# AI4Science-WestlakeU/wdno

Hardware: AMD Instinct MI355X
Metric: diffusion train steps/sec, 2D smoke U-Net (8 samples per GPU per step) (higher is better)
Workload: dtype f32

## Files before the change

### include/wdno_hip.h

```cpp
#ifndef WDNO_HIP_H
#define WDNO_HIP_H
#include <stdint.h>
#include <stddef.h>

#ifdef __cplusplus
extern "C" {
#endif

typedef void* wdno_stream_t;

enum { WDNO_OK = 0, WDNO_EINVAL = -1, WDNO_ELAUNCH = -2, WDNO_EUNSUPPORTED = -3, WDNO_EWORKSPACE = -4 };

#define WDNO_AMAX_SLOTS 64
#define WDNO_AMAX_STRIDE 16
#define WDNO_AMAX_FLOATS (WDNO_AMAX_SLOTS * WDNO_AMAX_STRIDE)
const char* wdno_strerror(int code);
int wdno_version(void);
const char* wdno_last_hip_error(void);
int wdno_set_debug(int mode);

typedef struct {
  int nd;
  int mode;
  int L;
  int n_img;
  int in_dims[3];
  int out_dims[3];
  int64_t cs_img, cs_band, cs0, cs1;
} wdno_dwt_desc;
size_t wdno_dwt_ws_bytes(const wdno_dwt_desc* d);
int wdno_dwt_fwd(const float* x, float* coef, const wdno_dwt_desc* d, const float* filters_host, void* ws, size_t ws_bytes, wdno_stream_t s);
int wdno_dwt_inv(const float* coef, float* x, const wdno_dwt_desc* d, const float* filters_host, void* ws, size_t ws_bytes, wdno_stream_t s);
int wdno_dwt_fwd_adjoint(const float* dcoef, float* dx, const wdno_dwt_desc* d, const float* filters_host, void* ws, size_t ws_bytes, wdno_stream_t s);
int wdno_dwt_inv_adjoint(const float* dx, float* dcoef, const wdno_dwt_desc* d, const float* filters_host, void* ws, size_t ws_bytes, wdno_stream_t s);
int wdno_dwt_fwd_packed(const float* x, float* state, const wdno_dwt_desc* d, const float* filters_host, int img_inner, int64_t cs_outer, int row_w,
                        const float* rescaler, wdno_stream_t s);
int wdno_upsample_coef(const float* in, float* out, int64_t outer, int a, int mid, int b, int c, int fa, int fb, int fc, wdno_stream_t s);
int wdno_pack_smoke_state(const float* coef, int64_t coef_sim_stride, const float* init_coef, int64_t init_sim_stride, const float* smokeout,
                          int64_t so_sim_stride, const int64_t* idx, const float* rescaler, float* state, int64_t B, int F, int nt, int nx,
                          int pad_t, int pad_x, wdno_stream_t s);
int wdno_pack_smoke_fields(const float* coef, int64_t coef_sim_stride, const float* rho0, int64_t rho0_sim_stride, const float* curve,
                           int64_t curve_sim_stride, const float* dec_lo_host, const float* dec_hi_host, int L, const float* rescaler,
                           float* state, int64_t B, int F, int nt, int nx, int pad_t, int pad_x, int H0, int W0, int T0, wdno_stream_t s);

int wdno_nc_to_cl(const float* src, float* dst, int64_t N, int C, int64_t S, int Cp, wdno_stream_t s);
int wdno_cl_to_nc(const float* src, float* dst, int64_t N, int C, int64_t S, int Cp, wdno_stream_t s);
int wdno_concat2_cl_planes(const float* a, int Ca, const float* b, int Cb, const float* rec_a, const float* rec_b, void* hi, void* lo,
                           float* scale_out, int64_t P, wdno_stream_t s);
int wdno_concat2_cl(const float* a, int Ca, const float* b, int Cb, float* out, int64_t P, wdno_stream_t s);
int wdno_concat2_cl_amax(const float* a, int Ca, const float* b, int Cb, float* out, float* amax_rec, int64_t P, wdno_stream_t s);
int wdno_split2_cl(const float* in, float* a, int Ca, float* b, int Cb, int64_t P, wdno_stream_t s);
int wdno_upsample2x_cl_fwd(const float* in, float* out, int64_t N, int H, int W, int C, wdno_stream_t s);
int wdno_upsample2x_cl_bwd(const float* dout, float* din, int64_t N, int H, int W, int C, wdno_stream_t s);

typedef struct {
  int N, D, H, W, C;
  int OD, OH, OW, K;
  int kd, kh, kw;
  int sd, sh, sw;
  int pd, ph, pw;
  int YD, YH, YW;
  int osd, osh, osw, ood, ooh, oow;
} wdno_conv_geom;
int wdno_conv_fwd(const float* x, const float* wp, const float* bias, const float* residual, float* y,
                  const wdno_conv_geom* g, wdno_stream_t s);
int wdno_amax(const float* x, int64_t n, float* amax_zeroed, wdno_stream_t s);
int wdno_amax_record(const float* x, int64_t n, float* rec_zeroed, wdno_stream_t s);
int wdno_split_f16(const float* x, const float* amax_rec, void* hi, void* lo, float* scale_out, int64_t rows, int C, int C8, wdno_stream_t s);
size_t wdno_split_colsum_ws_bytes(int64_t rows, int C8);
int wdno_split_f16_colsum(const float* x, const float* amax_rec, void* hi, void* lo, float* scale_out, float* colsum_out,
                          void* ws, size_t ws_bytes, int64_t rows, int C, int C8, wdno_stream_t s);
int wdno_pack_split_weight(const float* w, const float* amax, void* hi, void* lo, float* scale_out, int K, int C, int kd, int kh, int kw,
                           int A, int B, int mode, wdno_stream_t s);
typedef struct { const void* x; int64_t n; void* out; } wdno_amax_item;
typedef struct {
  const void* w; const void* amax; void* hi; void* lo; void* scale_out;
  int K, C, kd, kh, kw, A, B, mode;
} wdno_wsplit_item;
int wdno_amax_multi(const void* table, int n_items, int blocks_per_item, wdno_stream_t s);
int wdno_pack_split_weight_multi(const void* table, int n_items, int blocks_per_item, wdno_stream_t s);
int wdno_conv_fwd_f16x3(const void* xh, const void* xl, const float* sx, const void* wph, const void* wpl, const float* sw,
                        const float* bias, const float* residual, float* y, const wdno_conv_geom* g, wdno_stream_t s);
int wdno_conv_fwd_f16x3_amax(const void* xh, const void* xl, const float* sx, const void* wph, const void* wpl, const float* sw,
                             const float* bias, const float* residual, float* y, float* amax_rec, const wdno_conv_geom* g,
                             wdno_stream_t s);
typedef struct { int channels, d0, h0, w0; } wdno_zero_box;
int wdno_conv_fwd_f16x3_zbox(const void* xh, const void* xl, const float* sx, const void* wph, const void* wpl, const float* sw,
                             const float* bias, const float* residual, float* y, float* amax_rec, const wdno_conv_geom* g,
                             const wdno_zero_box* zb, wdno_stream_t s);
int wdno_conv_fwd_bf16_ex(const void* x16, const void* wp16, const float* bias, const float* residual, void* y, int y_bf16, float* amax_rec,
                          const wdno_conv_geom* g, const wdno_zero_box* zb, wdno_stream_t s);
int wdno_conv_fwd_f16x3_ws(const void* xh, const void* xl, const float* sx, const void* wph, const void* wpl, const float* sw,
                           const float* bias, const float* residual, float* y, float* amax_rec, const wdno_conv_geom* g,
                           void* ws, size_t ws_bytes, wdno_stream_t s);
size_t wdno_conv_fwd_split_ws_bytes(const wdno_conv_geom* g);
size_t wdno_conv_wgrad_f16x3_ws_bytes(const wdno_conv_geom* g);
int wdno_conv_pixel_table(void* table, const wdno_conv_geom* g, wdno_stream_t s);
int wdno_conv_wgrad_f16x3(const void* xh, const void* xl, const float* sx, const void* dyh, const void* dyl, const float* sdy,
                          const void* pixel_table, float* dwp, void* ws, size_t ws_bytes, const wdno_conv_geom* g, wdno_stream_t s);
int wdno_conv_wgrad_f16x3_param(const void* xh, const void* xl, const float* sx, const void* dyh, const void* dyl, const float* sdy,
                                const void* pixel_table, float* dw, int Kn, int Cn, void* ws, size_t ws_bytes,
                                const wdno_conv_geom* g, wdno_stream_t s);
#define WDNO_WGRAD_REDUCE_MAX 40
typedef struct wdno_wgrad_reduce_item {
  const float* ws; float* dw;
  int n, splits;
  int K8, C8, kw, ntap, Kn, Cn;
  int tiled;
  int reserved;
} wdno_wgrad_reduce_item;
int wdno_conv_wgrad_partials(const void* xh, const void* xl, const float* sx, const void* dyh, const void* dyl, const float* sdy,
                             const void* pixel_table, float* dw, int Kn, int Cn, void* ws, size_t ws_bytes,
                             const wdno_conv_geom* g, wdno_wgrad_reduce_item* item, wdno_stream_t s);
int wdno_wgrad_reduce_multi(const wdno_wgrad_reduce_item* items, int n_items, wdno_stream_t s);
size_t wdno_conv_wgrad_ws_bytes(const wdno_conv_geom* g);
int wdno_conv_wgrad(const float* x, const float* dy, float* dwp, void* ws, size_t ws_bytes,
                    const wdno_conv_geom* g, wdno_stream_t s);
#define WDNO_ROWS_SUM_MAX 64
typedef struct wdno_rows_sum_item {
  const void* part; float* out;
  int rows, stride, col0, ncols;
  int is_double, reserved;
} wdno_rows_sum_item;
int wdno_rows_sum_multi(const wdno_rows_sum_item* items, int n_items, wdno_stream_t s);
size_t wdno_colsum_ws_bytes(int64_t P, int C);
int wdno_colsum(const float* in, float* out, int64_t P, int C, void* ws, size_t ws_bytes, wdno_stream_t s);

int wdno_cast_bf16(const float* x, void* out16, int64_t rows, int C, int C8, wdno_stream_t s);
int wdno_cast_bf16_colsum(const float* x, void* out16, float* colsum_out, void* ws, size_t ws_bytes, int64_t rows, int C, int C8, wdno_stream_t s);
int wdno_conv_fwd_bf16(const void* x16, const void* wp16, const float* bias, const float* residual, float* y, float* amax_rec,
                       const wdno_conv_geom* g, wdno_stream_t s);
int wdno_conv_wgrad_bf16_param(const void* x16, const void* dy16, const void* pixel_table, float* dw, int Kn, int Cn, void* ws,
                               size_t ws_bytes, const wdno_conv_geom* g, wdno_stream_t s);

size_t wdno_groupnorm_ws_bytes(int64_t N, int64_t S, int C, int G);
size_t wdno_groupnorm_stats_floats(int64_t N, int C, int G);
int wdno_groupnorm_act_fwd(const float* x, const float* gamma, const float* beta, const float* ss, float* y,
                           float* stats, int64_t N, int64_t S, int C, int G, float eps, int silu,
                           void* ws, size_t ws_bytes, wdno_stream_t s);
int wdno_groupnorm_act_fwd_amax(const float* x, const float* gamma, const float* beta, const float* ss, float* y,
                                float* stats, float* amax_rec, int64_t N, int64_t S, int C, int G, float eps, int silu,
                                void* ws, size_t ws_bytes, wdno_stream_t s);
int wdno_groupnorm_act_bwd(const float* x, const float* dy, const float* gamma, const float* beta, const float* ss,
                           const float* stats, float* dx, float* dgb_partial, float* dss,
                           int64_t N, int64_t S, int C, int G, int silu, void* ws, size_t ws_bytes, wdno_stream_t s);
int wdno_groupnorm_act_bwd_amax(const float* x, const float* dy, const float* gamma, const float* beta, const float* ss,
                                const float* stats, float* dx, float* dgb_partial, float* dss, float* amax_rec,
                                int64_t N, int64_t S, int C, int G, int silu, void* ws, size_t ws_bytes, wdno_stream_t s);
size_t wdno_groupnorm_bwd_planes_ws_bytes(int64_t N, int64_t S, int C, int G);
size_t wdno_groupnorm_fwd_planes_ws_bytes(int64_t N, int64_t S, int C, int G);
int wdno_groupnorm_act_fwd_planes(const float* x, const float* gamma, const float* beta, const float* ss, void* y_hi, void* y_lo,
                                  float* y_scale, float* stats, float* bound_rec, int64_t N, int64_t S, int C, int G, float eps, int silu,
                                  void* ws, size_t ws_bytes, wdno_stream_t s);
int wdno_groupnorm_act_add_fwd_planes(const float* x, const float* gamma, const float* beta, const float* ss, const float* residual,
                                      const float* res_rec, float* y, void* y_hi, void* y_lo, float* y_scale, float* stats,
                                      float* bound_rec, float* y_amax_rec, int64_t N, int64_t S, int C, int G, float eps, int silu,
                                      void* ws, size_t ws_bytes, wdno_stream_t s);
int wdno_groupnorm_act_bwd_planes(const float* x, const float* dy, const float* gamma, const float* beta, const float* ss,
                                  const float* stats, void* dx_hi, void* dx_lo, float* dx_scale, float* dx_colsum,
                                  float* dgb_partial, float* dgb_sum, float* dss, float* bound_rec, int64_t N, int64_t S, int C, int G, int silu,
                                  void* ws, size_t ws_bytes, wdno_stream_t s);
int wdno_groupnorm_bwd_planes_tail(int64_t N, int64_t S, int C, int G, size_t* csp_offset, int* rows);
int wdno_groupnorm_act_fwd_amax_t(const void* x, int x_bf16, const float* gamma, const float* beta, const float* ss, float* y,
                                  float* stats, float* amax_rec, int64_t N, int64_t S, int C, int G, float eps, int silu,
                                  void* ws, size_t ws_bytes, wdno_stream_t s);
int wdno_groupnorm_act_fwd_planes_t(const void* x, int x_bf16, const float* gamma, const float* beta, const float* ss, void* y_hi, void* y_lo,
                                    float* y_scale, float* stats, float* bound_rec, int64_t N, int64_t S, int C, int G, float eps,
                                    int silu, void* ws, size_t ws_bytes, wdno_stream_t s);
int wdno_groupnorm_act_add_fwd_planes_t(const void* x, int x_bf16, const float* gamma, const float* beta, const float* ss, const float* residual,
                                        const float* res_rec, float* y, void* y_hi, void* y_lo, float* y_scale, float* stats,
                                        float* bound_rec, float* y_amax_rec, int64_t N, int64_t S, int C, int G, float eps, int silu,
                                        void* ws, size_t ws_bytes, wdno_stream_t s);
int wdno_groupnorm_act_bwd_planes_t(const void* x, int x_bf16, const void* dy, int dy_bf16, const float* gamma, const float* beta, const float* ss,
                                    const float* stats, void* dx_hi, void* dx_lo, float* dx_scale, float* dx_colsum,
                                    float* dgb_partial, float* dgb_sum, float* dss, float* bound_rec, int64_t N, int64_t S, int C, int G, int silu,
                                    void* ws, size_t ws_bytes, wdno_stream_t s);
int wdno_layernorm_fwd(const float* x, const float* g, float* y, int64_t P, int C, float eps, wdno_stream_t s);
int wdno_layernorm_fwd_amax(const float* x, const float* g, float* y, float* amax_rec, int64_t P, int C, float eps, wdno_stream_t s);
int wdno_layernorm_fwd_planes(const float* x, const float* g, void* y_hi, void* y_lo, float* y_scale, int64_t P, int C, float eps,
                              wdno_stream_t s);
size_t wdno_layernorm_bwd_ws_bytes(int64_t P, int C);
int wdno_layernorm_bwd(const float* x, const float* g, const float* dy, float* dx, float* dg, int64_t P, int C,
                       float eps, void* ws, size_t ws_bytes, wdno_stream_t s);
int wdno_layernorm_bwd_add(const float* x, const float* g, const float* dy, const float* add_to, float* dx, float* dg, int64_t P, int C,
                           float eps, void* ws, size_t ws_bytes, wdno_stream_t s);
int wdno_layernorm_bwd_add_amax(const float* x, const float* g, const float* dy, const float* add_to, float* dx, float* dg, float* amax_rec,
                                int64_t P, int C, float eps, void* ws, size_t ws_bytes, wdno_stream_t s);

typedef struct {
  int n_uo, n_ui, n_tok, heads;
  int64_t so, si, st;
} wdno_attn_desc;
int wdno_attn_fwd(const float* qkv, const float* rot_cos, const float* rot_sin, const float* bias, float* out,
                  const wdno_attn_desc* d, float scale, wdno_stream_t s);
size_t wdno_attn_bwd_ws_bytes(const wdno_attn_desc* d);
int wdno_attn_bwd(const float* qkv, const float* rot_cos, const float* rot_sin, const float* bias, const float* out,
                  const float* dout, float* dqkv, float* dbias, const wdno_attn_desc* d, float scale, void* ws, size_t ws_bytes,
                  wdno_stream_t s);
int wdno_attn_fwd_amax(const float* qkv, const float* rot_cos, const float* rot_sin, const float* bias, float* out, float* amax_rec,
                       const wdno_attn_desc* d, float scale, wdno_stream_t s);
int wdno_attn_bwd_amax(const float* qkv, const float* rot_cos, const float* rot_sin, const float* bias, const float* out,
                       const float* dout, float* dqkv, float* dbias, float* amax_rec, const wdno_attn_desc* d, float scale,
                       void* ws, size_t ws_bytes, wdno_stream_t s);
int wdno_attn_bwd_planes(const float* qkv, const float* rot_cos, const float* rot_sin, const float* bias, const float* out,
                         const float* dout, void* dqkv_hi, void* dqkv_lo, float* dqkv_scale, float* dbias,
                         const float* rec_qkv, const float* rec_dout, const wdno_attn_desc* d, float scale, void* ws, size_t ws_bytes,
                         wdno_stream_t s);
int wdno_attn_fwd_planes(const float* qkv, const float* rot_cos, const float* rot_sin, const float* bias, float* out, void* out_hi,
                         void* out_lo, float* out_scale, float* amax_rec, const float* rec_qkv, const wdno_attn_desc* d, float scale,
                         wdno_stream_t s);
size_t wdno_linattn_ws_bytes(int64_t units, int heads);
int wdno_linattn_fwd(const float* qkv, float* out, float* kstats , float* ctx ,
                     int64_t units, int n_tok, int heads, float scale, wdno_stream_t s);
int wdno_linattn_bwd(const float* qkv, const float* dout, const float* kstats, const float* ctx, float* dqkv,
                     void* ws, size_t ws_bytes, int64_t units, int n_tok, int heads, float scale, wdno_stream_t s);
int wdno_linattn_fwd_amax(const float* qkv, float* out, float* kstats, float* ctx, float* amax_rec, int64_t units, int n_tok, int heads,
                          float scale, wdno_stream_t s);
int wdno_linattn_bwd_amax(const float* qkv, const float* dout, const float* kstats, const float* ctx, float* dqkv, float* amax_rec,
                          void* ws, size_t ws_bytes, int64_t units, int n_tok, int heads, float scale, wdno_stream_t s);
int wdno_linattn_bwd_planes(const float* qkv, const float* dout, const float* kstats, const float* ctx, void* dqkv_hi, void* dqkv_lo,
                            float* dqkv_scale, const float* rec_qkv, const float* rec_dout, float* rec_dctx, void* ws, size_t ws_bytes,
                            int64_t units, int n_tok, int heads, float scale, wdno_stream_t s);
int wdno_linattn_fwd_planes(const float* qkv, void* out_hi, void* out_lo, float* out_scale, float* kstats, float* ctx,
                            const float* rec_qkv, int64_t units, int n_tok, int heads, float scale, wdno_stream_t s);

int wdno_tattn_fused_takes(int C, int n_tok, int heads);
int wdno_tattn_fused_fwd(const float* x, const float* gamma, float eps, const void* wq_hi, const void* wq_lo, const float* wq_scale,
                         const void* wo_hi, const void* wo_lo, const float* wo_scale, const float* rot_cos, const float* rot_sin,
                         const float* bias, float* y, float* amax_rec, float* qkv_out, float* rec_v,
                         int64_t n_batch, int n_tok, int64_t hw, int C, int heads, float scale, wdno_stream_t s);
size_t wdno_tattn_fused_bwd_ws_bytes(void);
int wdno_tattn_fused_bwd_grads(void);
int wdno_tattn_fused_bwd(const float* x, const float* dy, const float* gamma, float eps, const void* wq_hi, const void* wq_lo,
                         const float* wq_scale, const void* wo_hi, const void* wo_lo, const float* wo_scale, const float* rot_cos,
                         const float* rot_sin, const float* bias, const float* rec_dy, const float* rec_v, float* dx, float* amax_rec,
                         float* grads, void* ws, size_t ws_bytes,
                         int64_t n_batch, int n_tok, int64_t hw, int C, int heads, float scale, wdno_stream_t s);

int wdno_lattn_fused_takes(int C, int heads, int n_tok);
size_t wdno_lattn_fused_ws_bytes(int64_t units, int n_tok);
int wdno_lattn_fused_fwd(const float* x, const float* gamma, float eps, const void* wq_hi, const void* wq_lo, const float* wq_scale,
                         const void* wo_hi, const void* wo_lo, const float* wo_scale, const float* bias_out, float* y, float* amax_rec,
                         float* ctx_out, float* kstat_out, void* ws, size_t ws_bytes, int64_t units, int n_tok, int C, int heads, float scale,
                         wdno_stream_t s);

int wdno_lattn_fused_bwd_grads(void);
size_t wdno_lattn_fused_bwd_ws_bytes(int64_t units, int n_tok);
int wdno_lattn_fused_bwd(const float* x, const float* dy, const float* gamma, float eps, const void* wq_hi, const void* wq_lo,
                         const float* wq_scale, const void* wot_hi, const void* wot_lo, const float* wot_scale, const float* ctx,
                         const float* kstat, const float* rec_dy, float* dx, float* amax_rec, float* grads, void* ws, size_t ws_bytes,
                         int64_t units, int n_tok, int C, int heads, float scale, wdno_stream_t s);

int wdno_relpos_bias_fwd(const float* w, const int64_t* bucket, float* out, int n, int heads, wdno_stream_t s);
int wdno_relpos_bias_bwd(const float* dbias, const int64_t* bucket, float* dw, int n, int heads, int num_buckets, wdno_stream_t s);

int wdno_linear_rows_fwd(const float* x, int x_stride, const float* w, int w_stride, const float* bias, float* y, int P, int C, int K,
                         int Kp, wdno_stream_t s);
int wdno_linear_rows_wgrad(const float* x, int x_stride, const float* dy, int dy_stride, float* dw, float* db, int P, int C, int K,
                           wdno_stream_t s);
// ... 112 lines not shown
```

### wdno_amd/_lib.py

```python
import contextlib
import ctypes as C
import os

import torch

HERE = os.path.dirname(os.path.abspath(__file__))
LIB_PATH = os.path.join(HERE, 'libwdno_hip.so')

P = C.c_void_p
I = C.c_int
L = C.c_int64
F = C.c_float
Z = C.c_size_t


class DwtDesc(C.Structure):
    _fields_ = [('nd', I), ('mode', I), ('L', I), ('n_img', I), ('in_dims', I * 3), ('out_dims', I * 3),
                ('cs_img', L), ('cs_band', L), ('cs0', L), ('cs1', L)]


class ConvGeom(C.Structure):
    _fields_ = [(k, I) for k in ('N', 'D', 'H', 'W', 'C', 'OD', 'OH', 'OW', 'K', 'kd', 'kh', 'kw', 'sd', 'sh', 'sw',
                                 'pd', 'ph', 'pw', 'YD', 'YH', 'YW', 'osd', 'osh', 'osw', 'ood', 'ooh', 'oow')]


class AttnDesc(C.Structure):
    _fields_ = [('n_uo', I), ('n_ui', I), ('n_tok', I), ('heads', I), ('so', L), ('si', L), ('st', L)]


class CondDesc(C.Structure):
    _fields_ = [(k, I) for k in ('tree', 'B', 'F', 'C', 'H', 'W', 'cT', 'cH', 'cW', 'cond_pad', 'cond_a', 'cond_b',
                                 'cond_c', 'cond_low', 'u_rows', 'uT_rows')]


class WgradReduceItem(C.Structure):
    _fields_ = [('ws', C.c_void_p), ('dw', C.c_void_p), ('n', I), ('splits', I), ('K8', I), ('C8', I), ('kw', I), ('ntap', I), ('Kn', I), ('Cn', I),
                ('tiled', I), ('reserved', I)]


class RowsSumItem(C.Structure):
    _fields_ = [('part', C.c_void_p), ('out', C.c_void_p), ('rows', I), ('stride', I), ('col0', I), ('ncols', I), ('is_double', I), ('reserved', I)]


class BurgersDesc(C.Structure):
    _fields_ = [(k, I) for k in ('N', 's', 'nx0', 'nt_f', 'nxf', 'steps', 'record_time', 'f_time', 'num_t', 'sub_s', 'out_cols', 'waves',
                                 'points')] + [(k, F) for k in ('c', 'd', 'dm', 'dt')]


class BurgersGenerateDesc(C.Structure):
    _fields_ = [(k, I) for k in ('N', 's', 't', 'steps', 'record_time', 'f_time', 'num_t', 'st', 'sx', 'f_rows', 'cols', 'waves', 'points',
                                 'clamp')] + [(k, F) for k in ('c', 'd', 'dm', 'dt', 'alpha')]


class BurgersGuidanceDesc(C.Structure):
    _fields_ = [(k, I) for k in ('B', 'C', 'H', 'W', 'sample_stride', 'chan_stride', 'row_stride', 'h', 'w', 'n_t', 'n_x', 'L', 'mode', 'ntile',
                                 'tw', 'lds_bytes', 'num_timesteps', 'condition_f', 'clip_x0')] + [(k, F) for k in ('wu', 'wf')]


class SmokeSolveDesc(C.Structure):
    _fields_ = [(k, I) for k in ('B', 'nt', 'nx', 'time_interval', 'space_interval', 'num_t', 'max_iter', 'n_out', 'threads')] + [('accuracy', F)]


class SmokeGenerateDesc(C.Structure):
    _fields_ = [(k, I) for k in ('B', 'scenelength', 'record_scale', 'stride', 'max_iter', 'threads', 'noise_mode')] + [('accuracy', F), ('seed', C.c_uint64)]


PD, PG, PA, PC = C.POINTER(DwtDesc), C.POINTER(ConvGeom), C.POINTER(AttnDesc), C.POINTER(CondDesc)
PF = C.POINTER(C.c_float)

PROTOTYPES = {
    'wdno_strerror': (C.c_char_p, [I]),
    'wdno_version': (I, []),
    'wdno_last_hip_error': (C.c_char_p, []),
    'wdno_set_debug': (I, [I]),
    'wdno_dwt_ws_bytes': (Z, [PD]),
    'wdno_dwt_fwd': (I, [P, P, PD, PF, P, Z, P]),
    'wdno_dwt_fwd_packed': (I, [P, P, PD, PF, I, L, I, P, P]),
    'wdno_dwt_inv': (I, [P, P, PD, PF, P, Z, P]),
    'wdno_dwt_fwd_adjoint': (I, [P, P, PD, PF, P, Z, P]),
    'wdno_dwt_inv_adjoint': (I, [P, P, PD, PF, P, Z, P]),
    'wdno_upsample_coef': (I, [P, P, L, I, I, I, I, I, I, I, P]),
    'wdno_pack_smoke_state': (I, [P, L, P, L, P, L, P, P, P, L, I, I, I, I, I, P]),
    'wdno_pack_smoke_fields': (I, [P, L, P, L, P, L, PF, PF, I, P, P, L, I, I, I, I, I, I, I, I, P]),
    'wdno_nc_to_cl': (I, [P, P, L, I, L, I, P]),
    'wdno_cl_to_nc': (I, [P, P, L, I, L, I, P]),
    'wdno_concat2_cl': (I, [P, I, P, I, P, L, P]),
    'wdno_concat2_cl_planes': (I, [P, I, P, I, P, P, P, P, P, L, P]),
    'wdno_concat2_cl_amax': (I, [P, I, P, I, P, P, L, P]),
    'wdno_split2_cl': (I, [P, P, I, P, I, L, P]),
    'wdno_upsample2x_cl_fwd': (I, [P, P, L, I, I, I, P]),
    'wdno_upsample2x_cl_bwd': (I, [P, P, L, I, I, I, P]),
    'wdno_conv_fwd': (I, [P, P, P, P, P, PG, P]),
    'wdno_amax': (I, [P, L, P, P]),
    'wdno_amax_record': (I, [P, L, P, P]),
    'wdno_split_f16': (I, [P, P, P, P, P, L, I, I, P]),
    'wdno_split_colsum_ws_bytes': (Z, [L, I]),
    'wdno_split_f16_colsum': (I, [P, P, P, P, P, P, P, Z, L, I, I, P]),
    'wdno_pack_split_weight': (I, [P, P, P, P, P, I, I, I, I, I, I, I, I, P]),
    'wdno_amax_multi': (I, [P, I, I, P]),
    'wdno_pack_split_weight_multi': (I, [P, I, I, P]),
    'wdno_conv_fwd_f16x3': (I, [P, P, P, P, P, P, P, P, P, PG, P]),
    'wdno_conv_fwd_f16x3_amax': (I, [P, P, P, P, P, P, P, P, P, P, PG, P]),
    'wdno_conv_fwd_f16x3_ws': (I, [P, P, P, P, P, P, P, P, P, P, PG, P, Z, P]),
    'wdno_conv_fwd_split_ws_bytes': (Z, [PG]),
    'wdno_conv_wgrad_f16x3_ws_bytes': (Z, [PG]),
    'wdno_conv_pixel_table': (I, [P, PG, P]),
    'wdno_conv_wgrad_f16x3': (I, [P, P, P, P, P, P, P, P, P, Z, PG, P]),
    'wdno_conv_wgrad_f16x3_param': (I, [P, P, P, P, P, P, P, P, I, I, P, Z, PG, P]),
    'wdno_conv_wgrad_partials': (I, [P, P, P, P, P, P, P, P, I, I, P, Z, PG, P, P]),
    'wdno_wgrad_reduce_multi': (I, [P, I, P]),
    'wdno_rows_sum_multi': (I, [P, I, P]),
    'wdno_cast_bf16': (I, [P, P, L, I, I, P]),
    'wdno_cast_bf16_colsum': (I, [P, P, P, P, Z, L, I, I, P]),
    'wdno_conv_fwd_bf16': (I, [P, P, P, P, P, P, PG, P]),
    'wdno_conv_fwd_f16x3_zbox': (I, [P, P, P, P, P, P, P, P, P, P, PG, P, P]),
    'wdno_conv_fwd_bf16_ex': (I, [P, P, P, P, P, I, P, PG, P, P]),
    'wdno_conv_wgrad_bf16_param': (I, [P, P, P, P, I, I, P, Z, PG, P]),
    'wdno_conv_wgrad_ws_bytes': (Z, [PG]),
    'wdno_conv_wgrad': (I, [P, P, P, P, Z, PG, P]),
    'wdno_colsum_ws_bytes': (Z, [L, I]),
    'wdno_colsum': (I, [P, P, L, I, P, Z, P]),
    'wdno_groupnorm_ws_bytes': (Z, [L, L, I, I]),
    'wdno_groupnorm_stats_floats': (Z, [L, I, I]),
    'wdno_groupnorm_act_fwd': (I, [P, P, P, P, P, P, L, L, I, I, F, I, P, Z, P]),
    'wdno_groupnorm_act_fwd_amax': (I, [P, P, P, P, P, P, P, L, L, I, I, F, I, P, Z, P]),
    'wdno_groupnorm_act_bwd': (I, [P, P, P, P, P, P, P, P, P, L, L, I, I, I, P, Z, P]),
    'wdno_groupnorm_act_bwd_amax': (I, [P, P, P, P, P, P, P, P, P, P, L, L, I, I, I, P, Z, P]),
    'wdno_groupnorm_bwd_planes_ws_bytes': (Z, [L, L, I, I]),
    'wdno_groupnorm_bwd_planes_tail': (I, [L, L, I, I, C.POINTER(Z), C.POINTER(I)]),
    'wdno_groupnorm_fwd_planes_ws_bytes': (Z, [L, L, I, I]),
    'wdno_groupnorm_act_fwd_planes': (I, [P, P, P, P, P, P, P, P, P, L, L, I, I, F, I, P, Z, P]),
    'wdno_groupnorm_act_add_fwd_planes': (I, [P, P, P, P, P, P, P, P, P, P, P, P, P, L, L, I, I, F, I, P, Z, P]),
    'wdno_layernorm_fwd_planes': (I, [P, P, P, P, P, L, I, F, P]),
    'wdno_groupnorm_act_bwd_planes': (I, [P, P, P, P, P, P, P, P, P, P, P, P, P, P, L, L, I, I, I, P, Z, P]),
    'wdno_groupnorm_act_fwd_amax_t': (I, [P, I, P, P, P, P, P, P, L, L, I, I, F, I, P, Z, P]),
    'wdno_groupnorm_act_fwd_planes_t': (I, [P, I, P, P, P, P, P, P, P, P, L, L, I, I, F, I, P, Z, P]),
    'wdno_groupnorm_act_add_fwd_planes_t': (I, [P, I, P, P, P, P, P, P, P, P, P, P, P, P, L, L, I, I, F, I, P, Z, P]),
    'wdno_groupnorm_act_bwd_planes_t': (I, [P, I, P, I, P, P, P, P, P, P, P, P, P, P, P, P, L, L, I, I, I, P, Z, P]),
    'wdno_layernorm_fwd': (I, [P, P, P, L, I, F, P]),
    'wdno_layernorm_fwd_amax': (I, [P, P, P, P, L, I, F, P]),
    'wdno_layernorm_bwd_ws_bytes': (Z, [L, I]),
    'wdno_layernorm_bwd': (I, [P, P, P, P, P, L, I, F, P, Z, P]),
    'wdno_layernorm_bwd_add': (I, [P, P, P, P, P, P, L, I, F, P, Z, P]),
    'wdno_layernorm_bwd_add_amax': (I, [P, P, P, P, P, P, P, L, I, F, P, Z, P]),
    'wdno_attn_fwd': (I, [P, P, P, P, P, PA, F, P]),
    'wdno_attn_bwd_ws_bytes': (Z, [PA]),
    'wdno_attn_bwd': (I, [P, P, P, P, P, P, P, P, PA, F, P, Z, P]),
    'wdno_attn_fwd_amax': (I, [P, P, P, P, P, P, PA, F, P]),
    'wdno_attn_bwd_amax': (I, [P, P, P, P, P, P, P, P, P, PA, F, P, Z, P]),
    'wdno_attn_fwd_planes': (I, [P, P, P, P, P, P, P, P, P, P, PA, F, P]),
    'wdno_linattn_fwd_planes': (I, [P, P, P, P, P, P, P, L, I, I, F, P]),
    'wdno_attn_bwd_planes': (I, [P, P, P, P, P, P, P, P, P, P, P, P, PA, F, P, Z, P]),
    'wdno_tattn_fused_takes': (I, [I, I, I]),
    'wdno_tattn_fused_fwd': (I, [P, P, F, P, P, P, P, P, P, P, P, P, P, P, P, P, L, I, L, I, I, F, P]),
    'wdno_lattn_fused_takes': (I, [I, I, I]),
    'wdno_lattn_fused_ws_bytes': (Z, [L, I]),
    'wdno_lattn_fused_fwd': (I, [P, P, F, P, P, P, P, P, P, P, P, P, P, P, P, Z, L, I, I, I, F, P]),
    'wdno_lattn_fused_bwd_grads': (I, []),
    'wdno_lattn_fused_bwd_ws_bytes': (Z, [L, I]),
    'wdno_lattn_fused_bwd': (I, [P, P, P, F, P, P, P, P, P, P, P, P, P, P, P, P, P, Z, L, I, I, I, F, P]),
    'wdno_tattn_fused_bwd_ws_bytes': (Z, []),
    'wdno_tattn_fused_bwd_grads': (I, []),
    'wdno_tattn_fused_bwd': (I, [P, P, P, F, P, P, P, P, P, P, P, P, P, P, P, P, P, P, P, Z, L, I, L, I, I, F, P]),
    'wdno_linattn_ws_bytes': (Z, [L, I]),
    'wdno_linattn_fwd': (I, [P, P, P, P, L, I, I, F, P]),
    'wdno_linattn_bwd': (I, [P, P, P, P, P, P, Z, L, I, I, F, P]),
    'wdno_linattn_fwd_amax': (I, [P, P, P, P, P, L, I, I, F, P]),
    'wdno_linattn_bwd_amax': (I, [P, P, P, P, P, P, P, Z, L, I, I, F, P]),
    'wdno_linattn_bwd_planes': (I, [P, P, P, P, P, P, P, P, P, P, P, Z, L, I, I, F, P]),
    'wdno_act_fwd': (I, [P, P, L, I, P]),
    'wdno_act_bwd': (I, [P, P, P, L, I, P]),
    'wdno_linear_rows_fwd': (I, [P, I, P, I, P, P, I, I, I, I, P]),
    'wdno_linear_rows_wgrad': (I, [P, I, P, I, P, P, I, I, I, P]),
    'wdno_linear_multi_fwd': (I, [P, I, I, P, P, I, I, P]),
    'wdno_linear_multi_wgrad': (I, [P, I, I, P, P, P, P, I, I, P]),
    'wdno_linear_multi_dgrad_ws_bytes': (Z, [I, I, I]),
    'wdno_linear_multi_dgrad': (I, [P, I, I, P, P, I, I, P, Z, P]),
    'wdno_add': (I, [P, P, P, L, P]),
    'wdno_add_amax': (I, [P, P, P, P, L, P]),
    'wdno_sinusoidal_emb': (I, [P, P, P, I, I, P]),
    'wdno_q_sample_cond': (I, [P, P, P, P, P, P, P, PC, P]),
    'wdno_apply_cond': (I, [P, P, PC, P]),
    'wdno_weighted_mse_ws_bytes': (Z, [L]),
    'wdno_weighted_mse': (I, [P, P, P, P, F, P, P, L, L, I, L, P, Z, P]),
    'wdno_weighted_mse_bwd': (I, [P, P, P, P, F, P, P, L, L, I, L, P]),
    'wdno_p_sample_update': (I, [P, P, P, P, P, P, P, P, P, P, P, L, L, I, P]),
    'wdno_ddim_update': (I, [P, P, P, P, P, P, F, F, F, P, P, L, L, P]),
    'wdno_ddim_update_dev': (I, [P, P, P, P, P, P, P, P, P, L, L, P]),
    'wdno_sumsq_ws_bytes': (Z, [L]),
    'wdno_sumsq': (I, [P, L, P, P, Z, P]),
    'wdno_adam_clip_step': (I, [P, P, P, P, L, P, F, F, F, F, F, F, I, P]),
    'wdno_ema_update': (I, [P, P, L, F, P]),
    'wdno_gather_items': (I, [P, I, I, P]),
    'wdno_relpos_bias_fwd': (I, [P, P, P, I, I, P]),
    'wdno_relpos_bias_bwd': (I, [P, P, P, I, I, I, P]),
    'wdno_burgers_solve': (I, [P, P, P, C.POINTER(BurgersDesc), P]),
    'wdno_burgers_generate': (I, [P, P, P, P, P, C.POINTER(BurgersGenerateDesc), P]),
    'wdno_burgers_guidance': (I, [P, P, P, P, P, P, P, P, P, C.POINTER(BurgersGuidanceDesc), PF, P]),
    'wdno_smoke_solve': (I, [P, P, P, P, P, P, P, P, P, P, P, P, P, P, C.POINTER(SmokeSolveDesc), P]),
    'wdno_smoke_generate': (I, [P, P, P, P, P, P, P, P, P, P, P, P, P, P, C.POINTER(SmokeGenerateDesc), P]),
    'wdno_smoke_noise': (I, [P, P, P, P, I, C.c_uint64, P, P]),
}

_lib = None


def load():
    global _lib
    if _lib is not None:
        return _lib
    if not os.path.exists(LIB_PATH):
        raise RuntimeError(f'{LIB_PATH} is missing: run `python -c "import __graft_entry__ as g; g.build()"` '
                           '(there is no CPU / eager fallback for the wdno_amd hot path)')
    lib = C.CDLL(LIB_PATH)
    for name, (res, args) in PROTOTYPES.items():
        fn = getattr(lib, name)
        fn.restype = res
        fn.argtypes = args
    _lib = lib
    if os.environ.get('WDNO_DEBUG'):
# ... 25 lines not shown
```

### wdno_amd/csrc/conv_common.h

```cpp
#pragma once
#include "common.h"

typedef float f32x16 __attribute__((ext_vector_type(16)));

#define BK 32
#define LDS_STRIDE 36

struct ConvP {
  wdno_conv_geom g;
  int R;
  int nchunk;
  int nsteps;
  int64_t P;
  int identity_out;
  int debug;
  int tiles_n;
  int ntiles;
  int ksplit;
  float* amax_rec;
  int tsplit;
  float* split_ws;
  size_t split_ws_bytes;
  int zb_blocks, zb_d, zb_h;
  int out_bf16;
};

__device__ __forceinline__ int xcd_swizzle(int bid, int nwg) {
  int q = nwg >> 3, r = nwg & 7;
  int xcd = bid & 7, idx = bid >> 3;
  int start = xcd < r ? xcd * (q + 1) : r * (q + 1) + (xcd - r) * q;
  return start + idx;
}

__device__ __forceinline__ int64_t out_row(const wdno_conv_geom& g, int64_t p) {
  int ow = (int)(p % g.OW); int64_t t = p / g.OW;
  int oh = (int)(t % g.OH); t /= g.OH;
  int od = (int)(t % g.OD);
  int64_t n = t / g.OD;
  return ((n * g.YD + (od * g.osd + g.ood)) * g.YH + (oh * g.osh + g.ooh)) * g.YW + (ow * g.osw + g.oow);
}

static inline int check_geom(const wdno_conv_geom* g) {
  if (!g) return WDNO_EINVAL;
  if (g->N <= 0 || g->D <= 0 || g->H <= 0 || g->W <= 0 || g->C <= 0 || g->K <= 0) return WDNO_EINVAL;
  if (g->OD <= 0 || g->OH <= 0 || g->OW <= 0 || g->kd <= 0 || g->kh <= 0 || g->kw <= 0) return WDNO_EINVAL;
  if (g->sd <= 0 || g->sh <= 0 || g->sw <= 0 || g->osd <= 0 || g->osh <= 0 || g->osw <= 0) return WDNO_EINVAL;
  if ((g->C & 3) || (g->K & 3)) return WDNO_EUNSUPPORTED;
  if ((g->OD - 1) * g->osd + g->ood >= g->YD || (g->OH - 1) * g->osh + g->ooh >= g->YH || (g->OW - 1) * g->osw + g->oow >= g->YW)
    return WDNO_EINVAL;
  return WDNO_OK;
}
#include "debug_modes.h"
void wdno_wgrad_h3d_plan(const wdno_conv_geom* g, int* bm, int* bn, int* splits, int* pix_per_split, int* splitpair = nullptr);
int wdno_conv_wgrad_h3_dma(const void* xh, const void* xl, const void* dyh, const void* dyl, const float* sx, const float* sdy,
                           const void* table, float* wsf, const wdno_conv_geom* g, hipStream_t st);
int wdno_conv_fwd_h3_dma(const void* xh, const void* xl, const void* wh, const void* wl, const float* sx, const float* sw,
                         const float* bias, const float* residual, float* y, ConvP& p, hipStream_t st, int stages);
bool wdno_conv_h3t_takes(const wdno_conv_geom& g);
int wdno_conv_h3t_split(const wdno_conv_geom& g, int64_t P, int cus);
int wdno_conv_fwd_h3_tap(int shape, const void* xh, const void* xl, const void* wh, const void* wl, const float* sx, const float* sw,
                         const float* bias, const float* residual, float* y, ConvP& p, hipStream_t st);
#ifdef __HIPCC__
__device__ __forceinline__ uint4 bf16x8_from_runs(float4 va, float4 vb) {
  const uint2 A = bf16x4_pack(va), B = bf16x4_pack(vb);
  const auto sx = __builtin_amdgcn_permlane32_swap(A.x, B.x, false, false);
  const auto sy = __builtin_amdgcn_permlane32_swap(A.y, B.y, false, false);
  return make_uint4(sx[0], sy[0], sx[1], sy[1]);
}
__device__ __forceinline__ void lgkm0_barrier() {
  __builtin_amdgcn_s_waitcnt(0xc07f);
  asm volatile("s_barrier" : : : "memory");
}
#endif
static inline void fill_params(ConvP& p, const wdno_conv_geom* g) {
  p.g = *g;
  p.amax_rec = nullptr;
  p.ksplit = 1;
  p.tsplit = 1;
  p.split_ws = nullptr;
  p.split_ws_bytes = 0;
  p.zb_blocks = 0; p.zb_d = 0; p.zb_h = 0;
  p.out_bf16 = 0;
  p.debug = wdno_debug_mode;
  p.R = g->kw * g->C;
  p.nchunk = cdiv(p.R, BK);
  p.nsteps = g->kd * g->kh * p.nchunk;
  p.P = (int64_t)g->N * g->OD * g->OH * g->OW;
  p.identity_out = (g->YD == g->OD && g->YH == g->OH && g->YW == g->OW && g->osd == 1 && g->osh == 1 && g->osw == 1 &&
                    g->ood == 0 && g->ooh == 0 && g->oow == 0) ? 1 : 0;
}
```

### wdno_amd/csrc/conv_h3.hip

```cpp
#include "conv_common.h"
#include <type_traits>
#include <algorithm>

typedef _Float16 half8 __attribute__((ext_vector_type(8)));
typedef __bf16 bf16x8 __attribute__((ext_vector_type(8)));
template <bool LP>
__device__ __forceinline__ f32x16 mfma_16(half8 a, half8 b, f32x16 c) {
  if constexpr (LP) return __builtin_amdgcn_mfma_f32_32x32x16_bf16(__builtin_bit_cast(bf16x8, a), __builtin_bit_cast(bf16x8, b), c, 0, 0, 0);
  else return __builtin_amdgcn_mfma_f32_32x32x16_f16(a, b, c, 0, 0, 0);
}

#define HBK 32
#define HST 40

template <bool RECORD>
__global__ __launch_bounds__(256) void amax_kernel(const float* __restrict__ x, int64_t n, unsigned* __restrict__ out) {
  __shared__ float red[4];
  const int64_t n4 = n >> 2;
  const float4* x4 = reinterpret_cast<const float4*>(x);
  float m = 0.f;
  const int64_t stride = (int64_t)gridDim.x * 1024;
  for (int64_t k0 = (int64_t)blockIdx.x * 1024 + threadIdx.x; k0 < n4; k0 += stride) {
    float4 v[4];
#pragma unroll
// ... 392 lines not shown
  __syncthreads();
  if (nst > 1) load_tile(S1{});
  if (nst > 2) load_tile(S0{});
  for (int step = 0; step < nst; step += 2) {
    iter(S0{}, step);
    if (step + 1 < nst) iter(S1{}, step + 1);
  }

  const float inv = LP ? 1.0f : 1.0f / (sx[0] * sw[0]);
  float am = 0.f;
#pragma unroll
  for (int a = 0; a < TM; ++a) {
#pragma unroll
    for (int e = 0; e < 16; ++e) {
      int row = (e & 3) + 8 * (e >> 2) + 4 * hh;
      int64_t pm = m0 + m_base + a * 32 + row;
      if (pm >= p.P) continue;
      int64_t yr = p.identity_out ? pm : out_row(g, pm);
#pragma unroll
      for (int b = 0; b < TN; ++b) {
        int kc = n0 + n_base + b * 32 + li;
        if (kc < g.K) {
          float v = acc[a][b][e] * inv;
          if (p.ksplit > 1) {
            if (blockIdx.y == 0) {
              if (bias) v += bias[kc];
              if (res) v += res[yr * g.K + kc];
            }
            unsafeAtomicAdd(&y[yr * g.K + kc], v);
            continue;
          }
          if (bias) v += bias[kc];
          if (res) v += res[yr * g.K + kc];
          if (LP && p.out_bf16) reinterpret_cast<unsigned short*>(y)[yr * g.K + kc] = bf16_rne(v);
          else y[yr * g.K + kc] = v;
          am = fmaxf(am, fabsf(v));
        }
      }
    }
  }
  if (p.amax_rec) wave_amax_emit(am, p.amax_rec, (int)blockIdx.x * 4 + wave);
}

template <int BM, int BN, int WM, int WN, bool LP>
static int launch_h3(const void* xh, const void* xl, const void* wh, const void* wl, const float* sx, const float* sw,
                     const float* bias, const float* residual, float* y, ConvP& p, hipStream_t st) {
  const wdno_conv_geom& g = p.g;
  int64_t tiles_m = cdiv64(p.P, BM);
  p.tiles_n = cdiv(g.K, BN);
  int64_t nt = tiles_m * p.tiles_n;
  if (nt > 0x7fffffff) return WDNO_EUNSUPPORTED;
  p.ntiles = (int)nt;
  size_t lds = (size_t)2 * (LP ? 1 : 2) * (BM + BN) * HST * sizeof(_Float16);
  static bool attr_done = false;
  if (!attr_done) {
    (void)hipFuncSetAttribute((const void*)conv_fwd_h3_kernel<BM, BN, WM, WN, LP>, hipFuncAttributeMaxDynamicSharedMemorySize, (int)lds);
    attr_done = true;
  }
  const int64_t x_elems = (int64_t)g.N * g.D * g.H * g.W * g.C;
  const int64_t w_elems = (int64_t)g.kd * g.kh * g.K * p.R;
  if (x_elems * 2 >= OOB_OFFSET || w_elems * 2 >= OOB_OFFSET || p.P >= 0x7fffffff) return WDNO_EUNSUPPORTED;
  float* rec = p.amax_rec;
  if (p.ksplit > 1) {
    if (hipMemsetAsync(y, 0, (size_t)p.P * g.K * sizeof(float), st) != hipSuccess) return WDNO_ELAUNCH;
    p.amax_rec = nullptr;
  }
  conv_fwd_h3_kernel<BM, BN, WM, WN, LP><<<dim3((unsigned)p.ntiles, (unsigned)p.ksplit), 256, lds, st>>>(
      (const _Float16*)xh, (const _Float16*)xl, (const _Float16*)wh, (const _Float16*)wl, sx, sw, bias, residual, y, p,
      (unsigned)(x_elems * 2), (unsigned)(w_elems * 2));
  if (p.ksplit > 1 && rec) {
    amax_kernel<true><<<stream_grid(p.P * g.K / 16 + 1, 256), 256, 0, st>>>(y, p.P * g.K, reinterpret_cast<unsigned*>(rec));
    p.amax_rec = rec;
  }
  return WDNO_OK;
}

extern "C" int wdno_conv_fwd_f16x3(const void* xh, const void* xl, const float* sx, const void* wph, const void* wpl, const float* sw,
                                   const float* bias, const float* residual, float* y, const wdno_conv_geom* g, wdno_stream_t s) {
  return wdno_conv_fwd_f16x3_amax(xh, xl, sx, wph, wpl, sw, bias, residual, y, nullptr, g, s);
}
template <bool LP>
static int conv_fwd_16(const void* xh, const void* xl, const float* sx, const void* wph, const void* wpl, const float* sw,
                       const float* bias, const float* residual, float* y, float* amax_rec, const wdno_conv_geom* g, wdno_stream_t s,
                       float* split_ws = nullptr, size_t split_ws_bytes = 0, const wdno_zero_box* zb = nullptr, int y_bf16 = 0) {
  int rc = check_geom(g);
  if (rc) return rc;
  if (g->C & 7) return WDNO_EUNSUPPORTED;
  if (y_bf16 && (!LP || residual)) return WDNO_EUNSUPPORTED;
  ConvP p;
  fill_params(p, g);
  p.out_bf16 = y_bf16 ? 1 : 0;
  if (zb) {
    if (zb->channels < 0 || zb->d0 < 0 || zb->h0 < 0 || zb->w0 < 0) return WDNO_EINVAL;
    p.zb_blocks = zb->channels / 16; p.zb_d = zb->d0; p.zb_h = zb->h0;
  }
  p.amax_rec = amax_rec;
  p.split_ws = split_ws;
  p.split_ws_bytes = split_ws_bytes;
  p.nchunk = cdiv(p.R, HBK);
  p.nsteps = g->kd * g->kh * p.nchunk;
  hipStream_t st = as_stream(s);
  const int64_t P = p.P;
  const int K = g->K;
  auto blocks = [&](int bm, int bn) { return cdiv64(P, bm) * cdiv(K, bn); };
  const int dbg = wdno_debug_mode;
  const bool small_tap = p.identity_out && wdno_conv_h3t_takes(*g) && g->kw == 3 && blocks(64, 64) >= 64;
  if (dbg != WDNO_DBG_ROW_ATTN_AND_REG_STAGED_CONV && (dbg == WDNO_DBG_FORCE_DMA_CONV || dbg == WDNO_DBG_CHUNKED_DMA_CONV || dbg == WDNO_DBG_FORCE_TILES_160 || dbg == WDNO_DBG_FORCE_TILES_320 || small_tap || (K > 64 ? blocks(128, 128) : blocks(256, 64)) >= 100)) {
    rc = wdno_conv_fwd_h3_dma(xh, LP ? nullptr : xl, wph, LP ? nullptr : wpl, sx, sw, bias, residual, y, p, st, 3);
    if (rc == WDNO_OK) return wdno_check_launch();
    if (rc != WDNO_EUNSUPPORTED) return rc;
  }
  if (K > 64) {
    if (blocks(128, 128) >= 512 || blocks(64, 128) < 2 * blocks(128, 128)) rc = launch_h3<128, 128, 2, 2, LP>(xh, xl, wph, wpl, sx, sw, bias, residual, y, p, st);
    else if (blocks(64, 128) < 200) {
      if (blocks(64, 64) <= 384 && g->kd * g->kh >= 2 && p.nsteps >= 64 && p.identity_out && residual != y && !LP) p.ksplit = 2;
      rc = launch_h3<64, 64, 2, 2, LP>(xh, xl, wph, wpl, sx, sw, bias, residual, y, p, st);
    }
    else rc = launch_h3<64, 128, 1, 4, LP>(xh, xl, wph, wpl, sx, sw, bias, residual, y, p, st);
  } else {
    if (blocks(128, 64) >= 512 || P <= 128) rc = launch_h3<128, 64, 4, 1, LP>(xh, xl, wph, wpl, sx, sw, bias, residual, y, p, st);
    else rc = launch_h3<64, 64, 2, 2, LP>(xh, xl, wph, wpl, sx, sw, bias, residual, y, p, st);
  }
  if (rc) return rc;
  return wdno_check_launch();
}
extern "C" int wdno_conv_fwd_f16x3_amax(const void* xh, const void* xl, const float* sx, const void* wph, const void* wpl, const float* sw,
                                        const float* bias, const float* residual, float* y, float* amax_rec, const wdno_conv_geom* g,
                                        wdno_stream_t s) {
  return conv_fwd_16<false>(xh, xl, sx, wph, wpl, sw, bias, residual, y, amax_rec, g, s);
}
extern "C" int wdno_conv_fwd_f16x3_ws(const void* xh, const void* xl, const float* sx, const void* wph, const void* wpl, const float* sw,
                                      const float* bias, const float* residual, float* y, float* amax_rec, const wdno_conv_geom* g,
                                      void* ws, size_t ws_bytes, wdno_stream_t s) {
  return conv_fwd_16<false>(xh, xl, sx, wph, wpl, sw, bias, residual, y, amax_rec, g, s, (float*)ws, ws ? ws_bytes : 0);
}
extern "C" int wdno_conv_fwd_f16x3_zbox(const void* xh, const void* xl, const float* sx, const void* wph, const void* wpl, const float* sw,
                                        const float* bias, const float* residual, float* y, float* amax_rec, const wdno_conv_geom* g,
                                        const wdno_zero_box* zb, wdno_stream_t s) {
  return conv_fwd_16<false>(xh, xl, sx, wph, wpl, sw, bias, residual, y, amax_rec, g, s, nullptr, 0, zb);
}
extern "C" int wdno_conv_fwd_bf16_ex(const void* x16, const void* wp16, const float* bias, const float* residual, void* y, int y_bf16, float* amax_rec,
                                     const wdno_conv_geom* g, const wdno_zero_box* zb, wdno_stream_t s) {
  return conv_fwd_16<true>(x16, x16, nullptr, wp16, wp16, nullptr, bias, residual, (float*)y, amax_rec, g, s, nullptr, 0, zb, y_bf16);
}
extern "C" size_t wdno_conv_fwd_split_ws_bytes(const wdno_conv_geom* g) {
  if (!g || check_geom(g) || (g->C & 7)) return 0;
  ConvP p;
  fill_params(p, g);
  if (!p.identity_out || !wdno_conv_h3t_takes(*g)) return 0;
  const int runs = wdno_conv_h3t_split(*g, p.P, wdno_num_cus() & ~7);
  return runs > 1 ? (size_t)runs * p.P * g->K * sizeof(float) : 0;
}
extern "C" int wdno_conv_fwd_bf16(const void* x16, const void* wp16, const float* bias, const float* residual, float* y, float* amax_rec,
                                  const wdno_conv_geom* g, wdno_stream_t s) {
  return conv_fwd_16<true>(x16, x16, nullptr, wp16, wp16, nullptr, bias, residual, y, amax_rec, g, s);
}

typedef _Float16 half4 __attribute__((ext_vector_type(4)));
#define WH_BKP 32
#define WH_PAD 32

__global__ __launch_bounds__(256) void pixel_table_kernel(int4v* __restrict__ tbl, wdno_conv_geom g, int P) {
  int p = blockIdx.x * 256 + threadIdx.x;
  if (p >= P) return;
  int q = p;
  int ow = q % g.OW; q /= g.OW;
  int oh = q % g.OH; q /= g.OH;
  int od = q % g.OD;
  int n = q / g.OD;
  int d0 = od * g.sd - g.pd, h0 = oh * g.sh - g.ph, w0 = ow * g.sw - g.pw;
  int4v e;
  e.x = ((n * g.YD + (od * g.osd + g.ood)) * g.YH + (oh * g.osh + g.ooh)) * g.YW + (ow * g.osw + g.oow);
  e.y = (((n * g.D + d0) * g.H + h0) * g.W + w0) * g.C;
  e.z = (d0 << 16) | (h0 & 0xffff);
  e.w = w0;
  tbl[p] = e;
}
extern "C" int wdno_conv_pixel_table(void* table, const wdno_conv_geom* g, wdno_stream_t s) {
  int rc = check_geom(g);
  if (rc) return rc;
  int64_t P = (int64_t)g->N * g->OD * g->OH * g->OW;
  if (P >= 0x7fffffff || (int64_t)g->N * g->D * g->H * g->W * g->C >= 0x3fffffff) return WDNO_EUNSUPPORTED;
  pixel_table_kernel<<<(unsigned)cdiv64(P, 256), 256, 0, as_stream(s)>>>((int4v*)table, *g, (int)P);
  return wdno_check_launch();
}

struct WgradHP {
  ConvP c;
  int tiles_k, tiles_r, splits, bn;
  int64_t pix_per_split;
  int xcd_group;
};

__device__ __forceinline__ half8 tr_frag(const _Float16* tile, int stride, int pix0, int ch0, int lane) {
  const int g = lane >> 4, xl = lane & 15;
  const _Float16* p0 = tile + (pix0 + 8 * (g >> 1) + (xl >> 2)) * stride + ch0 + 16 * (g & 1) + 4 * (xl & 3);
  typedef short short4v __attribute__((ext_vector_type(4)));
  typedef short4v __attribute__((address_space(3))) * lds_s4;
  short4v a = __builtin_amdgcn_ds_read_tr16_b64_v4i16((lds_s4)(p0));
  short4v b = __builtin_amdgcn_ds_read_tr16_b64_v4i16((lds_s4)(p0 + 4 * stride));
  typedef short short8v __attribute__((ext_vector_type(8)));
  short8v c = __builtin_shufflevector(a, b, 0, 1, 2, 3, 4, 5, 6, 7);
  return __builtin_bit_cast(half8, c);
}

#define WH_RING 4
template <int BM, int BN, int WM, int WN, bool LP>
__global__ __launch_bounds__(256) void conv_wgrad_h3_kernel(const _Float16* __restrict__ xh, const _Float16* __restrict__ xl,
                                                             const _Float16* __restrict__ dyh, const _Float16* __restrict__ dyl,
                                                             const float* __restrict__ sx, const float* __restrict__ sdy,
                                                             const int4v* __restrict__ table, float* __restrict__ ws, WgradHP wpz,
                                                             unsigned x_bytes, unsigned dy_bytes) {
  constexpr int TM = BM / (WM * 32);
  constexpr int TN = BN / (WN * 32);
  constexpr int SA = BM + WH_PAD, SB = BN + WH_PAD;
  constexpr int A_C8 = BM / 8, B_C8 = BN / 8;
  constexpr int A_RPP = 256 / A_C8;
  constexpr int A_PASSES = WH_BKP / A_RPP, B_PASSES = WH_BKP * B_C8 / 256;
  static_assert(256 % A_C8 == 0 && (WH_BKP * B_C8) % 256 == 0, "loader mapping");
  constexpr int NPL = LP ? 1 : 2;
  constexpr int STAGE = NPL * WH_BKP * (SA + SB);
  extern __shared__ __attribute__((aligned(16))) _Float16 hsm[];
  int4v* pinfo = reinterpret_cast<int4v*>(hsm + 2 * STAGE);

  const ConvP& p = wpz.c;
  const wdno_conv_geom& g = p.g;
// ... 618 lines not shown
```

### wdno_amd/csrc/conv_h3t.hip

```cpp
#include "conv_common.h"
#include <type_traits>

typedef _Float16 half8 __attribute__((ext_vector_type(8)));
typedef __bf16 bf16x8 __attribute__((ext_vector_type(8)));
typedef int int4v __attribute__((ext_vector_type(4)));
#define T_OOB 0x7ffffff0

template <bool LP>
__device__ __forceinline__ f32x16 t_mfma(half8 a, half8 b, f32x16 c) {
  if constexpr (LP) return __builtin_amdgcn_mfma_f32_32x32x16_bf16(__builtin_bit_cast(bf16x8, a), __builtin_bit_cast(bf16x8, b), c, 0, 0, 0);
  else return __builtin_amdgcn_mfma_f32_32x32x16_f16(a, b, c, 0, 0, 0);
}
__device__ __forceinline__ int4v t_rsrc(const void* ptr, unsigned bytes) {
  uint64_t a = reinterpret_cast<uint64_t>(ptr);
  int4v r;
  r.x = __builtin_amdgcn_readfirstlane((int)(unsigned)a);
  r.y = __builtin_amdgcn_readfirstlane((int)(unsigned)((a >> 32) & 0xffffu));
  r.z = __builtin_amdgcn_readfirstlane((int)bytes);
  r.w = 0x00020000;
  return r;
}
__device__ __forceinline__ void t_piece(int4v rsrc, int off, unsigned lds_dst) {
  lds_dst = __builtin_amdgcn_readfirstlane(lds_dst);
  asm volatile("s_mov_b32 m0, %1\n\ts_nop 0\n\tbuffer_load_dwordx4 %0, %2, 0 offen lds" : : "v"(off), "s"(lds_dst), "s"(rsrc) : "memory");
}

struct TapLive { unsigned z[2], y[2]; };
__device__ __forceinline__ unsigned t_bits(int lo, int hi, int k) {
  lo = max(lo, 0); hi = min(hi, k - 1);
  return hi >= lo ? ((2u << hi) - 1u) & ~((1u << lo) - 1u) : 0u;
}
__device__ __forceinline__ TapLive t_tap_live(const wdno_conv_geom& g, int p0, int p1, int zb_d, int zb_h) {
  const int hw = g.OH * g.OW;
  const int f0 = p0 / hw, f1 = p1 / hw;
  const int od0 = f0 % g.OD, od1 = f1 % g.OD;
  const int oh0 = (p0 - f0 * hw) / g.OW, oh1 = (p1 - f1 * hw) / g.OW;
  TapLive t;
#pragma unroll
  for (int c = 0; c < 2; ++c) {
    const int dl = c ? g.D : min(g.D, zb_d), hl = c ? g.H : min(g.H, zb_h);
    t.z[c] = f1 - f0 > 1 ? t_bits(0, g.kd - 1, g.kd) : t_bits(g.pd - od0, dl - 1 + g.pd - od0, g.kd) | t_bits(g.pd - od1, dl - 1 + g.pd - od1, g.kd);
    t.y[c] = f0 == f1 ? t_bits(g.ph - oh1, hl - 1 + g.ph - oh0, g.kh)
           : f1 - f0 == 1 ? t_bits(g.ph - (g.OH - 1), hl - 1 + g.ph - oh0, g.kh) | t_bits(g.ph - oh1, hl - 1 + g.ph, g.kh)
           : t_bits(g.ph - (g.OH - 1), hl - 1 + g.ph, g.kh);
  }
  return t;
}
__device__ __forceinline__ int t_live_stages(const TapLive& t, int ncb, int nzb) {
  const int n = __builtin_popcount(t.z[0]) * __builtin_popcount(t.y[0]) * nzb + __builtin_popcount(t.z[1]) * __builtin_popcount(t.y[1]) * (ncb - nzb);
  return (n + 1) & ~1;
}

template <int BM, int BN, int KW, int CB>
struct TapShape {
  static constexpr int ROWB = CB * 2;
  static constexpr int RPP = 1024 / ROWB;
  static constexpr int ZR = CB == 32 ? 4 : 16;
  static constexpr int AROWS = BM + KW - 1;
  static constexpr int ZB = (AROWS + ZR - 1) / ZR * ZR;
  static constexpr int APIECES = (ZB + ZR + RPP - 1) / RPP;
  static constexpr int A_PLANE = APIECES * 1024;
  static constexpr int BPIECES = (KW * BN + RPP - 1) / RPP;
  static constexpr int B_PLANE = BPIECES * 1024;
};

template <int BM, int BN, int WM, int WN, int KW, int CB, bool LP, bool SP = false>
__global__ __launch_bounds__(512) void conv_fwd_h3t_kernel(const _Float16* __restrict__ xh, const _Float16* __restrict__ xl,
                                                            const _Float16* __restrict__ wh, const _Float16* __restrict__ wl,
                                                            const float* __restrict__ sx, const float* __restrict__ sw,
                                                            const float* __restrict__ bias, const float* __restrict__ res,
                                                            float* __restrict__ y, ConvP p, unsigned x_bytes, unsigned w_bytes) {
  using S = TapShape<BM, BN, KW, CB>;
  constexpr int TM = BM / (WM * 32), TN = BN / (WN * 32);
  constexpr int NPL = LP ? 1 : 2;
  constexpr int ROWB = S::ROWB, RPP = S::RPP, CPR = ROWB / 16;
  constexpr int A_PLANE = S::A_PLANE, B_PLANE = S::B_PLANE;
  constexpr int A_LO = A_PLANE, B_HI = NPL * A_PLANE, B_LO = B_HI + B_PLANE;
  constexpr int STAGE = NPL * (A_PLANE + B_PLANE);
  constexpr int PA = (S::APIECES + 3) / 4, PB = (S::BPIECES + 3) / 4;
  constexpr int KSN = CB / 16;
  constexpr int NSUB = KSN * KW;
  extern __shared__ __attribute__((aligned(1024))) char smem[];
  const wdno_conv_geom& g = p.g;
  const int tid = threadIdx.x;
  const int wave = __builtin_amdgcn_readfirstlane(tid >> 6), lane = tid & 63;
  const int nruns = SP ? p.tsplit : 1;
  const int nvt = p.ntiles * nruns;
  const int my_tiles = (nvt - (int)blockIdx.x + (int)gridDim.x - 1) / (int)gridDim.x;
  const int ncb = (g.C + CB - 1) / CB;
  const bool padded = (NSUB & 1) && ((g.kd * g.kh * ncb) & 1);
  const int nstages = g.kd * g.kh * ncb / nruns + (padded ? 1 : 0);
  constexpr bool SKIP = KW == 7 && !SP;
  const int nzb = SKIP ? p.zb_blocks : 0;
  const bool skipping = SKIP && p.zb_blocks >= 0 && p.debug != WDNO_DBG_STEM_EVERY_STAGE;
  auto tile_live = [&](int t) {
    const int vt = xcd_swizzle((int)blockIdx.x + t * (int)gridDim.x, nvt);
    const int m0 = (vt / p.tiles_n) * BM;
    return t_tap_live(g, m0, min(m0 + BM, (int)p.P) - 1, nzb > 0 ? p.zb_d : g.D, nzb > 0 ? p.zb_h : g.H);
  };

  if (wave >= WM * WN) {
    const int pq = wave - WM * WN;
    int4v rxh = t_rsrc(xh, x_bytes), rxl = t_rsrc(xl, x_bytes), rwh = t_rsrc(wh, w_bytes), rwl = t_rsrc(wl, w_bytes);
    asm volatile("s_nop 4" : "+s"(rxh), "+s"(rxl), "+s"(rwh), "+s"(rwl));
    const unsigned lds0 = __builtin_amdgcn_readfirstlane((unsigned)(size_t)(__attribute__((address_space(3))) char*)smem);
    const int prow = lane / CPR;
    const int c8 = (CB == 32 ? ((lane & 3) ^ ((lane >> 4) & 3)) : ((lane & 1) ^ ((lane >> 4) & 1))) * 8;
    int a_off[PA], b_off[PB];
    unsigned a_mask[PA];
    bool b_ok[PB];
    auto tap_bits = [](int c0, int k, int n) -> unsigned {
      int lo = c0 < 0 ? -c0 : 0, hi = n - c0 < k ? n - c0 : k;
      return hi > lo ? ((1u << hi) - 1u) & ~((1u << lo) - 1u) : 0u;
    };
    int c_tile = 0, s_dz = 0, s_dy = 0, s_cb = 0, s_rem = 0;
    int x_uni = 0, w_uni = 0;
    TapLive lv = {{0u, 0u}, {0u, 0u}};
    int s_cnt = 0;
    auto next_live = [&]() {
      for (;;) {
        if (++s_cb == ncb) { s_cb = 0; if (++s_dy == g.kh) { s_dy = 0; ++s_dz; } }
        if (s_dz >= g.kd) return;
        const int c = s_cb < nzb ? 0 : 1;
        if (((lv.z[c] >> s_dz) & 1u) && ((lv.y[c] >> s_dy) & 1u)) return;
      }
    };
    auto setup_tile = [&](int t) {
      const int vt = xcd_swizzle((int)blockIdx.x + t * (int)gridDim.x, nvt);
      const int run = SP ? vt / p.ntiles : 0, tile = vt - run * p.ntiles;
      if constexpr (SP) {
        const int g0 = run * nstages;
        s_cb = g0 % ncb;
        s_dy = (g0 / ncb) % g.kh;
        s_dz = g0 / (ncb * g.kh);
        s_rem = nstages;
        x_uni = ((s_dz * g.H + s_dy) * g.W * g.C + s_cb * CB) * 2;
        w_uni = ((s_dz * g.kh + s_dy) * g.K * p.R + s_cb * CB) * 2;
      }
      const int tile_m = tile / p.tiles_n, tile_n = tile - tile_m * p.tiles_n;
      const int64_t p0 = (int64_t)tile_m * BM;
#pragma unroll
      for (int i = 0; i < PA; ++i) {
        const int r = RPP * (pq + 4 * i) + prow;
        const int64_t pr = p0 + r - g.pw;
        const bool live = r < S::AROWS && pr >= 0 && pr < p.P;
        int q = live ? (int)pr : 0;
        q /= g.OW;
        const int oh = q % g.OH; q /= g.OH;
        const int od = q % g.OD;
        a_mask[i] = live ? (tap_bits(od - g.pd, g.kd, g.D) | (tap_bits(oh - g.ph, g.kh, g.H) << 8)) : 0u;
        a_off[i] = (((int)pr - (g.pd * g.H + g.ph) * g.W) * g.C + c8) * 2;
      }
#pragma unroll
      for (int i = 0; i < PB; ++i) {
        const int row = RPP * (pq + 4 * i) + prow;
        const int dx = row / BN, k = tile_n * BN + (row - dx * BN);
        b_ok[i] = k < g.K && dx < KW;
        b_off[i] = (k * p.R + dx * g.C + c8) * 2;
      }
    };
    bool fresh = true;
    if (my_tiles > 0) setup_tile(0);
    const bool no_dma = p.debug == WDNO_DBG_NO_DMA || p.debug >= WDNO_DBG_NO_DMA_OFFSET;
    auto issue_stage = [&](int buf) {
      if (skipping) {
        if (fresh) {
          lv = tile_live(c_tile);
          s_dz = 0; s_dy = 0; s_cb = -1; s_cnt = 0; fresh = false;
          next_live();
        }
        x_uni = ((s_dz * g.H + s_dy) * g.W * g.C + s_cb * CB) * 2;
        w_uni = ((s_dz * g.kh + s_dy) * g.K * p.R + s_cb * CB) * 2;
      }
      const bool pad = s_dz == g.kd;
      const unsigned need = pad ? 0x10000u : (1u << s_dz) | (1u << (8 + s_dy));
// ... 145 lines not shown
      for (int i = 0; i < NMF; ++i) {
        __builtin_amdgcn_sched_group_barrier(0x008, 1, 0);
        if (i * RPM < NRD) __builtin_amdgcn_sched_group_barrier(0x100, RPM, 0);
      }
    };
    auto stage_body = [&](auto PARC, auto LASTC) {
      constexpr int PAR = decltype(PARC)::value;
      constexpr bool LAST = decltype(LASTC)::value;
#pragma unroll
      for (int sub = 0; sub < NSUB; ++sub) {
        if (sub + 1 < NSUB) {
          read_frags((PAR + sub + 1) & 1, boff, (sub + 1) / KSN, (sub + 1) % KSN);
        } else if (!LAST) {
          boff = STAGE - boff;
          lgkm0_barrier();
          read_frags((PAR + NSUB) & 1, boff, 0, 0);
        }
        mfma_set((PAR + sub) & 1);
        if (sub + 1 < NSUB || !LAST) interleave();
        __builtin_amdgcn_sched_barrier(0);
      }
    };
    using P0 = std::integral_constant<int, 0>;
    using P1 = std::integral_constant<int, 1>;
    if constexpr (NSUB % 2 == 0) {
      for (int s = 0; s + 1 < nstages; ++s) stage_body(P0{}, std::false_type{});
      stage_body(P0{}, std::true_type{});
    } else if constexpr (KW != 7) {
      for (int s = 0; s + 2 < nstages; s += 2) { stage_body(P0{}, std::false_type{}); stage_body(P1{}, std::false_type{}); }
      stage_body(P0{}, std::false_type{});
      stage_body(P1{}, std::true_type{});
    } else {
      const unsigned allz = (1u << g.kd) - 1u, ally = (1u << g.kh) - 1u;
      const TapLive lvc = skipping ? tile_live(t) : TapLive{{allz, allz}, {ally, ally}};
      const int nst = t_live_stages(lvc, ncb, nzb);
      f32x16 acc2[TM][TN];
#pragma unroll
      for (int a = 0; a < TM; ++a)
#pragma unroll
        for (int b = 0; b < TN; ++b)
#pragma unroll
          for (int e = 0; e < 16; ++e) asm volatile("v_mov_b32 %0, 0" : "=v"(acc2[a][b][e]));
      int g_dz = 0, g_dy = -1, flush_at = 0;
      auto next_row = [&]() {
        for (;;) {
          if (++g_dy == g.kh) { g_dy = 0; ++g_dz; }
          if (g_dz >= g.kd) { flush_at = 0x7fffffff; return; }
          const int n = (int)((lvc.z[0] >> g_dz) & (lvc.y[0] >> g_dy) & 1u) * nzb + (int)((lvc.z[1] >> g_dz) & (lvc.y[1] >> g_dy) & 1u) * (ncb - nzb);
          if (n) { flush_at += n; return; }
        }
      };
      next_row();
      auto row_done = [&](int done) {
        if (done != flush_at) return;
#pragma unroll
        for (int a = 0; a < TM; ++a)
#pragma unroll
          for (int b = 0; b < TN; ++b)
#pragma unroll
            for (int e = 0; e < 16; ++e) {
              acc2[a][b][e] += acc[a][b][e];
              asm volatile("v_mov_b32 %0, 0" : "=v"(acc[a][b][e]));
            }
        next_row();
      };
      for (int s = 0; s + 2 < nst; s += 2) {
        stage_body(P0{}, std::false_type{}); row_done(s + 1);
        stage_body(P1{}, std::false_type{}); row_done(s + 2);
      }
      stage_body(P0{}, std::false_type{}); row_done(nst - 1);
      stage_body(P1{}, std::true_type{});
#pragma unroll
      for (int a = 0; a < TM; ++a)
#pragma unroll
        for (int b = 0; b < TN; ++b)
#pragma unroll
          for (int e = 0; e < 16; ++e) acc[a][b][e] += acc2[a][b][e];
    }
    boff = STAGE - boff;
    const uint64_t e_begin = stamps ? __builtin_amdgcn_s_memtime() : 0;
#pragma unroll
    for (int a = 0; a < TM; ++a) {
      const int64_t pm = m0 + m_base + a * 32 + li;
      if (pm >= p.P) continue;
      const int64_t yr = pm;
      if constexpr (SP) {
        float* wrow = p.split_ws + ((int64_t)run * p.P + pm) * g.K;
#pragma unroll
        for (int b = 0; b < TN; ++b) {
#pragma unroll
          for (int e4 = 0; e4 < 4; ++e4) {
            const int kc = n0 + n_base + b * 32 + 8 * e4 + 4 * hh;
            if (kc < g.K) *reinterpret_cast<float4*>(wrow + kc) = make_float4(acc[a][b][4 * e4], acc[a][b][4 * e4 + 1], acc[a][b][4 * e4 + 2], acc[a][b][4 * e4 + 3]);
          }
        }
        continue;
      }
      float* yrow = y + yr * g.K;
      const float* rrow = res ? res + yr * g.K : nullptr;
      if (LP && p.out_bf16) {
        unsigned short* y16 = reinterpret_cast<unsigned short*>(y) + yr * g.K;
#pragma unroll
        for (int b = 0; b < TN; ++b) {
#pragma unroll
          for (int e4 = 0; e4 < 4; e4 += 2) {
            const int k0 = n0 + n_base + b * 32 + 8 * e4;
            if (k0 >= g.K) continue;
            const int ka = k0 + 4 * hh, kb = ka + 8;
            float4 va = make_float4(acc[a][b][4 * e4] * inv, acc[a][b][4 * e4 + 1] * inv, acc[a][b][4 * e4 + 2] * inv, acc[a][b][4 * e4 + 3] * inv);
            float4 vb = make_float4(acc[a][b][4 * e4 + 4] * inv, acc[a][b][4 * e4 + 5] * inv, acc[a][b][4 * e4 + 6] * inv, acc[a][b][4 * e4 + 7] * inv);
            if (bias) {
              const float4 ta = *reinterpret_cast<const float4*>(bias + ka);
              va.x += ta.x; va.y += ta.y; va.z += ta.z; va.w += ta.w;
              if (k0 + 8 < g.K) { const float4 tb = *reinterpret_cast<const float4*>(bias + kb); vb.x += tb.x; vb.y += tb.y; vb.z += tb.z; vb.w += tb.w; }
            }
            const uint4 o = bf16x8_from_runs(va, vb);
            if (k0 + 8 * hh < g.K) *reinterpret_cast<uint4*>(y16 + k0 + 8 * hh) = o;
            am = amax4(amax4(am, va), vb);
          }
        }
        continue;
      }
#pragma unroll
      for (int b = 0; b < TN; ++b) {
#pragma unroll
        for (int e4 = 0; e4 < 4; ++e4) {
          const int kc = n0 + n_base + b * 32 + 8 * e4 + 4 * hh;
          if (kc < g.K) {
            float4 v = make_float4(acc[a][b][4 * e4] * inv, acc[a][b][4 * e4 + 1] * inv, acc[a][b][4 * e4 + 2] * inv, acc[a][b][4 * e4 + 3] * inv);
            if (bias) { const float4 tb = *reinterpret_cast<const float4*>(bias + kc); v.x += tb.x; v.y += tb.y; v.z += tb.z; v.w += tb.w; }
            if (rrow) { const float4 tr = *reinterpret_cast<const float4*>(rrow + kc); v.x += tr.x; v.y += tr.y; v.z += tr.z; v.w += tr.w; }
            *reinterpret_cast<float4*>(yrow + kc) = v;
            am = amax4(am, v);
          }
        }
      }
    }
    if (stamps) c_epi += __builtin_amdgcn_s_memtime() - e_begin;
  }
  if (stamps) am = sdbg == WDNO_DBG_STAMP_CYCLES ? (float)(__builtin_amdgcn_s_memtime() - c_begin) : sdbg == WDNO_DBG_STAMP_EPILOGUE ? (float)c_epi : (float)(__builtin_amdgcn_s_memrealtime() - r_begin);
  if (p.amax_rec) wave_amax_emit(am, p.amax_rec, (int)blockIdx.x * (WM * WN) + wave);
}

__global__ __launch_bounds__(256) void conv_split_reduce_kernel(const float4* __restrict__ ws, int nruns, int64_t n4, int K4, const float* __restrict__ sx,
                                                                 const float* __restrict__ sw, const float4* __restrict__ bias, const float4* res,
                                                                 float4* y, float* __restrict__ amax_rec) {
  const float inv = sx ? 1.0f / (sx[0] * sw[0]) : 1.0f;
  float am = 0.f;
  for (int64_t i = (int64_t)blockIdx.x * 256 + threadIdx.x; i < n4; i += (int64_t)gridDim.x * 256) {
    float4 v = ws[i];
    for (int r = 1; r < nruns; ++r) { const float4 u = ws[(int64_t)r * n4 + i]; v.x += u.x; v.y += u.y; v.z += u.z; v.w += u.w; }
    v.x *= inv; v.y *= inv; v.z *= inv; v.w *= inv;
    if (bias) { const float4 tb = bias[(int)(i % K4)]; v.x += tb.x; v.y += tb.y; v.z += tb.z; v.w += tb.w; }
    if (res) { const float4 tr = res[i]; v.x += tr.x; v.y += tr.y; v.z += tr.z; v.w += tr.w; }
    y[i] = v;
    am = amax4(am, v);
  }
  if (amax_rec) wave_amax_emit(am, amax_rec, (int)blockIdx.x * 4 + (int)(threadIdx.x >> 6));
}

template <int BM, int BN, int WM, int WN, int KW, int CB, bool LP, bool SP = false>
static int launch_h3t(const void* xh, const void* xl, const void* wh, const void* wl, const float* sx, const float* sw,
                      const float* bias, const float* residual, float* y, ConvP& p, hipStream_t st) {
  using S = TapShape<BM, BN, KW, CB>;
  const wdno_conv_geom& g = p.g;
  int64_t tiles_m = cdiv64(p.P, BM);
  p.tiles_n = cdiv(g.K, BN);
  int64_t nt = tiles_m * p.tiles_n;
  if (nt > 0x7fffffff) return WDNO_EUNSUPPORTED;
  p.ntiles = (int)nt;
  constexpr size_t lds = (size_t)2 * (LP ? 1 : 2) * (S::A_PLANE + S::B_PLANE);
  static_assert(lds <= 160 * 1024, "two stages must fit the LDS");
  const int64_t x_elems = (int64_t)g.N * g.D * g.H * g.W * g.C;
  const int64_t w_elems = (int64_t)g.kd * g.kh * g.K * p.R;
  if (x_elems * 2 >= T_OOB || w_elems * 2 >= T_OOB || p.P >= 0x7fffffff - BM) return WDNO_EUNSUPPORTED;
  if (SP) {
    const int nst = g.kd * g.kh * ((g.C + CB - 1) / CB);
    if (p.tsplit < 2 || ((CB / 16) * KW & 1) || nst % p.tsplit || !p.split_ws || (size_t)p.tsplit * p.P * g.K * sizeof(float) > p.split_ws_bytes || (g.K & 3))
      return WDNO_EINVAL;
  } else p.tsplit = 1;
  int grid = wdno_num_cus() & ~7;
  if (grid < 8) grid = 8;
  if ((int64_t)p.ntiles * p.tsplit < grid) grid = p.ntiles * p.tsplit;
  static bool done = false;
  if (!done) { (void)hipFuncSetAttribute((const void*)conv_fwd_h3t_kernel<BM, BN, WM, WN, KW, CB, LP, SP>, hipFuncAttributeMaxDynamicSharedMemorySize, (int)lds); done = true; }
  conv_fwd_h3t_kernel<BM, BN, WM, WN, KW, CB, LP, SP><<<grid, 512, lds, st>>>((const _Float16*)xh, (const _Float16*)xl, (const _Float16*)wh, (const _Float16*)wl,
                                                                    sx, sw, bias, residual, y, p, (unsigned)(x_elems * 2), (unsigned)(w_elems * 2));
  if (p.tsplit > 1) {
    const int64_t n4 = p.P * g.K / 4;
    conv_split_reduce_kernel<<<(unsigned)std::min<int64_t>((n4 + 255) / 256, 2048), 256, 0, st>>>(
        (const float4*)p.split_ws, p.tsplit, n4, g.K / 4, LP ? nullptr : sx, sw, (const float4*)bias, (const float4*)residual, (float4*)y, p.amax_rec);
  }
  return WDNO_OK;
}

static bool t_stem(const wdno_conv_geom& g) { return g.kw == 7 && (g.C % 16) == 0 && g.K <= 64; }
bool wdno_conv_h3t_takes(const wdno_conv_geom& g) {
  return g.sd == 1 && g.sh == 1 && g.sw == 1 && g.OD == g.D && g.OH == g.H && g.OW == g.W && ((g.kw == 3 && (g.C % 32) == 0) || t_stem(g)) &&
         g.kd <= 8 && g.kh <= 8 && wdno_debug_mode != WDNO_DBG_CHUNKED_DMA_CONV;
}
int wdno_conv_h3t_split(const wdno_conv_geom& g, int64_t P, int cus) {
  if (wdno_debug_mode == WDNO_DBG_CONV_NO_RUN_SPLIT || g.kw != 3 || (g.C % 32) || g.K < 128 || (g.K & 3)) return 1;
  const int64_t t128 = cdiv64(P, 128) * cdiv(g.K, 128);
  const int nst = g.kd * g.kh * (g.C / 32);
  return t128 * 4 <= cus && nst % 4 == 0 && nst / 4 >= 8 ? 4 : 1;
}
template <bool LP>
static int fwd_h3t(int shape, const void* xh, const void* xl, const void* wh, const void* wl, const float* sx, const float* sw,
                   const float* bias, const float* residual, float* y, ConvP& p, hipStream_t st) {
  if (shape == 0 && p.tsplit > 1 && !LP) return launch_h3t<128, 128, 2, 2, 3, 32, false, true>(xh, xl, wh, wl, sx, sw, bias, residual, y, p, st);
  if (shape == 0) return launch_h3t<128, 128, 2, 2, 3, 32, LP>(xh, xl, wh, wl, sx, sw, bias, residual, y, p, st);
  if (shape == 1) return launch_h3t<192, 128, 2, 2, 3, 32, LP>(xh, xl, wh, wl, sx, sw, bias, residual, y, p, st);
  if (shape == 3) return launch_h3t<192, 64, 2, 2, 3, 32, LP>(xh, xl, wh, wl, sx, sw, bias, residual, y, p, st);
  if (shape == 4) return launch_h3t<160, 128, 1, 4, 3, 32, LP>(xh, xl, wh, wl, sx, sw, bias, residual, y, p, st);
  if (shape == 5) return launch_h3t<320, 64, 2, 2, 3, 32, LP>(xh, xl, wh, wl, sx, sw, bias, residual, y, p, st);
  if (shape == 6) return launch_h3t<64, 64, 2, 2, 3, 32, LP>(xh, xl, wh, wl, sx, sw, bias, residual, y, p, st);
  if (shape == 7) return launch_h3t<128, 64, 2, 2, 3, 32, LP>(xh, xl, wh, wl, sx, sw, bias, residual, y, p, st);
  return launch_h3t<256, 64, 4, 1, 3, 32, LP>(xh, xl, wh, wl, sx, sw, bias, residual, y, p, st);
}
int wdno_conv_fwd_h3_tap(int shape, const void* xh, const void* xl, const void* wh, const void* wl, const float* sx, const float* sw,
                         const float* bias, const float* residual, float* y, ConvP& p, hipStream_t st) {
  if (p.g.kw == 7) {
    const int ncb = (p.g.C + 15) / 16;
    if (p.zb_blocks >= ncb) p.zb_blocks = ncb - 1;
    const int cus = wdno_num_cus();
    if (xl != nullptr && cdiv64(p.P, 256) < cus && cdiv64(p.P, 192) <= cus && cdiv64(p.P, 192) > cdiv64(p.P, 256) && wdno_debug_mode != WDNO_DBG_STEM_TILES_256)
      return launch_h3t<192, 64, 2, 2, 7, 16, false>(xh, xl, wh, wl, sx, sw, bias, residual, y, p, st);
    if (xl == nullptr) return launch_h3t<256, 64, 4, 1, 7, 16, true>(xh, xh, wh, wh, sx, sw, bias, residual, y, p, st);
    return launch_h3t<256, 64, 4, 1, 7, 16, false>(xh, xl, wh, wl, sx, sw, bias, residual, y, p, st);
  }
  if (xl == nullptr && p.g.K > 64 && cdiv64(p.P, 256) * cdiv(p.g.K, 128) >= 2 * wdno_num_cus())
    return launch_h3t<256, 128, 4, 1, 3, 32, true>(xh, xh, wh, wh, sx, sw, bias, residual, y, p, st);
  if (xl == nullptr) return fwd_h3t<true>(shape, xh, xh, wh, wh, sx, sw, bias, residual, y, p, st);
  return fwd_h3t<false>(shape, xh, xl, wh, wl, sx, sw, bias, residual, y, p, st);
}
```

### wdno_amd/csrc/debug_modes.h

```cpp
#pragma once

#define WDNO_DEBUG_MODES(X)                                                                                                                       \
  X(WDNO_DBG_OFF, 0)                                                                                                               \
                                \
  X(WDNO_DBG_ROW_ATTN_AND_REG_STAGED_CONV, 5)                                                                                                      \
  X(WDNO_DBG_WGRAD_NO_XCD_GROUPING, 6)   \
  X(WDNO_DBG_FORCE_DMA_CONV, 7)                     \
       \
  X(WDNO_DBG_CHUNKED_DMA_CONV, 8)                                                                                                                  \
                                                                                                               \
  X(WDNO_DBG_PER_AXIS_DWT_AND_WGRAD_WINDOW_K64, 11)                                                                                                \
  X(WDNO_DBG_DWT_SKIP_W_PASS, 12)                                        \
  X(WDNO_DBG_DWT_SKIP_H_PASS, 13)                                                    \
  X(WDNO_DBG_DWT_SKIP_T_PASS, 14)                                     \
     \
  X(WDNO_DBG_NO_DMA, 21)                                                                                                                           \
  X(WDNO_DBG_WGRAD_NO_DMA_NO_PIECE, 22)                  \
            \
  X(WDNO_DBG_STAMP_CYCLES, 23)                                                         \
  X(WDNO_DBG_STAMP_EPILOGUE, 24)                                                                          \
  X(WDNO_DBG_STAMP_REALTIME, 26)                                          \
  X(WDNO_DBG_FORCE_TILES_160, 30)           \
  X(WDNO_DBG_FORCE_TILES_320, 31)                                   \
  X(WDNO_DBG_ATTN_GENERIC_NTOK, 44)      \
  X(WDNO_DBG_DWT3_SYNTH_LDS, 45)              \
  X(WDNO_DBG_CONV_NO_RUN_SPLIT, 56)      \
  X(WDNO_DBG_STEM_EVERY_STAGE, 57)                  \
  X(WDNO_DBG_ATTN_FWD_ROWS, 67)          \
  X(WDNO_DBG_ATTN_BWD_ROWS, 68)                                              \
  X(WDNO_DBG_WGRAD_NO_SPLIT_PAIR, 70)    \
  X(WDNO_DBG_STEM_TILES_256, 72)                             \
                               \
  X(WDNO_DBG_NO_DMA_STAMP_CYCLES, 123)                                                                                                             \
  X(WDNO_DBG_NO_DMA_STAMP_EPILOGUE, 124)                                                                                                           \
  X(WDNO_DBG_NO_DMA_STAMP_REALTIME, 126)

enum wdno_debug : int {
#define WDNO_DBG_ENUM(name, value) name = value,
  WDNO_DEBUG_MODES(WDNO_DBG_ENUM)
#undef WDNO_DBG_ENUM
  WDNO_DBG_NO_DMA_OFFSET = 100
};

extern int wdno_debug_mode;
```

### wdno_amd/csrc/norm.hip

```cpp
#include "common.h"
#include <type_traits>

#define GN_MAXC 1024

struct gn_bf16 {};
template <typename T> struct gn_ld;
template <> struct gn_ld<float> {
  static __device__ __forceinline__ float4 ld4(const void* p, int64_t e) { return *reinterpret_cast<const float4*>(static_cast<const float*>(p) + e); }
};
template <> struct gn_ld<gn_bf16> {
  static __device__ __forceinline__ float4 ld4(const void* p, int64_t e) {
    const uint2 u = *reinterpret_cast<const uint2*>(static_cast<const unsigned short*>(p) + e);
    return make_float4(__uint_as_float(u.x << 16), __uint_as_float(u.x & 0xffff0000u), __uint_as_float(u.y << 16), __uint_as_float(u.y & 0xffff0000u));
  }
};
template <typename T> __device__ __forceinline__ void gn_ld8(const void* p, int64_t e, float (&v)[8]) {
  const float4 a = gn_ld<T>::ld4(p, e), b = gn_ld<T>::ld4(p, e + 4);
  v[0] = a.x; v[1] = a.y; v[2] = a.z; v[3] = a.w; v[4] = b.x; v[5] = b.y; v[6] = b.z; v[7] = b.w;
}

static inline int pow2ceil(int v) { int p = 1; while (p < v) p <<= 1; return p; }
static inline int gn_chunks(int64_t S, int64_t N, int C) {
  int64_t c = cdiv64(S, 64);
  if (c > 64) c = 64;
// ... 58 lines not shown
          float dv[4] = {d.x, d.y, d.z, d.w};
#pragma unroll
          for (int j = 0; j < 4; ++j) {
            float dz = dv[j];
            if (silu) dz *= silu_grad_f(ca[j] * xv[j] + cbb[j]);
            float xh = (xv[j] - mean[j]) * rstd[j];
            s0[j] += (double)dz;
            s1[j] += (double)dz * (double)xh;
            m0[j] = fmaxf(m0[j], fabsf(dz)); m1[j] = fmaxf(m1[j], fabsf(xh));
          }
        }
      }
    }
  }
#pragma unroll
  for (int j = 0; j < 4; ++j) { red[(ty * txp + tx) * 8 + j] = s0[j]; red[(ty * txp + tx) * 8 + 4 + j] = s1[j]; }
  __syncthreads();
  if (ty == 0 && tx < C4) {
    for (int t = 1; t < nty; ++t)
#pragma unroll
      for (int j = 0; j < 4; ++j) { s0[j] += red[(t * txp + tx) * 8 + j]; s1[j] += red[(t * txp + tx) * 8 + 4 + j]; }
    double* o = part + (((int64_t)n * nchunk + chunk) * C + tx * 4) * 2;
#pragma unroll
    for (int j = 0; j < 4; ++j) { o[j * 2] = s0[j]; o[j * 2 + 1] = s1[j]; }
  }
  if (mx) {
    float a = fmaxf(fmaxf(m0[0], m0[1]), fmaxf(m0[2], m0[3])), b = fmaxf(fmaxf(m1[0], m1[1]), fmaxf(m1[2], m1[3]));
    a = wave_max(a); b = wave_max(b);
    if ((threadIdx.x & 63) == 0) { redm[(threadIdx.x >> 6) * 2] = a; redm[(threadIdx.x >> 6) * 2 + 1] = b; }
    __syncthreads();
    if (threadIdx.x == 0) {
      float* o = mx + ((int64_t)n * nchunk + chunk) * 2;
      o[0] = fmaxf(fmaxf(redm[0], redm[2]), fmaxf(redm[4], redm[6]));
      o[1] = fmaxf(fmaxf(redm[1], redm[3]), fmaxf(redm[5], redm[7]));
    }
  }
}

__device__ __forceinline__ void gn_chunk_totals(const double* __restrict__ part, int n, int nchunk, int Call, double* sa, double* sb, int cb0 = 0, int cn = -1) {
  const int C = cn < 0 ? Call : cn;
  part += cb0 * 2;
  const int nsub = C <= 128 ? 256 / C : 1;
  for (int idx = threadIdx.x; idx < C * nsub; idx += 256) {
    const int q = idx / C, c = idx - q * C;
    const int k1 = (q + 1) * nchunk / nsub;
    int k = q * nchunk / nsub;
    double a0 = 0, b0 = 0, a1 = 0, b1 = 0;
    for (; k + 7 < k1; k += 8) {
      const double* q0 = part + (((int64_t)n * nchunk + k) * Call + c) * 2;
      double va[8], vb[8];
#pragma unroll
      for (int u = 0; u < 8; ++u) { va[u] = q0[(int64_t)u * Call * 2]; vb[u] = q0[(int64_t)u * Call * 2 + 1]; }
#pragma unroll
      for (int u = 0; u < 8; u += 2) { a0 += va[u]; b0 += vb[u]; a1 += va[u + 1]; b1 += vb[u + 1]; }
    }
    for (; k + 1 < k1; k += 2) {
      const double* q0 = part + (((int64_t)n * nchunk + k) * Call + c) * 2;
      const double* q1 = q0 + (int64_t)Call * 2;
      a0 += q0[0]; b0 += q0[1]; a1 += q1[0]; b1 += q1[1];
    }
    if (k < k1) {
      const double* q0 = part + (((int64_t)n * nchunk + k) * Call + c) * 2;
      a0 += q0[0]; b0 += q0[1];
    }
    sa[idx] = a0 + a1; sb[idx] = b0 + b1;
  }
  __syncthreads();
  if (nsub > 1) {
    const int c = threadIdx.x;
    double a = 0, b = 0;
    if (c < C)
      for (int q = 0; q < nsub; ++q) { a += sa[q * C + c]; b += sb[q * C + c]; }
    __syncthreads();
    if (c < C) { sa[c] = a; sb[c] = b; }
    __syncthreads();
  }
}

__global__ __launch_bounds__(256) void gn_finalize_kernel(const double* __restrict__ part, const float* __restrict__ stats_in,
                                                           const float* __restrict__ gamma, const float* __restrict__ beta,
                                                           const float* __restrict__ ss, float* __restrict__ stats_out,
                                                           float* __restrict__ cb, float* __restrict__ gb, int64_t S, int C, int G,
                                                           int nchunk, float eps, const float* __restrict__ mx = nullptr,
                                                           float* __restrict__ bound_rec = nullptr) {
  __shared__ double chs[GN_MAXC], chq[GN_MAXC];
  __shared__ float gmean[GN_MAXC], grstd[GN_MAXC];
  const int n = blockIdx.x, cg = C / G;
  const int gps = (G + (int)gridDim.y - 1) / (int)gridDim.y, gs0 = (int)blockIdx.y * gps, gs1 = min(G, gs0 + gps);
  if (gs0 >= gs1) return;
  const int cs0 = gs0 * cg, csn = (gs1 - gs0) * cg;
  gamma += cs0; beta += cs0;
  if (ss) ss += cs0;
  cb += (int64_t)cs0 * 4; gb += (int64_t)gs0 * 4;
  if (stats_out) stats_out += (int64_t)gs0 * 2;
  if (stats_in) stats_in += (int64_t)gs0 * 2;
  const int Call = C, Gall = G;
  C = csn; G = gs1 - gs0;
  if (part) {
    gn_chunk_totals(part, n, nchunk, Call, chs, chq, cs0, csn);
    if (cg > 64) {
      __shared__ double ra[256], rb[256];
      for (int g = 0; g < G; ++g) {
        double a = 0, b = 0;
        for (int c = g * cg + threadIdx.x; c < (g + 1) * cg; c += 256) { a += chs[c]; b += chq[c]; }
        ra[threadIdx.x] = a; rb[threadIdx.x] = b;
        __syncthreads();
        for (int o = 128; o > 0; o >>= 1) {
          if (threadIdx.x < o) { ra[threadIdx.x] += ra[threadIdx.x + o]; rb[threadIdx.x] += rb[threadIdx.x + o]; }
          __syncthreads();
        }
        if (threadIdx.x == 0) { chs[g * cg] = ra[0]; chq[g * cg] = rb[0]; }
        __syncthreads();
      }
    }
    for (int g = threadIdx.x; g < G; g += 256) {
      double a = 0, b = 0;
      if (cg > 64) { a = chs[g * cg]; b = chq[g * cg]; }
      else for (int c = g * cg; c < (g + 1) * cg; ++c) { a += chs[c]; b += chq[c]; }
      double m = (double)cg * (double)S;
      double mean = a / m;
      double var = b / m - mean * mean;
      if (var < 0) var = 0;
      float rstd = (float)(1.0 / sqrt(var + (double)eps));
      gmean[g] = (float)mean; grstd[g] = rstd;
      stats_out[((int64_t)n * Gall + g) * 2 + 0] = (float)mean;
      stats_out[((int64_t)n * Gall + g) * 2 + 1] = rstd;
    }
  } else {
    for (int g = threadIdx.x; g < G; g += 256) {
      gmean[g] = stats_in[((int64_t)n * Gall + g) * 2 + 0];
      grstd[g] = stats_in[((int64_t)n * Gall + g) * 2 + 1];
    }
  }
  __syncthreads();
  for (int g = threadIdx.x; g < G; g += 256) {
    float* o = gb + ((int64_t)n * Gall + g) * 4;
    o[0] = gmean[g]; o[1] = grstd[g]; o[2] = 0.f; o[3] = 0.f;
  }
  float ma = 0.f, mb = 0.f;
  for (int c = threadIdx.x; c < C; c += 256) {
    int g = c / cg;
    float sc1 = ss ? ss[(int64_t)n * 2 * Call + c] + 1.0f : 1.0f;
    float sh = ss ? ss[(int64_t)n * 2 * Call + Call + c] : 0.0f;
    float k1 = grstd[g] * gamma[c];
    float a = k1 * sc1;
    float b = (beta[c] - gmean[g] * k1) * sc1 + sh;
    float* o = cb + ((int64_t)n * Call + c) * 4;
    o[0] = a; o[1] = b; o[2] = a; o[3] = 0.f;
    ma = fmaxf(ma, fabsf(a)); mb = fmaxf(mb, fabsf(b));
  }
  if (bound_rec) {
    float mxx = 0.f;
    for (int k = threadIdx.x; k < nchunk; k += 256) mxx = fmaxf(mxx, mx[((int64_t)n * nchunk + k) * 2]);
    __shared__ float bm[3][4];
    float v[3] = {wave_max(ma), wave_max(mb), wave_max(mxx)};
    if ((threadIdx.x & 63) == 0)
      for (int q = 0; q < 3; ++q) bm[q][threadIdx.x >> 6] = v[q];
    __syncthreads();
    if (threadIdx.x == 0) {
      float t[3];
      for (int q = 0; q < 3; ++q) t[q] = fmaxf(fmaxf(bm[q][0], bm[q][1]), fmaxf(bm[q][2], bm[q][3]));
      atomicMax(reinterpret_cast<unsigned*>(bound_rec) + (n & (WDNO_AMAX_SLOTS - 1)) * WDNO_AMAX_STRIDE, __float_as_uint(t[0] * t[2] + t[1]));
    }
  }
}

template <typename XT = float>
__global__ __launch_bounds__(256) void gn_apply_kernel(const void* __restrict__ x, const float* __restrict__ cb, float* __restrict__ y,
                                                        int64_t S, int C, int silu, float* __restrict__ amax_rec) {
  const int n = blockIdx.y;
  const int C4 = C >> 2;
  const int64_t total4 = S * C4;
  const int64_t xe = (int64_t)n * S * C;
  float4* yp = reinterpret_cast<float4*>(y + (int64_t)n * S * C);
  const float4* cbp = reinterpret_cast<const float4*>(cb + (int64_t)n * C * 4);
  const int64_t stride = (int64_t)gridDim.x * 256;
  float am = 0.f;
  for (int64_t i = (int64_t)blockIdx.x * 256 + threadIdx.x; i < total4; i += stride) {
    int c4 = (int)(i % C4);
    float4 v = gn_ld<XT>::ld4(x, xe + i * 4);
    float4 k0 = cbp[c4 * 4 + 0], k1 = cbp[c4 * 4 + 1], k2 = cbp[c4 * 4 + 2], k3 = cbp[c4 * 4 + 3];
    float4 o;
    o.x = k0.x * v.x + k0.y; o.y = k1.x * v.y + k1.y; o.z = k2.x * v.z + k2.y; o.w = k3.x * v.w + k3.y;
    if (silu) { o.x = silu_f(o.x); o.y = silu_f(o.y); o.z = silu_f(o.z); o.w = silu_f(o.w); }
    yp[i] = o;
    am = amax4(am, o);
  }
  if (amax_rec) amax_record_emit(am, amax_rec, blockIdx.y * gridDim.x + blockIdx.x);
}

__global__ __launch_bounds__(256) void gn_bwd_finalize_kernel(const double* __restrict__ part, const float* __restrict__ gamma,
                                                               const float* __restrict__ beta, const float* __restrict__ ss,
                                                               float* __restrict__ gb, float* __restrict__ dgb, float* __restrict__ dss,
                                                               int64_t S, int C, int G, int nchunk, const float* __restrict__ cb = nullptr,
                                                               const float* __restrict__ mx = nullptr, float* __restrict__ bound_rec = nullptr) {
  __shared__ double chA[GN_MAXC], chB[GN_MAXC];
  const int n = blockIdx.x, cg = C / G;
  const int gps = (G + (int)gridDim.y - 1) / (int)gridDim.y, gs0 = (int)blockIdx.y * gps, gs1 = min(G, gs0 + gps);
  if (gs0 >= gs1) return;
  const int cs0 = gs0 * cg, csn = (gs1 - gs0) * cg;
  gamma += cs0; beta += cs0;
  if (ss) ss += cs0;
  if (dss) dss += cs0;
  dgb += cs0; gb += (int64_t)gs0 * 4;
  if (cb) cb += (int64_t)cs0 * 4;
  const int Call = C, Gall = G;
  C = csn; G = gs1 - gs0;
  gn_chunk_totals(part, n, nchunk, Call, chA, chB, cs0, csn);
  for (int c = threadIdx.x; c < C; c += 256) {
    const double a = chA[c], b = chB[c];
    float sc1 = ss ? ss[(int64_t)n * 2 * Call + c] + 1.0f : 1.0f;
    if (dss) {
      dss[(int64_t)n * 2 * Call + c] = (float)((double)gamma[c] * b + (double)beta[c] * a);
      dss[(int64_t)n * 2 * Call + Call + c] = (float)a;
    }
    dgb[((int64_t)n * 2 + 0) * Call + c] = (float)((double)sc1 * b);
    dgb[((int64_t)n * 2 + 1) * Call + c] = (float)((double)sc1 * a);
    double w = (double)gamma[c] * (double)sc1;
    chA[c] = w * a; chB[c] = w * b;
  }
  __syncthreads();
  if (cg > 64) {
    __shared__ double ra[256], rb[256];
    for (int g = 0; g < G; ++g) {
      double a = 0, b = 0;
      for (int c = g * cg + threadIdx.x; c < (g + 1) * cg; c += 256) { a += chA[c]; b += chB[c]; }
      ra[threadIdx.x] = a; rb[threadIdx.x] = b;
      __syncthreads();
      for (int o = 128; o > 0; o >>= 1) {
        if (threadIdx.x < o) { ra[threadIdx.x] += ra[threadIdx.x + o]; rb[threadIdx.x] += rb[threadIdx.x + o]; }
        __syncthreads();
      }
      if (threadIdx.x == 0) { chA[g * cg] = ra[0]; chB[g * cg] = rb[0]; }
      __syncthreads();
    }
  }
// ... 144 lines not shown
      ov[j] = o;
      am = fmaxf(am, fabsf(o));
      _Float16 th, tl;
      plane_pack(o, s, single, th, tl);
      h[j] = th; l[j] = tl;
    }
    *reinterpret_cast<float4*>(yp + i * 8) = make_float4(ov[0], ov[1], ov[2], ov[3]);
    *reinterpret_cast<float4*>(yp + i * 8 + 4) = make_float4(ov[4], ov[5], ov[6], ov[7]);
    if (planes) *reinterpret_cast<gn_half8*>(hp + i * 8) = h;
    if (planes && !single) *reinterpret_cast<gn_half8*>(lp + i * 8) = l;
  }
  if (amax_out) amax_record_emit(am, amax_out, blockIdx.y * gridDim.x + blockIdx.x);
}

template <typename XT = float, typename DT = float>
__global__ __launch_bounds__(256) void gn_bwd_apply_planes_kernel(const void* __restrict__ x, const void* __restrict__ dy,
                                                                   const float* __restrict__ cb, const float* __restrict__ gb,
                                                                   _Float16* __restrict__ hi, _Float16* __restrict__ lo,
                                                                   float* __restrict__ scale_out, const float* __restrict__ rec,
                                                                   double* __restrict__ csp, int64_t S, int C, int cg, int G, int silu) {
  __shared__ double red[256][9];
  const int n = blockIdx.y;
  const int C8 = C >> 3;
  const int64_t total8 = S * C8;
  const bool single = lo == nullptr;
  const float s = single ? 1.0f : scale_from_amax(amax_record_read(rec));
  if (!single && blockIdx.x == 0 && blockIdx.y == 0 && threadIdx.x == 0) scale_out[0] = s;
  const int64_t xe = (int64_t)n * S * C;
  _Float16* hp = hi + (int64_t)n * S * C;
  _Float16* lp = single ? nullptr : lo + (int64_t)n * S * C;
  const float4* cbp = reinterpret_cast<const float4*>(cb + (int64_t)n * C * 4);
  const float4* gbp = reinterpret_cast<const float4*>(gb + (int64_t)n * G * 4);
  const int64_t stride = (int64_t)gridDim.x * 256;
  const int c0 = (int)(((int64_t)blockIdx.x * 256 + threadIdx.x) % C8) * 8;
  float4 kk[8], gq[8];
#pragma unroll
  for (int j = 0; j < 8; ++j) { kk[j] = cbp[c0 + j]; gq[j] = gbp[(c0 + j) / cg]; }
  double acc[8] = {0, 0, 0, 0, 0, 0, 0, 0};
  for (int64_t i = (int64_t)blockIdx.x * 256 + threadIdx.x; i < total8; i += stride) {
    float xv[8], dv[8];
    gn_ld8<XT>(x, xe + i * 8, xv);
    gn_ld8<DT>(dy, xe + i * 8, dv);
    gn_half8 h, l;
#pragma unroll
    for (int j = 0; j < 8; ++j) {
      float dz = dv[j];
      if (silu) dz *= silu_grad_f(kk[j].x * xv[j] + kk[j].y);
      const float xh = (xv[j] - gq[j].x) * gq[j].y;
      const float o = kk[j].z * dz - gq[j].z - xh * gq[j].w;
      acc[j] += (double)o;
      _Float16 th, tl;
      plane_pack(o, s, single, th, tl);
      h[j] = th; l[j] = tl;
    }
    *reinterpret_cast<gn_half8*>(hp + i * 8) = h;
    if (!single) *reinterpret_cast<gn_half8*>(lp + i * 8) = l;
  }
#pragma unroll
  for (int j = 0; j < 8; ++j) red[threadIdx.x][j] = acc[j];
  __syncthreads();
  if (threadIdx.x < C8) {
    for (int t = threadIdx.x + C8; t < 256; t += C8)
#pragma unroll
      for (int j = 0; j < 8; ++j) acc[j] += red[t][j];
    double* o = csp + ((int64_t)n * gridDim.x + blockIdx.x) * C + c0;
#pragma unroll
    for (int j = 0; j < 8; ++j) o[j] = acc[j];
  }
}

extern "C" size_t wdno_groupnorm_ws_bytes(int64_t N, int64_t S, int C, int G) {
  size_t part = (size_t)N * gn_chunks(S, N, C) * C * 2 * sizeof(double);
  return part + (size_t)N * C * 4 * sizeof(float) + (size_t)N * G * 4 * sizeof(float) + 64;
}
extern "C" size_t wdno_groupnorm_stats_floats(int64_t N, int C, int G) { return (size_t)N * G * 2 + (size_t)N * C * 4 + (size_t)N * G * 4; }
static inline float* gn_cb(float* stats, int64_t N, int G) { return stats + (size_t)N * G * 2; }
static inline float* gn_gb(float* stats, int64_t N, int C, int G) { return stats + (size_t)N * G * 2 + (size_t)N * C * 4; }
static inline unsigned gn_slices(int C, int G) { return C / G > 64 ? 1u : (unsigned)(G < 32 ? G : 32); }
static int gn_check(int64_t N, int64_t S, int C, int G) {
  if (N <= 0 || S <= 0 || C <= 0 || G <= 0 || N > 65535) return WDNO_EINVAL;
  if ((C & 3) || C > GN_MAXC || (C % G) != 0) return WDNO_EUNSUPPORTED;
  return WDNO_OK;
}
#define GN_PARTIAL0(XB, ...) do { if (XB) gn_partial_kernel<0, gn_bf16><<<__VA_ARGS__; else gn_partial_kernel<0, float><<<__VA_ARGS__; } while (0)
extern "C" int wdno_groupnorm_act_fwd_amax_t(const void* x, int x_bf16, const float* gamma, const float* beta, const float* ss, float* y,
                                      float* stats, float* amax_rec, int64_t N, int64_t S, int C, int G, float eps, int silu,
                                      void* ws, size_t ws_bytes, wdno_stream_t s) {
  int rc = gn_check(N, S, C, G);
  if (rc) return rc;
  if (ws_bytes < wdno_groupnorm_ws_bytes(N, S, C, G)) return WDNO_EWORKSPACE;
  const int nchunk = gn_chunks(S, N, C);
  double* part = (double*)ws;
  float* cb = gn_cb(stats, N, G);
  float* gb = gn_gb(stats, N, C, G);
  const int txp = pow2ceil(C / 4);
  const int64_t rpc = cdiv64(S, nchunk);
  hipStream_t st = as_stream(s);
  GN_PARTIAL0(x_bf16, dim3(nchunk, (unsigned)N), 256, 0, st>>>(x, nullptr, nullptr, nullptr, part, S, C, C / G, G, txp, rpc, 0));
  gn_finalize_kernel<<<dim3((unsigned)N, gn_slices(C, G)), 256, 0, st>>>(part, nullptr, gamma, beta, ss, stats, cb, gb, S, C, G, nchunk, eps);
  int gx = stream_grid(S * (C / 4), 256);
  if (gx > 512) gx = 512;
  if (x_bf16) gn_apply_kernel<gn_bf16><<<dim3(gx, (unsigned)N), 256, 0, st>>>(x, cb, y, S, C, silu, amax_rec);
  else gn_apply_kernel<float><<<dim3(gx, (unsigned)N), 256, 0, st>>>(x, cb, y, S, C, silu, amax_rec);
  return wdno_check_launch();
}
extern "C" int wdno_groupnorm_act_fwd_amax(const float* x, const float* gamma, const float* beta, const float* ss, float* y,
                                      float* stats, float* amax_rec, int64_t N, int64_t S, int C, int G, float eps, int silu,
                                      void* ws, size_t ws_bytes, wdno_stream_t s) {
  return wdno_groupnorm_act_fwd_amax_t(x, 0, gamma, beta, ss, y, stats, amax_rec, N, S, C, G, eps, silu, ws, ws_bytes, s);
}
extern "C" int wdno_groupnorm_act_fwd(const float* x, const float* gamma, const float* beta, const float* ss, float* y,
                                      float* stats, int64_t N, int64_t S, int C, int G, float eps, int silu,
                                      void* ws, size_t ws_bytes, wdno_stream_t s) {
  return wdno_groupnorm_act_fwd_amax(x, gamma, beta, ss, y, stats, nullptr, N, S, C, G, eps, silu, ws, ws_bytes, s);
}
extern "C" int wdno_groupnorm_act_bwd_amax(const float* x, const float* dy, const float* gamma, const float* beta, const float* ss,
                                      const float* stats, float* dx, float* dgb_partial, float* dss, float* amax_rec,
                                      int64_t N, int64_t S, int C, int G, int silu, void* ws, size_t ws_bytes, wdno_stream_t s) {
  int rc = gn_check(N, S, C, G);
  if (rc) return rc;
  if (ws_bytes < wdno_groupnorm_ws_bytes(N, S, C, G)) return WDNO_EWORKSPACE;
  const int nchunk = gn_chunks(S, N, C);
  double* part = (double*)ws;
  const float* cb = gn_cb(const_cast<float*>(stats), N, G);
  float* gb = gn_gb(const_cast<float*>(stats), N, C, G);
  const int txp = pow2ceil(C / 4);
  const int64_t rpc = cdiv64(S, nchunk);
  hipStream_t st = as_stream(s);
  gn_partial_kernel<1><<<dim3(nchunk, (unsigned)N), 256, 0, st>>>(x, dy, cb, gb, part, S, C, C / G, G, txp, rpc, silu);
  gn_bwd_finalize_kernel<<<dim3((unsigned)N, gn_slices(C, G)), 256, 0, st>>>(part, gamma, beta, ss, gb, dgb_partial, dss, S, C, G, nchunk);
  int gx = stream_grid(S * (C / 4), 256);
  if (gx > 512) gx = 512;
  gn_bwd_apply_kernel<<<dim3(gx, (unsigned)N), 256, 0, st>>>(x, dy, cb, gb, dx, S, C, C / G, G, silu, amax_rec);
  return wdno_check_launch();
}
extern "C" int wdno_groupnorm_act_bwd(const float* x, const float* dy, const float* gamma, const float* beta, const float* ss,
                                      const float* stats, float* dx, float* dgb_partial, float* dss,
                                      int64_t N, int64_t S, int C, int G, int silu, void* ws, size_t ws_bytes, wdno_stream_t s) {
  return wdno_groupnorm_act_bwd_amax(x, dy, gamma, beta, ss, stats, dx, dgb_partial, dss, nullptr, N, S, C, G, silu, ws, ws_bytes, s);
}


extern "C" size_t wdno_groupnorm_fwd_planes_ws_bytes(int64_t N, int64_t S, int C, int G) {
  return wdno_groupnorm_ws_bytes(N, S, C, G) + (size_t)N * gn_chunks(S, N, C) * 2 * sizeof(float) + 128;
}
extern "C" int wdno_groupnorm_act_fwd_planes_t(const void* x, int x_bf16, const float* gamma, const float* beta, const float* ss, void* y_hi, void* y_lo,
                                             float* y_scale, float* stats, float* bound_rec, int64_t N, int64_t S, int C, int G, float eps,
                                             int silu, void* ws, size_t ws_bytes, wdno_stream_t s) {
  int rc = gn_check(N, S, C, G);
  if (rc) return rc;
  const int C8 = C / 8;
  if ((C & 7) || C8 > 256 || (C8 & (C8 - 1))) return WDNO_EUNSUPPORTED;
  if (ws_bytes < wdno_groupnorm_fwd_planes_ws_bytes(N, S, C, G)) return WDNO_EWORKSPACE;
  const int nchunk = gn_chunks(S, N, C);
  double* part = (double*)ws;
  float* cb = gn_cb(stats, N, G);
  float* gb = gn_gb(stats, N, C, G);
  float* mx = (float*)((char*)ws + ((wdno_groupnorm_ws_bytes(N, S, C, G) + 63) & ~(size_t)63));
  const int txp = pow2ceil(C / 4);
  const int64_t rpc = cdiv64(S, nchunk);
  hipStream_t st = as_stream(s);
  GN_PARTIAL0(x_bf16, dim3(nchunk, (unsigned)N), 256, 0, st>>>(x, nullptr, nullptr, nullptr, part, S, C, C / G, G, txp, rpc, 0, y_lo ? mx : nullptr));
  gn_finalize_kernel<<<dim3((unsigned)N, gn_slices(C, G)), 256, 0, st>>>(part, nullptr, gamma, beta, ss, stats, cb, gb, S, C, G, nchunk, eps, mx, y_lo ? bound_rec : nullptr);
  int gx = stream_grid(S * (C / 8), 256);
  if (gx > 512) gx = 512;
  if (x_bf16) gn_apply_planes_kernel<gn_bf16><<<dim3(gx, (unsigned)N), 256, 0, st>>>(x, cb, (_Float16*)y_hi, (_Float16*)y_lo, y_scale, bound_rec, S, C, silu);
  else gn_apply_planes_kernel<float><<<dim3(gx, (unsigned)N), 256, 0, st>>>(x, cb, (_Float16*)y_hi, (_Float16*)y_lo, y_scale, bound_rec, S, C, silu);
  return wdno_check_launch();
}
extern "C" int wdno_groupnorm_act_fwd_planes(const float* x, const float* gamma, const float* beta, const float* ss, void* y_hi, void* y_lo,
                                             float* y_scale, float* stats, float* bound_rec, int64_t N, int64_t S, int C, int G, float eps,
                                             int silu, void* ws, size_t ws_bytes, wdno_stream_t s) {
  return wdno_groupnorm_act_fwd_planes_t(x, 0, gamma, beta, ss, y_hi, y_lo, y_scale, stats, bound_rec, N, S, C, G, eps, silu, ws, ws_bytes, s);
}

extern "C" int wdno_groupnorm_act_add_fwd_planes_t(const void* x, int x_bf16, const float* gamma, const float* beta, const float* ss, const float* residual,
                                                 const float* res_rec, float* y, void* y_hi, void* y_lo, float* y_scale, float* stats,
                                                 float* bound_rec, float* y_amax_rec, int64_t N, int64_t S, int C, int G, float eps, int silu,
                                                 void* ws, size_t ws_bytes, wdno_stream_t s) {
  int rc = gn_check(N, S, C, G);
  if (rc) return rc;
  const int C8 = C / 8;
  if ((C & 7) || C8 > 256 || (C8 & (C8 - 1))) return WDNO_EUNSUPPORTED;
  if (!residual || !y || (y_lo && (!y_hi || !res_rec || !bound_rec || !y_scale))) return WDNO_EINVAL;
  if (ws_bytes < wdno_groupnorm_fwd_planes_ws_bytes(N, S, C, G)) return WDNO_EWORKSPACE;
  const int nchunk = gn_chunks(S, N, C);
  double* part = (double*)ws;
  float* cb = gn_cb(stats, N, G);
  float* gb = gn_gb(stats, N, C, G);
  float* mx = (float*)((char*)ws + ((wdno_groupnorm_ws_bytes(N, S, C, G) + 63) & ~(size_t)63));
  const int txp = pow2ceil(C / 4);
  const int64_t rpc = cdiv64(S, nchunk);
  hipStream_t st = as_stream(s);
  GN_PARTIAL0(x_bf16, dim3(nchunk, (unsigned)N), 256, 0, st>>>(x, nullptr, nullptr, nullptr, part, S, C, C / G, G, txp, rpc, 0, y_lo ? mx : nullptr));
  gn_finalize_kernel<<<dim3((unsigned)N, gn_slices(C, G)), 256, 0, st>>>(part, nullptr, gamma, beta, ss, stats, cb, gb, S, C, G, nchunk, eps, mx, y_lo ? bound_rec : nullptr);
  int gx = stream_grid(S * (C / 8), 256);
  if (gx > 512) gx = 512;
  if (x_bf16) gn_apply_add_planes_kernel<gn_bf16><<<dim3(gx, (unsigned)N), 256, 0, st>>>(x, cb, residual, y, (_Float16*)y_hi, (_Float16*)y_lo, y_scale, bound_rec,
                                                                                       res_rec, y_amax_rec, S, C, silu);
  else gn_apply_add_planes_kernel<float><<<dim3(gx, (unsigned)N), 256, 0, st>>>(x, cb, residual, y, (_Float16*)y_hi, (_Float16*)y_lo, y_scale, bound_rec, res_rec,
                                                                           y_amax_rec, S, C, silu);
  return wdno_check_launch();
}
extern "C" int wdno_groupnorm_act_add_fwd_planes(const float* x, const float* gamma, const float* beta, const float* ss, const float* residual,
                                                 const float* res_rec, float* y, void* y_hi, void* y_lo, float* y_scale, float* stats,
                                                 float* bound_rec, float* y_amax_rec, int64_t N, int64_t S, int C, int G, float eps, int silu,
                                                 void* ws, size_t ws_bytes, wdno_stream_t s) {
  return wdno_groupnorm_act_add_fwd_planes_t(x, 0, gamma, beta, ss, residual, res_rec, y, y_hi, y_lo, y_scale, stats, bound_rec, y_amax_rec, N, S, C, G, eps, silu,
                                             ws, ws_bytes, s);
}

__global__ __launch_bounds__(PRS_THREADS) void gn_bwd_tail_kernel(const double* __restrict__ csp, float* __restrict__ dx_colsum, int nb, int C, int nbx,
                                                                     const float* __restrict__ dgb, float* __restrict__ dgb_sum, int N) {
  if ((int)blockIdx.x < nbx) {
    partial_rows_sum_body<double>(csp, dx_colsum, nb, C, (int)blockIdx.x);
    return;
  }
  partial_rows_sum_body<float>(dgb, dgb_sum, N, 2 * C, (int)blockIdx.x - nbx);
}

static inline int gn_planes_grid(int64_t N, int64_t S, int C) {
  int gx = stream_grid(S * (C / 8), 256);
  int cap = (int)(2048 / N);
  if (cap < 2) cap = 2;
  if (cap > 128) cap = 128;
  if (gx > cap) gx = cap;
  return gx;
}
extern "C" size_t wdno_groupnorm_bwd_planes_ws_bytes(int64_t N, int64_t S, int C, int G) {
  return wdno_groupnorm_ws_bytes(N, S, C, G) + (size_t)N * gn_chunks(S, N, C) * 2 * sizeof(float) + (size_t)N * 128 * C * sizeof(double) + 64;
}
extern "C" int wdno_groupnorm_bwd_planes_tail(int64_t N, int64_t S, int C, int G, size_t* csp_offset, int* rows) {
  int rc = gn_check(N, S, C, G);
  if (rc) return rc;
  WDNO_REQUIRE(csp_offset && rows);
  *csp_offset = (wdno_groupnorm_ws_bytes(N, S, C, G) + 63) & ~(size_t)63;
  *rows = (int)N * gn_planes_grid(N, S, C);
  return WDNO_OK;
}
extern "C" int wdno_groupnorm_act_bwd_planes_t(const void* x, int x_bf16, const void* dy, int dy_bf16, const float* gamma, const float* beta, const float* ss,
                                             const float* stats, void* dx_hi, void* dx_lo, float* dx_scale, float* dx_colsum,
                                             float* dgb_partial, float* dgb_sum, float* dss, float* bound_rec, int64_t N, int64_t S, int C, int G, int silu,
                                             void* ws, size_t ws_bytes, wdno_stream_t s) {
  int rc = gn_check(N, S, C, G);
  if (rc) return rc;
  const int C8 = C / 8;
  if ((C & 7) || C8 > 256 || (C8 & (C8 - 1))) return WDNO_EUNSUPPORTED;
  if (ws_bytes < wdno_groupnorm_bwd_planes_ws_bytes(N, S, C, G)) return WDNO_EWORKSPACE;
  const int nchunk = gn_chunks(S, N, C);
  double* part = (double*)ws;
  const float* cb = gn_cb(const_cast<float*>(stats), N, G);
  float* gb = gn_gb(const_cast<float*>(stats), N, C, G);
  char* tail = (char*)ws + ((wdno_groupnorm_ws_bytes(N, S, C, G) + 63) & ~(size_t)63);
  double* csp = (double*)tail;
  float* mx = (float*)(csp + (size_t)N * 128 * C);
  const int txp = pow2ceil(C / 4);
  const int64_t rpc = cdiv64(S, nchunk);
  hipStream_t st = as_stream(s);
#define GN_BWD_TYPES(KERNEL, ...) do { \
    if (x_bf16 && dy_bf16) KERNEL(gn_bf16, gn_bf16, __VA_ARGS__); else if (x_bf16) KERNEL(gn_bf16, float, __VA_ARGS__); \
    else if (dy_bf16) KERNEL(float, gn_bf16, __VA_ARGS__); else KERNEL(float, float, __VA_ARGS__); } while (0)
#define GN_K_PARTIAL1(XT, DT, ...) gn_partial_kernel<1, XT, DT><<<dim3(nchunk, (unsigned)N), 256, 0, st>>>(__VA_ARGS__)
#define GN_K_BWD_APPLY(XT, DT, ...) gn_bwd_apply_planes_kernel<XT, DT><<<dim3(gx, (unsigned)N), 256, 0, st>>>(__VA_ARGS__)
  GN_BWD_TYPES(GN_K_PARTIAL1, x, dy, cb, gb, part, S, C, C / G, G, txp, rpc, silu, dx_lo ? mx : nullptr);
  gn_bwd_finalize_kernel<<<dim3((unsigned)N, gn_slices(C, G)), 256, 0, st>>>(part, gamma, beta, ss, gb, dgb_partial, dss, S, C, G, nchunk, cb, mx, dx_lo ? bound_rec : nullptr);
  const int gx = gn_planes_grid(N, S, C);
  GN_BWD_TYPES(GN_K_BWD_APPLY, x, dy, cb, gb, (_Float16*)dx_hi, (_Float16*)dx_lo, dx_scale, bound_rec, csp, S, C, C / G, G, silu);
  const int nbx = dx_colsum ? cdiv(C, 32) : 0, nby = dgb_sum ? cdiv(2 * C, 32) : 0;
  if (nbx + nby) gn_bwd_tail_kernel<<<nbx + nby, PRS_THREADS, 0, st>>>(csp, dx_colsum, (int)N * gx, C, nbx, dgb_partial, dgb_sum, (int)N);
  return wdno_check_launch();
}

extern "C" int wdno_groupnorm_act_bwd_planes(const float* x, const float* dy, const float* gamma, const float* beta, const float* ss,
                                             const float* stats, void* dx_hi, void* dx_lo, float* dx_scale, float* dx_colsum,
                                             float* dgb_partial, float* dgb_sum, float* dss, float* bound_rec, int64_t N, int64_t S, int C, int G, int silu,
                                             void* ws, size_t ws_bytes, wdno_stream_t s) {
  return wdno_groupnorm_act_bwd_planes_t(x, 0, dy, 0, gamma, beta, ss, stats, dx_hi, dx_lo, dx_scale, dx_colsum, dgb_partial, dgb_sum, dss, bound_rec, N, S, C, G,
                                         silu, ws, ws_bytes, s);
}

template <int TPR, int VPL, bool BWD>
__global__ __launch_bounds__(256) void layernorm_kernel(const float* __restrict__ x, const float* __restrict__ g,
                                                         const float* __restrict__ dy, float* __restrict__ out,
                                                         float* __restrict__ dg_part, int64_t P, int C, float eps,
                                                         const float* __restrict__ add_to, float* __restrict__ dx_amax,
// ... 198 lines not shown
```

### wdno_amd/ops.py

```python
import contextlib
import ctypes as C
import math
import os

import torch

from . import _lib
from ._lib import AttnDesc, CondDesc, ConvGeom, DwtDesc

WEIGHT_EPOCH = 0
_pack_cache = {}


PROFILE = None


class _timed:

    def __init__(self, key, flops):
        self.key, self.flops = key, flops

    def __enter__(self):
        if PROFILE is not None:
            self.e0 = torch.cuda.Event(enable_timing=True)
# ... 315 lines not shown
        out = w.new_zeros((2, 2, 1, 2, cout_p, 2, cin_p))
        for py in range(2):
            for px in range(2):
                for dy in range(2):
                    for dx in range(2):
                        out[py, px, 0, dy, :cout, dx, :cin] = w[:, :, 0, 3 - py - 2 * dy, 3 - px - 2 * dx].t()
        return out
    return _cached(w_io, 't', cin_p, cout_p, build)


CONV_MATH = os.environ.get('WDNO_CONV_MATH', 'f16x3')
LOWP_AVAILABLE = True


def _lp():
    return CONV_MATH == 'bf16'


@contextlib.contextmanager
def _math(mode):
    global CONV_MATH
    prev, CONV_MATH = CONV_MATH, mode
    try:
        yield
    finally:
        CONV_MATH = prev
H3_MIN_PIXELS = 1024
PATCH_DGRAD_H3 = True
H3_MIN_REDUCTION = 64


def pad8(c):
    return (c + 7) // 8 * 8


_amax_pool = {}
AMAX_FLOATS = 64 * 16
AMAX_HINTS = True


PLANES_FWD = True
GRAD_PLANES = True
_CAPTURE = None


@contextlib.contextmanager
def graph_capture(graph, stream=None):
    global _CAPTURE
    assert _CAPTURE is None, 'nested graph captures are not supported'
    with torch.cuda.graph(graph, stream=stream, capture_error_mode='thread_local'):
        _CAPTURE = [None, 0]
        try:
            yield graph
        finally:
            _CAPTURE = None


def _amax_slot(device):
    if _CAPTURE is not None:
        st = _CAPTURE
        if st[0] is None or st[1] >= st[0].shape[0]:
            st[0], st[1] = torch.zeros((1024, AMAX_FLOATS), device=device, dtype=torch.float32), 0
        rec = st[0][st[1]]
        st[1] += 1
        return rec
    key = str(device)
    st = _amax_pool.get(key)
    if st is None or st[1] >= st[0].shape[0]:
        st = [torch.zeros((1024, AMAX_FLOATS), device=device, dtype=torch.float32), 0]
        _amax_pool[key] = st
    rec = st[0][st[1]]
    st[1] += 1
    return rec


def _new_amax_record(device):
    return _amax_slot(device) if AMAX_HINTS and not _lp() else None


def _leave_amax(t, rec):
    if rec is not None:
        t._wdno_amax = (rec, t._version)
    return t


def _known_amax(t):
    h = getattr(t, '_wdno_amax', None)
    return h[0] if h is not None and h[1] == t._version and AMAX_HINTS else None


def tensor_amax(x):
    amax = _amax_slot(x.device)
    _lib.check(_lib_().wdno_amax_record(_p(x), x.numel(), _p(amax), _stream()), 'amax')
    return amax


def split_f16_of(t, x2d, amax=None, c8=None):
    h = getattr(t, '_wdno_planes', None)
    if (h is not None and h[1] == t._version and h[0][0].shape[0] == x2d.shape[0] and h[2] == CONV_MATH
            and (c8 is None or h[0][0].shape[1] == c8)):
        return h[0]
    planes = split_f16(x2d, amax, c8)
    try:
        t._wdno_planes = (planes, t._version, CONV_MATH)
    except Exception:
        pass
    return planes


def split_f16(x2d, amax=None, c8=None):
    rows, c = x2d.shape
    if c8 is None or _lp():
        c8 = pad8(c)
    lib = _lib_()
    if _lp():
        hi = torch.empty((rows, c8), device=x2d.device, dtype=torch.float16)
        _lib.check(lib.wdno_cast_bf16(_p(x2d), _p(hi), rows, c, c8, _stream()), 'cast_bf16')
        return hi, None, None
    if amax is None:
        amax = tensor_amax(x2d)
    hi = torch.empty((rows, c8), device=x2d.device, dtype=torch.float16)
    lo = torch.empty((rows, c8), device=x2d.device, dtype=torch.float16)
    scale = amax[1:2]
    _lib.check(lib.wdno_split_f16(_p(x2d), _p(amax), _p(hi), _p(lo), _p(scale), rows, c, c8, _stream()), 'split_f16')
    return hi, lo, scale


def split_f16_colsum(x2d, amax=None, bias=None, k=None):
    rows, c = x2d.shape
    c8 = pad8(c)
    g8 = c8 // 8
    if g8 > 256 or (g8 & (g8 - 1)):
        return split_f16(x2d, amax), colsum(x2d)
    lib = _lib_()
    nb = lib.wdno_split_colsum_ws_bytes(rows, c8)
    ws = _ws(nb, x2d.device)
    flat = None
    if bias is not None and DEFER_ROW_SUMS and _WGRAD_PENDING is not None:
        flat = _flat_grad_out(bias, (k,))
    cs = None if flat is not None else torch.empty(c8, device=x2d.device, dtype=torch.float32)
    if _lp():
        hi = torch.empty((rows, c8), device=x2d.device, dtype=torch.float16)
        _lib.check(lib.wdno_cast_bf16_colsum(_p(x2d), _p(hi), _p(cs), _p(ws), nb, rows, c, c8, _stream()), 'cast_bf16_colsum')
        planes = (hi, None, None)
    else:
        if amax is None:
            amax = tensor_amax(x2d)
        hi = torch.empty((rows, c8), device=x2d.device, dtype=torch.float16)
        lo = torch.empty((rows, c8), device=x2d.device, dtype=torch.float16)
        scale = amax[1:2]
        _lib.check(lib.wdno_split_f16_colsum(_p(x2d), _p(amax), _p(hi), _p(lo), _p(scale), _p(cs), _p(ws), nb, rows, c, c8, _stream()), 'split_f16_colsum')
        planes = (hi, lo, scale)
    if flat is not None:
        return planes, rows_sum_for_param(_RowsJob(ws, ws.data_ptr(), nb // (8 * c8), c8, 0, k, 1), bias, out=flat)
    return planes, cs[:c]


class _WPlan:
    __slots__ = ('w', 'wd', 'kind', 'cp8', 'kp', 'hi', 'lo', 'sc', 'ver', 'used', 'lp')


def _wmode(kind):
    if kind[0] == 'q':
        return 6 + 2 * int(kind[1]) + int(kind[2])
    if kind[0] == 'a':
        return 10 if kind == 'aq' else 11
# ... 83 lines not shown
    return [pl for pl in _wplans.values() if since is None or pl.used >= since]


def touch_plans(plans):
    e = WEIGHT_EPOCH
    for pl in plans:
        pl.used = e


def prepare_graph_refresh():
    epoch = WEIGHT_EPOCH
    for pl in _wplans.values():
        if pl.used >= epoch - 3:
            pl.used = epoch
    bump_weight_epoch(params=False)
    if _wplans:
        for lp in {pl.lp for pl in _wplans.values()}:
            _refresh_weight_plans(WEIGHT_EPOCH, lp)
    bump_weight_epoch(params=False)


def split_weight(w, kind, cp8, kp, pack=None):
    lp = _lp()
    key = (w.data_ptr(), kind, cp8, kp, tuple(w.shape), tuple(w.stride()), lp)
    ver = (w._version, WEIGHT_EPOCH)
    pl = _wplans.get(key)
    if pl is not None:
        if pl.ver != ver:
            _refresh_weight_plans(WEIGHT_EPOCH)
        if pl.ver == ver:
            pl.used = WEIGHT_EPOCH
            return pl.hi, pl.lo, pl.sc
    with torch.no_grad():
        wd = w.detach()
        wc = wd if wd.is_contiguous() else wd.contiguous()
        amax = None
        if not lp:
            amax = torch.zeros(1, device=w.device, dtype=torch.float32)
            _lib.check(_lib_().wdno_amax(_p(wc), wc.numel(), _p(amax), _stream()), 'amax')
        k, c, kd, kh, kw = _wdims(kind, _as5(wc))
        rows = kd * kh * kp * kw
        if pl is None:
            pl = _WPlan()
            pl.w, pl.wd, pl.kind, pl.cp8, pl.kp, pl.lp = wd, wd, kind, cp8, kp, lp
            pl.hi = torch.empty((rows, cp8), device=w.device, dtype=torch.float16)
            pl.lo = None if lp else torch.empty((rows, cp8), device=w.device, dtype=torch.float16)
            pl.sc = None if lp else torch.empty(1, device=w.device, dtype=torch.float32)
            if len(_wplans) > 4096:
                _wplans.clear(); _wtables.clear()
                bump_weight_epoch(params=False)
                ver = (w._version, WEIGHT_EPOCH)
            _wplans[key] = pl
        _lib.check(_lib_().wdno_pack_split_weight(_p(wc), _p(amax), _p(pl.hi), _p(pl.lo), _p(pl.sc), k, c, kd, kh, kw, kp, cp8,
                                                  _wmode(kind), _stream()), 'pack_split_weight')
    pl.ver = ver
    pl.used = WEIGHT_EPOCH
    return pl.hi, pl.lo, pl.sc


ACT16 = os.environ.get('WDNO_ACT16', '0') == '1'
ZERO_BOX = True


class _ZeroBox(C.Structure):
    _fields_ = [('channels', C.c_int), ('d0', C.c_int), ('h0', C.c_int), ('w0', C.c_int)]


def set_zero_box(t, box):
    t._wdno_zero_box = (tuple(int(v) for v in box), t._version)
    return t


def zero_box_of(t):
    h = getattr(t, '_wdno_zero_box', None)
    return h[0] if h is not None and h[1] == t._version and ZERO_BOX else None


def carry_zero_box(dst, src):
    box = zero_box_of(src)
    return set_zero_box(dst, box) if box is not None else dst


def conv_fwd_h3(planes, shape4, w, pack, kind, bias_p, residual, ks, st, pd, kp, out=None, osp=None, ostride=(1, 1, 1), ooff=(0, 0, 0),
                amax_rec=None, zero_box=None, out16=False):
    xh, xl, sx = planes
    n, d, h, ww = shape4
    cp8 = xh.shape[-1]
    wh, wl, sw = split_weight(w, kind, cp8, kp, pack)
    if osp is None:
        osp = tuple(_out_size(a, k, s_, p_) for a, k, s_, p_ in zip((d, h, ww), ks, st, pd))
    out16 = bool(out16 and xl is None and out is None and residual is None)
    if out is None:
        y = torch.empty((n, *osp, kp), device=xh.device, dtype=torch.bfloat16 if out16 else torch.float32)
        g = _geom((n, d, h, ww), cp8, kp, ks, st, pd, osp)
    else:
        y = out
        g = _geom((n, d, h, ww), cp8, kp, ks, st, pd, osp, y_sp=tuple(out.shape[1:4]), ostride=ostride, ooff=ooff)
    flops = 2.0 * n * osp[0] * osp[1] * osp[2] * kp * ks[0] * ks[1] * ks[2] * cp8
    tap = (out is None and tuple(st) == (1, 1, 1) and tuple(osp) == (d, h, ww) and max(ks) <= 8 and
           ((ks[2] == 3 and cp8 % 32 == 0) or (ks[2] == 7 and cp8 % 16 == 0 and kp <= 64)))
    with _timed(_fwd_h3_kernel_name(n * osp[0] * osp[1] * osp[2], kp, ks, tap, cp8 if xl is not None else None), flops):
        zb = None
        if zero_box is not None and tap and ks[2] == 7:
            zb = _ZeroBox(*zero_box)
        if xl is None:
            if zb is not None or out16:
                _lib.check(_lib_().wdno_conv_fwd_bf16_ex(_p(xh), _p(wh), _p(bias_p), _p(residual), _p(y), int(out16), _p(amax_rec), C.byref(g),
                                                         None if zb is None else C.byref(zb), _stream()), 'conv_fwd_bf16_ex')
                return y
            _lib.check(_lib_().wdno_conv_fwd_bf16(_p(xh), _p(wh), _p(bias_p), _p(residual), _p(y), _p(amax_rec), C.byref(g), _stream()), 'conv_fwd_bf16')
            return y
        if zb is not None:
            _lib.check(_lib_().wdno_conv_fwd_f16x3_zbox(_p(xh), _p(xl), _p(sx), _p(wh), _p(wl), _p(sw), _p(bias_p), _p(residual), _p(y),
                                                        _p(amax_rec), C.byref(g), C.byref(zb), _stream()), 'conv_fwd_f16x3_zbox')
            return y
        key = (n, d, h, ww, cp8, kp, tuple(ks), tuple(osp)) if tap and ks[2] == 3 else None
        wsb = 0
        if key is not None:
            wsb = _split_ws_bytes.get(key)
            if wsb is None:
                wsb = _split_ws_bytes[key] = int(_lib_().wdno_conv_fwd_split_ws_bytes(C.byref(g)))
        if wsb:
            ws = torch.empty(wsb // 4, device=xh.device, dtype=torch.float32)
            _lib.check(_lib_().wdno_conv_fwd_f16x3_ws(_p(xh), _p(xl), _p(sx), _p(wh), _p(wl), _p(sw), _p(bias_p), _p(residual), _p(y),
                                                      _p(amax_rec), C.byref(g), _p(ws), wsb, _stream()), 'conv_fwd_f16x3_ws')
            return y
        _lib.check(_lib_().wdno_conv_fwd_f16x3_amax(_p(xh), _p(xl), _p(sx), _p(wh), _p(wl), _p(sw), _p(bias_p), _p(residual), _p(y),
                                                    _p(amax_rec), C.byref(g), _stream()), 'conv_fwd_f16x3')
    return y


_split_ws_bytes = {}


_pixel_tables = {}


def _fwd_h3_kernel_name(pixels, k, ks, tap=False, c=None):
    cdiv = lambda a, b: -(-a // b)
    tiles = cdiv(pixels, 128) * cdiv(k, 128) if k > 64 else cdiv(pixels, 256)
    small_tap = tap and ks[2] == 3 and cdiv(pixels, 64) * cdiv(k, 64) >= 64
    if (tiles >= 100 or small_tap) and max(ks) <= 8:
        cus = 256
        cost = lambda bm, bn, wgt: cdiv(cdiv(pixels, bm) * cdiv(k, bn), cus) * bm * bn * wgt
        shapes = [(256, 64, 1.04), (192, 64, 1.08)] if k <= 64 else [(128, 128, 1.0), (192, 128, 1.0), (256, 64, 1.04), (192, 64, 1.08)]
        best = shapes[0]
        for sh in shapes[1:]:
            if cost(*sh) < cost(*best):
                best = sh
        if tap and ks[2] == 3:
            c_best = cost(*best)
            if k > 64 and cost(160, 128, 1.02) < c_best:
                best, c_best = (160, 128, 1.02), cost(160, 128, 1.02)
            if cost(320, 64, 1.05) < c_best:
                best, c_best = (320, 64, 1.05), cost(320, 64, 1.05)
            if cost(128, 64, 1.15) < c_best:
                best, c_best = (128, 64, 1.15), cost(128, 64, 1.15)
            if cost(64, 64, 1.35) < c_best:
                best = (64, 64, 1.35)
            if best[:2] == (64, 64) and c is not None and c % 32 == 0 and k >= 128:
                t128, nst = cdiv(pixels, 128) * cdiv(k, 128), ks[0] * ks[1] * (c // 32)
                if t128 * 4 <= cus and nst % 4 == 0 and nst // 4 >= 8:
                    return 'conv_fwd_h3t_kernel<128,128>/4'
        if tap and _lp() and k > 64 and cdiv(pixels, 256) * cdiv(k, 128) >= 2 * cus:
            best = (256, 128)
        if tap and ks[2] == 7:
            best = (256, 64)
            if not _lp() and cdiv(pixels, 256) < cus and cdiv(pixels, 256) < cdiv(pixels, 192) <= cus:
                best = (192, 64)
        return f'conv_fwd_h3{"t" if tap else "d"}_kernel<{best[0]},{best[1]}>'
    return 'conv_fwd_h3_kernel<..,128>' if k > 64 else 'conv_fwd_h3_kernel<..,64>'


def _wgrad_h3_kernel_name(k, run, window=False):
    if window == 'stem':
        return 'conv_wgrad_h3s_kernel<64,352>'
    if window:
        return 'conv_wgrad_h3w_kernel<64,384>'
    cdiv = lambda a, b: -(-a // b)
    bn = 192 if cdiv(run, 192) * 192 <= cdiv(run, 128) * 128 else 128
    return f'conv_wgrad_h3d_kernel<{128 if k > 64 else 64},{bn}>'


FLAT_WGRAD = True
_FLAT_ARMED = False
DEFER_WGRAD_REDUCE = True
_WGRAD_PENDING = None
WGRAD_FLUSH_BYTES = int(os.environ.get('WDNO_WGRAD_FLUSH_MB', '0')) << 20
DEFER_ROW_SUMS = True
_ROWSUM_PENDING = []
_DEFERRED_DSTS = set()


def flush_wgrad_reduces():
    global _WGRAD_PENDING, _ROWSUM_PENDING
    pend, rows = _WGRAD_PENDING, _ROWSUM_PENDING
    if rows:
        _ROWSUM_PENDING = []
        ritems = (_lib.RowsSumItem * len(rows))(*[it for it, _ in rows])
        _lib.check(_lib_().wdno_rows_sum_multi(C.cast(ritems, C.c_void_p), len(rows), _stream()), 'rows_sum_multi')
        _DEFERRED_DSTS.update(int(it.out) for it, _ in rows)
    if not pend:
        return
    _WGRAD_PENDING = [] if _FLAT_ARMED else None
# ... 224 lines not shown
        gb = torch.empty((k,), device=x.device, dtype=torch.float32) if has_bias else None
        _lib.check(lib.wdno_linear_rows_wgrad(_p(x), cp, _p(gy), kp, _p(gw), _p(gb), rows, c, k, _stream()), 'linear_rows_wgrad')
        gw = gw.reshape(weight.shape)
        if not ctx.needs_input_grad[1]:
            gw = None
        if not (has_bias and ctx.needs_input_grad[2]):
            gb = None
    return gx, gw, gb, None, None, None


class _Conv(torch.autograd.Function):

    @staticmethod
    def forward(ctx, x, weight, bias, residual, stride, padding, with_skip=False, grad_planes=False, to_norm=False):
        ctx.with_skip = with_skip
        ctx.to_norm = to_norm and grad_planes
        ctx.bias_ref = bias
        y = _Conv._forward(ctx, x, weight, bias, residual, stride, padding)
        if grad_planes and not ctx.rows and ctx.h3 and y.dim() in (4, 5) and residual is None:
            ks, st = ctx.meta[0], ctx.meta[1]
            n_, d_, h_, w_, _ = ctx.xshape
            if not ctx.needs_input_grad[0] or (st == (1, 1, 1) and _use_h3(n_ * d_ * h_ * w_, ctx.meta[6] * ks[0] * ks[1] * ks[2])):
                y._wdno_grad_planes = True
        if with_skip:
            return y, _alias_of(x)
        return y

    @staticmethod
    def _forward(ctx, x, weight, bias, residual, stride, padding):
        xrec = _known_amax(x)
        x_in = x
        ctx.x16 = x.dtype == torch.bfloat16
        if ctx.x16:
            if not (getattr(x, '_wdno_unwritten', False) and x.is_cuda):
                raise RuntimeError('wdno_amd: a bf16 tensor that is not a planes-only placeholder reached a convolution')
            x = x if x.is_contiguous() else x.contiguous()
        else:
            x = _chk(x, 'x')
        lead = None
        if x.dim() != 5:
            lead = x.shape[:-1]
            x5 = x.reshape(1, 1, 1, -1, x.shape[-1]) if x.dim() != 4 else x.unsqueeze(1)
        else:
            x5 = x
        w5 = _as5(weight)
        k, c = w5.shape[0], w5.shape[1]
        cp, kp = x5.shape[-1], pad4(k)
        assert cp == pad4(c), f'channel mismatch: tensor has {cp}, weight expects {c}'
        ks = tuple(w5.shape[2:])
        if x.dim() == 2 and x.shape[0] <= LINEAR_ROWS_MAX and weight.dim() == 2 and residual is None and c % 4 == 0 and k % 4 == 0:
            wc = weight.detach()
            wc = wc if wc.is_contiguous() else wc.contiguous()
            rows = x.shape[0]
            y = torch.empty((rows, kp), device=x.device, dtype=torch.float32)
            _lib.check(_lib_().wdno_linear_rows_fwd(_p(x), cp, _p(wc), c, _p(None if bias is None else bias.detach()), _p(y), rows, c, k, kp,
                                                    _stream()), 'linear_rows_fwd')
            ctx.save_for_backward(x, weight)
            ctx.h3 = False
            ctx.rows = True
            ctx.meta = (ks, stride, padding, k, c, cp, kp, bias is not None, False, lead, 2)
            return y
        ctx.rows = False
        with torch.no_grad():
            bias_p = _pad_vec(bias.detach() if bias is not None else None, kp)
        res5 = None
        if residual is not None:
            residual = _chk(residual, 'residual')
            res5 = residual
        osp_ = tuple(_out_size(a, kk, s_, p_) for a, kk, s_, p_ in zip(x5.shape[1:4], ks, stride, padding))
        h3 = _use_h3(x5.shape[0] * osp_[0] * osp_[1] * osp_[2], cp * ks[0] * ks[1] * ks[2])
        if getattr(x_in, '_wdno_unwritten', False):
            hp = getattr(x_in, '_wdno_planes', None)
            if not (h3 and hp is not None and hp[1] == x_in._version and hp[2] == CONV_MATH):
                raise RuntimeError('wdno_amd: a planes-only tensor reached a convolution that reads fp32')
        if h3:
            c8w = pad8(cp) + 8 if (ks[2] == 7 and kp <= 64 and tuple(stride) == (1, 1, 1) and pad8(cp) % 16) else None
            planes = split_f16_of(x_in, x5.reshape(-1, cp), xrec, c8w)
            yrec = _new_amax_record(x5.device)
            nx_, dx_, hx_, wx_ = x5.shape[:4]
            out16 = (ACT16 and _lp() and getattr(ctx, 'to_norm', False) and GRAD_PLANES and residual is None and x.dim() in (4, 5) and kp % 8 == 0
                     and kp // 8 <= 256 and (kp // 8) & (kp // 8 - 1) == 0
                     and (not ctx.needs_input_grad[0] or (tuple(stride) == (1, 1, 1) and _use_h3(nx_ * dx_ * hx_ * wx_, kp * ks[0] * ks[1] * ks[2]))))
            y = _leave_amax(conv_fwd_h3(planes, tuple(x5.shape[:4]), weight, pack_fwd, 'f', bias_p, res5, ks, stride, padding, kp,
                                        amax_rec=yrec, zero_box=zero_box_of(x_in) if x_in.dim() == 5 else None, out16=out16), yrec)
            ctx.save_for_backward(planes[0], planes[1], planes[2], weight)
        else:
            y = conv_fwd_raw(x5, pack_fwd(weight, cp, kp), bias_p, res5, ks, stride, padding, kp)
            ctx.save_for_backward(x5, weight)
        ctx.h3 = h3
        ctx.xshape = tuple(x5.shape)
        ctx.meta = (ks, stride, padding, k, c, cp, kp, bias is not None, residual is not None, lead, x.dim())
        if lead is not None:
            y = y.reshape(*lead, kp) if x.dim() != 4 else y.squeeze(1)
        return y

    @staticmethod
    def backward(ctx, gy, gskip=None):
        if ctx.rows:
            return _linear_rows_backward(ctx, gy) + (None, None, None)
        return _Conv._backward(ctx, gy, gskip) + (None, None, None)

    @staticmethod
    def _backward(ctx, gy, gskip):
        if ctx.h3:
            xh, xl, sx, weight = ctx.saved_tensors
            x5 = None
        else:
            x5, weight = ctx.saved_tensors
        ks, stride, padding, k, c, cp, kp, has_bias, has_res, lead, xdim = ctx.meta
        grec = _known_amax(gy)
        po = getattr(gy, '_wdno_planes_only', None)
        if po is not None and gy.dtype == torch.bfloat16:
            gy = gy if gy.is_contiguous() else gy.contiguous()
        else:
            gy = _chk(gy, 'grad')
        n, d, h, w, _ = ctx.xshape
        gyplanes = None
        gb_given = None
        if po is not None:
            if not (ctx.h3 and po[2] == gy._version and po[3] == CONV_MATH and not has_res):
                raise RuntimeError('wdno_amd: a planes-only gradient reached a convolution that cannot take it')
            gyplanes, gb_given = po[0], po[1]
        osp = tuple(_out_size(a, kk, s, p) for a, kk, s, p in zip((d, h, w), ks, stride, padding))
        gy5 = gy.reshape(n, *osp, kp)
        gx = gw = gb = gr = None
        want_gb = has_bias and ctx.needs_input_grad[2]
        will_split = (ctx.needs_input_grad[1] and ctx.h3) or (ctx.needs_input_grad[0] and stride == (1, 1, 1)
                                                              and _use_h3(n * d * h * w, kp * ks[0] * ks[1] * ks[2]))
        if po is not None:
            if not (will_split and (not ctx.needs_input_grad[0] or (stride == (1, 1, 1) and _use_h3(n * d * h * w, kp * ks[0] * ks[1] * ks[2])))):
                raise RuntimeError('wdno_amd: a planes-only gradient reached a convolution whose backward needs fp32 dy')
            if want_gb:
                gb = rows_sum_for_param(gb_given, getattr(ctx, 'bias_ref', None), k) if isinstance(gb_given, _RowsJob) else gb_given[:k].contiguous()
        elif want_gb and will_split:
            gyplanes, gbs = split_f16_colsum(gy5.reshape(-1, kp), grec, bias=getattr(ctx, 'bias_ref', None), k=k)
            gb = gbs[:k].contiguous()
        if ctx.needs_input_grad[0]:
            gs5 = None if gskip is None else _chk(gskip, 'skip gradient').reshape(n, d, h, w, cp)
            if stride == (1, 1, 1):
                pd = tuple(kk - 1 - p for kk, p in zip(ks, padding))
                if _use_h3(n * d * h * w, kp * ks[0] * ks[1] * ks[2]):
                    if gyplanes is None:
                        gyplanes = split_f16(gy5.reshape(-1, kp), grec)
                    drec = _new_amax_record(gy5.device)
                    gx5 = _leave_amax(conv_fwd_h3(gyplanes, tuple(gy5.shape[:4]), weight, lambda w_, c8_, k_: pack_dgrad(w_, k_, c8_), 'd', None, gs5,
                                                  ks, (1, 1, 1), pd, cp, amax_rec=drec, out16=getattr(ctx, 'x16', False) and gs5 is None), drec)
                else:
                    wd = pack_dgrad(weight, cp, kp)
                    gx5 = conv_fwd_raw(gy5, wd, None, gs5, ks, (1, 1, 1), pd, cp)
                gs5 = None
            elif ks == (1, 4, 4) and stride == (1, 2, 2) and padding == (0, 1, 1):
                oh_, ow_ = gy5.shape[2], gy5.shape[3]
                if ctx.h3 and _use_h3(n * d * oh_ * ow_, kp * 4) and _as5(weight).is_contiguous():
                    if gyplanes is None:
                        gyplanes = split_f16(gy5.reshape(-1, kp), grec)
                    drec = _new_amax_record(gy5.device)
                    gx5 = _leave_amax(conv_transpose_h3(gyplanes, tuple(gy5.shape[:4]), _as5(weight), None, cp, amax_rec=drec), drec)
                else:
                    wt = pack_transposed(_as5(weight), kp, cp)
                    gx5 = conv_transpose_raw(gy5, wt, None, cp)
            elif ks == (1, 2, 2) and stride == (1, 2, 2) and padding == (0, 0, 0):
                if ctx.h3 and _use_h3(n * d * gy5.shape[2] * gy5.shape[3], kp) and _as5(weight).is_contiguous() and PATCH_DGRAD_H3:
                    if gyplanes is None:
                        gyplanes = split_f16(gy5.reshape(-1, kp), grec)
                    drec = _new_amax_record(gy5.device)
                    gx5 = _leave_amax(_patch2_dgrad(gy5, weight, cp, kp, gyplanes, drec), drec)
                else:
                    gx5 = _patch2_dgrad(gy5, weight, cp, kp)
            else:
                raise RuntimeError(f'wdno_amd: unsupported convolution geometry for dgrad {ks} {stride} {padding}')
            if gs5 is not None:
                gx5 = gx5 + gs5
            if getattr(ctx, 'x16', False) and gx5.dtype != torch.bfloat16:
                gx5 = gx5.to(torch.bfloat16)
            gx = gx5
            if lead is not None:
# ... 148 lines not shown
            o = ybuf[p * start:p * (start + k)].view(p, k)
            o._wdno_grad_slot = gbuf[p * start:p * (start + k)].view(p, k)
            outs.append(o)
        ctx.save_for_backward(x, *[w for w in weights])
        ctx.meta = (tab, ks, f, p, c, [b is not None for b in biases])
        ctx.gbuf = gbuf
        return tuple(outs)

    @staticmethod
    def backward(ctx, *gys):
        x = ctx.saved_tensors[0]
        tab, ks, f, p, c, has_bias = ctx.meta
        gbuf = ctx.gbuf
        for (k, start), g in zip(ks, gys):
            slot = gbuf[p * start:p * (start + k)].view(p, k)
            if g is None:
                slot.zero_()
            elif g.data_ptr() != slot.data_ptr() or not g.is_contiguous():
                slot.copy_(g)
        lib = _lib_()
        n = len(ks)
        gx = None
        if ctx.needs_input_grad[0]:
            gx = torch.empty((p, c), device=x.device, dtype=torch.float32)
            nb = lib.wdno_linear_multi_dgrad_ws_bytes(f, p, c)
            ws = _ws(nb, x.device)
            _lib.check(lib.wdno_linear_multi_dgrad(_p(tab), n, f, _p(gbuf), _p(gx), p, c, _p(ws), nb, _stream()), 'linear_multi_dgrad')
        gw = torch.empty((f, c), device=x.device, dtype=torch.float32)
        gb = torch.empty((f,), device=x.device, dtype=torch.float32)
        _lib.check(lib.wdno_linear_multi_wgrad(_p(tab), n, f, _p(x), _p(gbuf), _p(gw), _p(gb), p, c, _stream()), 'linear_multi_wgrad')
        gws = tuple(gw[start:start + k] if ctx.needs_input_grad[2 + i] else None for i, (k, start) in enumerate(ks))
        gbs = tuple(gb[start:start + k] if hb and ctx.needs_input_grad[2 + n + i] else None for i, ((k, start), hb) in enumerate(zip(ks, has_bias)))
        return (gx, None) + gws + gbs


def linear_multi(x, layers):
    if not layers or x.dim() != 2 or x.shape[0] > LINEAR_MULTI_ROWS_MAX or x.shape[1] % 4 or x.shape[1] > 512 or x.dtype != torch.float32:
        return None
    ws = [l.weight for l in layers]
    if any(w.dim() != 2 or w.shape[1] != x.shape[1] or w.shape[0] % 4 or not w.is_contiguous() or w.dtype != torch.float32 for w in ws):
        return None
    bs = [l.bias for l in layers]
    return list(_LinearMulti.apply(x, len(ws), *ws, *bs))


def conv_transpose_h3(xplanes, shape4, weight, bias_p, cout_p, amax_rec=None):
    n, d, h, w = shape4
    y = torch.empty((n, d, 2 * h, 2 * w, cout_p), device=xplanes[0].device, dtype=torch.float32)
    for py in range(2):
        for px in range(2):
            conv_fwd_h3(xplanes, shape4, weight, pack_fwd, f'p{py}{px}', bias_p, None, (1, 2, 2), (1, 1, 1), (0, 1 - py, 1 - px),
                        cout_p, out=y, osp=(d, h, w), ostride=(1, 2, 2), ooff=(0, py, px), amax_rec=amax_rec)
    return y


def conv_transpose_cl(x, weight, bias=None):
    return _ConvT.apply(x, weight, bias)


def _claim_grad_slot(t):
    slot = getattr(t, '_wdno_grad_slot', None)
    if slot is not None:
        try:
            del t._wdno_grad_slot
        except AttributeError:
            pass
    return slot


class _GroupNormAct(torch.autograd.Function):
    @staticmethod
    def forward(ctx, x, gamma, beta, ss, groups, act_silu, eps, out_planes=False):
        x_in = x
        x = _chk_act(x, 'x')
        x16 = int(x.dtype == torch.bfloat16)
        n, c = x.shape[0], x.shape[-1]
        s = x.numel() // (n * c)
        lib = _lib_()
        nb = lib.wdno_groupnorm_ws_bytes(n, s, c, groups)
        ws = _ws(nb, x.device)
        stats = torch.empty((lib.wdno_groupnorm_stats_floats(n, c, groups),), device=x.device, dtype=torch.float32)
        ssc = None if ss is None else _chk(ss, 'scale_shift')
        ctx.ss_slot = _claim_grad_slot(ss) if ssc is ss else None
        c8_ = c // 8
        if out_planes and CONV_MATH in ('f16x3', 'bf16') and c % 8 == 0 and c8_ <= 256 and (c8_ & (c8_ - 1)) == 0:
            nbp = lib.wdno_groupnorm_fwd_planes_ws_bytes(n, s, c, groups)
            wsp = _ws(nbp, x.device)
            hi = torch.empty((n * s, c), device=x.device, dtype=torch.float16)
            lo = brec = scale = None
            if not _lp():
                lo = torch.empty((n * s, c), device=x.device, dtype=torch.float16)
                brec = _amax_slot(x.device)
                scale = brec[1:2]
            _lib.check(lib.wdno_groupnorm_act_fwd_planes_t(_p(x), x16, _p(gamma), _p(beta), _p(ssc), _p(hi), _p(lo), _p(scale), _p(stats), _p(brec),
                                                           n, s, c, groups, float(eps), int(act_silu), _p(wsp), nbp, _stream()), 'groupnorm_fwd_planes')
            ctx.save_for_backward(x, gamma, beta, ssc, stats)
            ctx.meta = (n, s, c, groups, int(act_silu))
            ctx.epoch = _param_epoch(gamma)
            ctx.grad_planes = GRAD_PLANES and getattr(x_in, '_wdno_grad_planes', False)
            y = torch.empty(x.shape, device=x.device, dtype=torch.bfloat16 if (x16 or (ACT16 and _lp())) else torch.float32)
            return _planes_only(y, (hi, lo, scale))
        y = torch.empty(x.shape, device=x.device, dtype=torch.float32)
        rec = _new_amax_record(x.device)
        _lib.check(lib.wdno_groupnorm_act_fwd_amax_t(_p(x), x16, _p(gamma), _p(beta), _p(ssc), _p(y), _p(stats), _p(rec), n, s, c, groups,
                                                     float(eps), int(act_silu), _p(ws), nb, _stream()), 'groupnorm_fwd')
        ctx.save_for_backward(x, gamma, beta, ssc, stats)
        ctx.meta = (n, s, c, groups, int(act_silu))
        ctx.epoch = _param_epoch(gamma)
        c8 = c // 8
        ctx.grad_planes = (GRAD_PLANES and getattr(x_in, '_wdno_grad_planes', False) and CONV_MATH in ('f16x3', 'bf16') and c % 8 == 0
                           and c8 <= 256 and (c8 & (c8 - 1)) == 0)
        return _leave_amax(y, rec)

    @staticmethod
    def backward(ctx, gy):
        x, gamma, beta, ss, stats = ctx.saved_tensors
        n, s, c, groups, act_silu = ctx.meta
        if getattr(ctx, 'epoch', None) not in (None, _param_epoch(gamma)):
            raise RuntimeError('wdno_amd GroupNorm backward: the parameters were updated (optimiser step / checkpoint load) between this forward and its backward')
        gy = _chk_act(gy, 'grad')
        x16, dy16 = int(x.dtype == torch.bfloat16), int(gy.dtype == torch.bfloat16)
        lib = _lib_()
        dgb = torch.empty((n, 2, c), device=x.device, dtype=torch.float32)
        dss = None if ss is None else (ctx.ss_slot if getattr(ctx, 'ss_slot', None) is not None else torch.empty_like(ss))
        if ctx.grad_planes and CONV_MATH in ('f16x3', 'bf16'):
            nb = lib.wdno_groupnorm_bwd_planes_ws_bytes(n, s, c, groups)
            ws = _ws(nb, x.device)
            hi = torch.empty((n * s, c), device=x.device, dtype=torch.float16)
            cs = torch.empty((c,), device=x.device, dtype=torch.float32)
            lo = rec = scale = None
            if not _lp():
                lo = torch.empty((n * s, c), device=x.device, dtype=torch.float16)
                rec = _amax_slot(x.device)
                scale = rec[1:2]
            og = ob = None
            if DEFER_ROW_SUMS and _WGRAD_PENDING is not None and n > 1:
                og = _flat_grad_out(gamma, (c,))
                ob = _flat_grad_out(beta, (c,)) if og is not None else None
                if og is not None and ob is None:
                    gamma._wdno_flat_busy = False
                    og = None
            if og is not None:
                off, prow = C.c_size_t(0), C.c_int(0)
                _lib.check(lib.wdno_groupnorm_bwd_planes_tail(n, s, c, groups, C.byref(off), C.byref(prow)), 'groupnorm_bwd_planes_tail')
                _lib.check(lib.wdno_groupnorm_act_bwd_planes_t(_p(x), x16, _p(gy), dy16, _p(gamma), _p(beta), _p(ss), _p(stats), _p(hi), _p(lo), _p(scale), None,
                                                               _p(dgb), None, _p(dss), _p(rec), n, s, c, groups, act_silu, _p(ws), nb, _stream()),
                           'groupnorm_bwd_planes')
                dx = _poison(torch.empty_like(x))
                dx._wdno_planes_only = ((hi, lo, scale), _RowsJob(ws, ws.data_ptr() + off.value, prow.value, c, 0, c, 1), dx._version, CONV_MATH)
                dgam = rows_sum_for_param(_RowsJob(dgb, dgb.data_ptr(), n, 2 * c, 0, c, 0), gamma, out=og)
                dbet = rows_sum_for_param(_RowsJob(dgb, dgb.data_ptr(), n, 2 * c, c, c, 0), beta, out=ob)
                return dx, dgam, dbet, dss, None, None, None, None
            red = torch.empty((2 * c,), device=x.device, dtype=torch.float32) if n > 1 else None
            _lib.check(lib.wdno_groupnorm_act_bwd_planes_t(_p(x), x16, _p(gy), dy16, _p(gamma), _p(beta), _p(ss), _p(stats), _p(hi), _p(lo), _p(scale), _p(cs),
                                                           _p(dgb), _p(red), _p(dss), _p(rec), n, s, c, groups, act_silu, _p(ws), nb, _stream()),
                       'groupnorm_bwd_planes')
            dx = _poison(torch.empty_like(x))
            dx._wdno_planes_only = ((hi, lo, scale), cs, dx._version, CONV_MATH)
            if red is None:
                red = dgb.reshape(2 * c)
            return dx, red[:c].contiguous(), red[c:].contiguous(), dss, None, None, None, None
        if x16 or dy16:
            raise RuntimeError('wdno_amd GroupNorm backward: bf16-stored activations reach the norm only together with the planes hand-over of dx '
                               '(ops.GRAD_PLANES / CONV_MATH changed between forward and backward?)')
        nb = lib.wdno_groupnorm_ws_bytes(n, s, c, groups)
        ws = _ws(nb, x.device)
        dx = torch.empty_like(x)
        rec = _new_amax_record(x.device)
        _lib.check(lib.wdno_groupnorm_act_bwd_amax(_p(x), _p(gy), _p(gamma), _p(beta), _p(ss), _p(stats), _p(dx), _p(dgb), _p(dss), _p(rec),
                                                   n, s, c, groups, act_silu, _p(ws), nb, _stream()), 'groupnorm_bwd')
        red = colsum(dgb.reshape(n, 2 * c)) if n > 1 else dgb.reshape(2 * c)
        return _leave_amax(dx, rec), red[:c].contiguous(), red[c:].contiguous(), dss, None, None, None, None


class _GroupNormActAdd(torch.autograd.Function):
    @staticmethod
    def forward(ctx, x, gamma, beta, ss, residual, groups, act_silu, eps):
        x_in = x
        x = _chk_act(x, 'x')
        x16 = int(x.dtype == torch.bfloat16)
        res = _chk(residual, 'residual')
        n, c = x.shape[0], x.shape[-1]
        s = x.numel() // (n * c)
        lib = _lib_()
        nb = lib.wdno_groupnorm_fwd_planes_ws_bytes(n, s, c, groups)
        ws = _ws(nb, x.device)
        y = torch.empty(x.shape, device=x.device, dtype=torch.float32)
        stats = torch.empty((lib.wdno_groupnorm_stats_floats(n, c, groups),), device=x.device, dtype=torch.float32)
        ssc = None if ss is None else _chk(ss, 'scale_shift')
        ctx.ss_slot = _claim_grad_slot(ss) if ssc is ss else None
        yrec = _new_amax_record(x.device)
        _lib.check(lib.wdno_groupnorm_act_add_fwd_planes_t(_p(x), x16, _p(gamma), _p(beta), _p(ssc), _p(res), None, _p(y), None, None, None, _p(stats),
                                                         None, _p(yrec), n, s, c, groups, float(eps), int(act_silu), _p(ws), nb, _stream()),
                   'groupnorm_add_fwd')
        ctx.save_for_backward(x, gamma, beta, ssc, stats)
        ctx.meta = (n, s, c, groups, int(act_silu))
        ctx.epoch = _param_epoch(gamma)
        c8 = c // 8
        ctx.grad_planes = (GRAD_PLANES and getattr(x_in, '_wdno_grad_planes', False) and CONV_MATH in ('f16x3', 'bf16') and c % 8 == 0
                           and c8 <= 256 and (c8 & (c8 - 1)) == 0)
        return _leave_amax(y, yrec)

    @staticmethod
    def backward(ctx, gy):
        r = _GroupNormAct.backward(ctx, gy)
        return r[0], r[1], r[2], r[3], gy, None, None, None


def groupnorm_act_add(x, gamma, beta, groups, residual, scale_shift=None, act=True, eps=1e-5):
    c = x.shape[-1]
    c8 = c // 8
    if not (c % 8 == 0 and c8 <= 256 and (c8 & (c8 - 1)) == 0 and x.shape == residual.shape):
        return add(groupnorm_act(x, gamma, beta, groups, scale_shift, act, eps), residual)
    return _GroupNormActAdd.apply(x, gamma, beta, scale_shift, residual, groups, act, eps)


def groupnorm_act(x, gamma, beta, groups, scale_shift=None, act=True, eps=1e-5, out_planes=False):
    return _GroupNormAct.apply(x, gamma, beta, scale_shift, groups, act, eps, out_planes)


def _alias_of(x):
    xs = x.view_as(x)
    for attr in ('_wdno_amax', '_wdno_planes', '_wdno_unwritten'):
        h = getattr(x, attr, None)
        if h is not None:
            try:
                setattr(xs, attr, h)
            except Exception:
                pass
    return xs


class _LayerNorm(torch.autograd.Function):
    @staticmethod
    def forward(ctx, x, g, eps, with_skip, out_planes=False):
        x_in = x
        x = _chk(x, 'x')
        c = x.shape[-1]
        p = x.numel() // c
        y = torch.empty_like(x)
        gf = g.reshape(-1)
        if out_planes and CONV_MATH in ('f16x3', 'bf16') and c % 8 == 0:
            hi = torch.empty((p, c), device=x.device, dtype=torch.float16)
            lo = scale = None
            if not _lp():
                lo = torch.empty((p, c), device=x.device, dtype=torch.float16)
                scale = torch.empty((1,), device=x.device, dtype=torch.float32)
            _lib.check(_lib_().wdno_layernorm_fwd_planes(_p(x), _p(gf), _p(hi), _p(lo), _p(scale), p, c, float(eps), _stream()), 'layernorm_fwd_planes')
            ctx.save_for_backward(x, g)
            ctx.eps = eps
            y = _planes_only(y, (hi, lo, scale))
            return (y, _alias_of(x_in)) if with_skip else y
        rec = _new_amax_record(x.device)
        _lib.check(_lib_().wdno_layernorm_fwd_amax(_p(x), _p(gf), _p(y), _p(rec), p, c, float(eps), _stream()), 'layernorm_fwd')
        ctx.save_for_backward(x, g)
        ctx.eps = eps
        if with_skip:
            return _leave_amax(y, rec), _alias_of(x_in)
        return _leave_amax(y, rec)

    @staticmethod
    def backward(ctx, gy, gskip=None):
        x, g = ctx.saved_tensors
        gy = _chk(gy, 'grad')
        c = x.shape[-1]
        p = x.numel() // c
        lib = _lib_()
        nb = lib.wdno_layernorm_bwd_ws_bytes(p, c)
        ws = _ws(nb, x.device)
        dx = torch.empty_like(x)
        dg = torch.empty((c,), device=x.device, dtype=torch.float32)
        add_to = None if gskip is None else _chk(gskip, 'skip gradient')
        rec = _new_amax_record(x.device)
        _lib.check(lib.wdno_layernorm_bwd_add_amax(_p(x), _p(g.reshape(-1)), _p(gy), _p(add_to), _p(dx), _p(dg), _p(rec), p, c, float(ctx.eps),
                                                   _p(ws), nb, _stream()), 'layernorm_bwd')
        return _leave_amax(dx, rec), dg.reshape(g.shape), None, None, None

# ... 418 lines not shown
```

Measured before the change: 33.77.

## Compute GroupNorm statistics in conv epilogue to skip separate stats pass

The k=3 tap convolution epilogue (and its split-K reduce kernel) now emits per-32-row, per-8-channel partial sums and sums of squares in double precision, plus per-block amax, into a side record. Subsequent GroupNorm forward kernels read these records instead of re-reading the conv output to compute mean and variance. This removes one full read pass over the activation for each conv followed by a GroupNorm. The cost is extra epilogue work (double-precision DPP/permlane reductions) and record buffers. A fallback path is kept for shapes that do not qualify.

```diff
diff --git a/include/wdno_hip.h b/include/wdno_hip.h
--- a/include/wdno_hip.h
+++ b/include/wdno_hip.h
@@ -94,6 +94,10 @@
                            const float* bias, const float* residual, float* y, float* amax_rec, const wdno_conv_geom* g,
                            void* ws, size_t ws_bytes, wdno_stream_t s);
 size_t wdno_conv_fwd_split_ws_bytes(const wdno_conv_geom* g);
+size_t wdno_conv_gn_rec_bytes(const wdno_conv_geom* g);
+int wdno_conv_fwd_f16x3_gn(const void* xh, const void* xl, const float* sx, const void* wph, const void* wpl, const float* sw,
+                           const float* bias, const float* residual, float* y, float* amax_rec, const wdno_conv_geom* g,
+                           void* ws, size_t ws_bytes, void* gn_rec, size_t gn_rec_bytes, int* gn_taken, wdno_stream_t s);
 size_t wdno_conv_wgrad_f16x3_ws_bytes(const wdno_conv_geom* g);
 int wdno_conv_pixel_table(void* table, const wdno_conv_geom* g, wdno_stream_t s);
 int wdno_conv_wgrad_f16x3(const void* xh, const void* xl, const float* sx, const void* dyh, const void* dyl, const float* sdy,
@@ -175,6 +179,16 @@
                                     const float* stats, void* dx_hi, void* dx_lo, float* dx_scale, float* dx_colsum,
                                     float* dgb_partial, float* dgb_sum, float* dss, float* bound_rec, int64_t N, int64_t S, int C, int G, int silu,
                                     void* ws, size_t ws_bytes, wdno_stream_t s);
+int wdno_groupnorm_act_fwd_amax_rec(const float* x, const void* conv_rec, const float* gamma, const float* beta, const float* ss, float* y,
+                                    float* stats, float* amax_rec, int64_t N, int64_t S, int C, int G, float eps, int silu,
+                                    void* ws, size_t ws_bytes, wdno_stream_t s);
+int wdno_groupnorm_act_fwd_planes_rec(const float* x, const void* conv_rec, const float* gamma, const float* beta, const float* ss, void* y_hi, void* y_lo,
+                                      float* y_scale, float* stats, float* bound_rec, int64_t N, int64_t S, int C, int G, float eps,
+                                      int silu, void* ws, size_t ws_bytes, wdno_stream_t s);
+int wdno_groupnorm_act_add_fwd_planes_rec(const float* x, const void* conv_rec, const float* gamma, const float* beta, const float* ss, const float* residual,
+                                          const float* res_rec, float* y, void* y_hi, void* y_lo, float* y_scale, float* stats,
+                                          float* bound_rec, float* y_amax_rec, int64_t N, int64_t S, int C, int G, float eps, int silu,
+                                          void* ws, size_t ws_bytes, wdno_stream_t s);
 int wdno_layernorm_fwd(const float* x, const float* g, float* y, int64_t P, int C, float eps, wdno_stream_t s);
 int wdno_layernorm_fwd_amax(const float* x, const float* g, float* y, float* amax_rec, int64_t P, int C, float eps, wdno_stream_t s);
 int wdno_layernorm_fwd_planes(const float* x, const float* g, void* y_hi, void* y_lo, float* y_scale, int64_t P, int C, float eps,
diff --git a/wdno_amd/_lib.py b/wdno_amd/_lib.py
--- a/wdno_amd/_lib.py
+++ b/wdno_amd/_lib.py
@@ -103,6 +103,8 @@
     'wdno_conv_fwd_f16x3_amax': (I, [P, P, P, P, P, P, P, P, P, P, PG, P]),
     'wdno_conv_fwd_f16x3_ws': (I, [P, P, P, P, P, P, P, P, P, P, PG, P, Z, P]),
     'wdno_conv_fwd_split_ws_bytes': (Z, [PG]),
+    'wdno_conv_gn_rec_bytes': (Z, [PG]),
+    'wdno_conv_fwd_f16x3_gn': (I, [P, P, P, P, P, P, P, P, P, P, PG, P, Z, P, Z, C.POINTER(I), P]),
     'wdno_conv_wgrad_f16x3_ws_bytes': (Z, [PG]),
     'wdno_conv_pixel_table': (I, [P, PG, P]),
     'wdno_conv_wgrad_f16x3': (I, [P, P, P, P, P, P, P, P, P, Z, PG, P]),
@@ -136,6 +138,9 @@
     'wdno_groupnorm_act_fwd_amax_t': (I, [P, I, P, P, P, P, P, P, L, L, I, I, F, I, P, Z, P]),
     'wdno_groupnorm_act_fwd_planes_t': (I, [P, I, P, P, P, P, P, P, P, P, L, L, I, I, F, I, P, Z, P]),
     'wdno_groupnorm_act_add_fwd_planes_t': (I, [P, I, P, P, P, P, P, P, P, P, P, P, P, P, L, L, I, I, F, I, P, Z, P]),
+    'wdno_groupnorm_act_fwd_amax_rec': (I, [P, P, P, P, P, P, P, P, L, L, I, I, F, I, P, Z, P]),
+    'wdno_groupnorm_act_fwd_planes_rec': (I, [P, P, P, P, P, P, P, P, P, P, L, L, I, I, F, I, P, Z, P]),
+    'wdno_groupnorm_act_add_fwd_planes_rec': (I, [P, P, P, P, P, P, P, P, P, P, P, P, P, P, L, L, I, I, F, I, P, Z, P]),
     'wdno_groupnorm_act_bwd_planes_t': (I, [P, I, P, I, P, P, P, P, P, P, P, P, P, P, P, P, L, L, I, I, I, P, Z, P]),
     'wdno_layernorm_fwd': (I, [P, P, P, L, I, F, P]),
     'wdno_layernorm_fwd_amax': (I, [P, P, P, P, L, I, F, P]),
diff --git a/wdno_amd/csrc/conv_common.h b/wdno_amd/csrc/conv_common.h
--- a/wdno_amd/csrc/conv_common.h
+++ b/wdno_amd/csrc/conv_common.h
@@ -23,7 +23,12 @@
   size_t split_ws_bytes;
   int zb_blocks, zb_d, zb_h;
   int out_bf16;
+  double* gn_sums;
+  float* gn_max;
+  int gn_taken;
 };
+static inline size_t gn_rec_sums_bytes(int64_t P, int K) { return (size_t)((P + 31) / 32) * (size_t)(K / 8) * 2 * sizeof(double); }
+static inline size_t gn_rec_bytes(int64_t P, int K) { return gn_rec_sums_bytes(P, K) + (size_t)((P + 31) / 32) * (size_t)((K + 31) / 32) * sizeof(float); }
 
 __device__ __forceinline__ int xcd_swizzle(int bid, int nwg) {
   int q = nwg >> 3, r = nwg & 7;
@@ -67,6 +72,50 @@
   const auto sy = __builtin_amdgcn_permlane32_swap(A.y, B.y, false, false);
   return make_uint4(sx[0], sy[0], sx[1], sy[1]);
 }
+#define DPP_XOR1 0xB1
+#define DPP_XOR2 0x4E
+#define DPP_HALF_MIRROR 0x141
+#define DPP_MIRROR 0x140
+#define DPP_ROR8 0x128
+template <int CTRL> __device__ __forceinline__ float dpp_f32(float v) {
+  return __builtin_bit_cast(float, __builtin_amdgcn_update_dpp(0, __builtin_bit_cast(int, v), CTRL, 0xf, 0xf, false));
+}
+template <int CTRL> __device__ __forceinline__ double dpp_f64(double v) {
+  const uint64_t u = __builtin_bit_cast(uint64_t, v);
+  const unsigned lo = (unsigned)__builtin_amdgcn_update_dpp(0, (int)(unsigned)u, CTRL, 0xf, 0xf, false);
+  const unsigned hi = (unsigned)__builtin_amdgcn_update_dpp(0, (int)(unsigned)(u >> 32), CTRL, 0xf, 0xf, false);
+  return __builtin_bit_cast(double, ((uint64_t)hi << 32) | lo);
+}
+__device__ __forceinline__ float wave_max_dpp(float v) {
+  v = fmaxf(v, dpp_f32<DPP_XOR1>(v));
+  v = fmaxf(v, dpp_f32<DPP_XOR2>(v));
+  v = fmaxf(v, dpp_f32<DPP_HALF_MIRROR>(v));
+  v = fmaxf(v, dpp_f32<DPP_MIRROR>(v));
+  const int i = __builtin_bit_cast(int, v);
+  return fmaxf(fmaxf(__builtin_bit_cast(float, __builtin_amdgcn_readlane(i, 0)), __builtin_bit_cast(float, __builtin_amdgcn_readlane(i, 16))),
+               fmaxf(__builtin_bit_cast(float, __builtin_amdgcn_readlane(i, 32)), __builtin_bit_cast(float, __builtin_amdgcn_readlane(i, 48))));
+}
+template <bool W32> __device__ __forceinline__ double swap_add_f64(double a, double b) {
+  const uint64_t ua = __builtin_bit_cast(uint64_t, a), ub = __builtin_bit_cast(uint64_t, b);
+  const auto lo = W32 ? __builtin_amdgcn_permlane32_swap((unsigned)ua, (unsigned)ub, false, false)
+                      : __builtin_amdgcn_permlane16_swap((unsigned)ua, (unsigned)ub, false, false);
+  const auto hi = W32 ? __builtin_amdgcn_permlane32_swap((unsigned)(ua >> 32), (unsigned)(ub >> 32), false, false)
+                      : __builtin_amdgcn_permlane16_swap((unsigned)(ua >> 32), (unsigned)(ub >> 32), false, false);
+  return __builtin_bit_cast(double, ((uint64_t)hi[0] << 32) | lo[0]) + __builtin_bit_cast(double, ((uint64_t)hi[1] << 32) | lo[1]);
+}
+__device__ __forceinline__ double wave_sum8_f64(const double (&d)[8], int lane) {
+  double r[4], t[2];
+#pragma unroll
+  for (int i = 0; i < 4; ++i) r[i] = swap_add_f64<true>(d[i], d[4 + i]);
+#pragma unroll
+  for (int i = 0; i < 2; ++i) t[i] = swap_add_f64<false>(r[i], r[2 + i]);
+  const bool up = (lane & 8) != 0;
+  double v = (up ? t[1] : t[0]) + dpp_f64<DPP_ROR8>(up ? t[0] : t[1]);
+  v += dpp_f64<DPP_XOR1>(v);
+  v += dpp_f64<DPP_XOR2>(v);
+  v += dpp_f64<DPP_HALF_MIRROR>(v);
+  return v;
+}
 __device__ __forceinline__ void lgkm0_barrier() {
   __builtin_amdgcn_s_waitcnt(0xc07f);
   asm volatile("s_barrier" : : : "memory");
@@ -81,6 +130,7 @@
   p.split_ws_bytes = 0;
   p.zb_blocks = 0; p.zb_d = 0; p.zb_h = 0;
   p.out_bf16 = 0;
+  p.gn_sums = nullptr; p.gn_max = nullptr; p.gn_taken = 0;
   p.debug = wdno_debug_mode;
   p.R = g->kw * g->C;
   p.nchunk = cdiv(p.R, BK);
diff --git a/wdno_amd/csrc/conv_h3.hip b/wdno_amd/csrc/conv_h3.hip
--- a/wdno_amd/csrc/conv_h3.hip
+++ b/wdno_amd/csrc/conv_h3.hip
@@ -498,7 +498,9 @@
 template <bool LP>
 static int conv_fwd_16(const void* xh, const void* xl, const float* sx, const void* wph, const void* wpl, const float* sw,
                        const float* bias, const float* residual, float* y, float* amax_rec, const wdno_conv_geom* g, wdno_stream_t s,
-                       float* split_ws = nullptr, size_t split_ws_bytes = 0, const wdno_zero_box* zb = nullptr, int y_bf16 = 0) {
+                       float* split_ws = nullptr, size_t split_ws_bytes = 0, const wdno_zero_box* zb = nullptr, int y_bf16 = 0,
+                       void* gn_rec = nullptr, size_t gn_rec_bytes = 0, int* gn_taken = nullptr) {
+  if (gn_taken) *gn_taken = 0;
   int rc = check_geom(g);
   if (rc) return rc;
   if (g->C & 7) return WDNO_EUNSUPPORTED;
@@ -513,6 +515,10 @@
   p.amax_rec = amax_rec;
   p.split_ws = split_ws;
   p.split_ws_bytes = split_ws_bytes;
+  if (gn_rec && !LP && gn_rec_bytes && gn_rec_bytes >= wdno_conv_gn_rec_bytes(g) && wdno_conv_gn_rec_bytes(g)) {
+    p.gn_sums = (double*)gn_rec;
+    p.gn_max = (float*)((char*)gn_rec + gn_rec_sums_bytes(p.P, g->K));
+  }
   p.nchunk = cdiv(p.R, HBK);
   p.nsteps = g->kd * g->kh * p.nchunk;
   hipStream_t st = as_stream(s);
@@ -521,8 +527,9 @@
   auto blocks = [&](int bm, int bn) { return cdiv64(P, bm) * cdiv(K, bn); };
   const int dbg = wdno_debug_mode;
   const bool small_tap = p.identity_out && wdno_conv_h3t_takes(*g) && g->kw == 3 && blocks(64, 64) >= 64;
-  if (dbg != WDNO_DBG_ROW_ATTN_AND_REG_STAGED_CONV && (dbg == WDNO_DBG_FORCE_DMA_CONV || dbg == WDNO_DBG_CHUNKED_DMA_CONV || dbg == WDNO_DBG_FORCE_TILES_160 || dbg == WDNO_DBG_FORCE_TILES_320 || small_tap || (K > 64 ? blocks(128, 128) : blocks(256, 64)) >= 100)) {
+  if (dbg != WDNO_DBG_ROW_ATTN_AND_REG_STAGED_CONV && (dbg == WDNO_DBG_FORCE_DMA_CONV || dbg == WDNO_DBG_CHUNKED_DMA_CONV || dbg == WDNO_DBG_FORCE_TILES_160 || dbg == WDNO_DBG_FORCE_TILES_320 || dbg == WDNO_DBG_GN_SEPARATE_STATS || small_tap || (K > 64 ? blocks(128, 128) : blocks(256, 64)) >= 100)) {
     rc = wdno_conv_fwd_h3_dma(xh, LP ? nullptr : xl, wph, LP ? nullptr : wpl, sx, sw, bias, residual, y, p, st, 3);
+    if (rc == WDNO_OK && gn_taken) *gn_taken = p.gn_taken;
     if (rc == WDNO_OK) return wdno_check_launch();
     if (rc != WDNO_EUNSUPPORTED) return rc;
   }
@@ -558,6 +565,19 @@
 extern "C" int wdno_conv_fwd_bf16_ex(const void* x16, const void* wp16, const float* bias, const float* residual, void* y, int y_bf16, float* amax_rec,
                                      const wdno_conv_geom* g, const wdno_zero_box* zb, wdno_stream_t s) {
   return conv_fwd_16<true>(x16, x16, nullptr, wp16, wp16, nullptr, bias, residual, (float*)y, amax_rec, g, s, nullptr, 0, zb, y_bf16);
+}
+extern "C" size_t wdno_conv_gn_rec_bytes(const wdno_conv_geom* g) {
+  if (!g || check_geom(g) || (g->C & 7) || (g->K & 7) || g->kw != 3 || wdno_debug_mode == WDNO_DBG_GN_SEPARATE_STATS) return 0;
+  ConvP p;
+  fill_params(p, g);
+  if (!p.identity_out || !wdno_conv_h3t_takes(*g) || ((((int64_t)g->OD * g->OH * g->OW) & 31) && g->N != 1)) return 0;
+  return gn_rec_bytes(p.P, g->K);
+}
+extern "C" int wdno_conv_fwd_f16x3_gn(const void* xh, const void* xl, const float* sx, const void* wph, const void* wpl, const float* sw,
+                                      const float* bias, const float* residual, float* y, float* amax_rec, const wdno_conv_geom* g,
+                                      void* ws, size_t ws_bytes, void* gn_rec, size_t gn_rec_bytes, int* gn_taken, wdno_stream_t s) {
+  return conv_fwd_16<false>(xh, xl, sx, wph, wpl, sw, bias, residual, y, amax_rec, g, s, (float*)ws, ws ? ws_bytes : 0, nullptr, 0, gn_rec, gn_rec_bytes,
+                            gn_taken);
 }
 extern "C" size_t wdno_conv_fwd_split_ws_bytes(const wdno_conv_geom* g) {
   if (!g || check_geom(g) || (g->C & 7)) return 0;
diff --git a/wdno_amd/csrc/conv_h3t.hip b/wdno_amd/csrc/conv_h3t.hip
--- a/wdno_amd/csrc/conv_h3t.hip
+++ b/wdno_amd/csrc/conv_h3t.hip
@@ -91,6 +91,7 @@
   const bool padded = (NSUB & 1) && ((g.kd * g.kh * ncb) & 1);
   const int nstages = g.kd * g.kh * ncb / nruns + (padded ? 1 : 0);
   constexpr bool SKIP = KW == 7 && !SP;
+  constexpr bool GST = KW == 3 && !SP;
   const int nzb = SKIP ? p.zb_blocks : 0;
   const bool skipping = SKIP && p.zb_blocks >= 0 && p.debug != WDNO_DBG_STEM_EVERY_STAGE;
   auto tile_live = [&](int t) {
@@ -402,7 +403,8 @@
 #pragma unroll
     for (int a = 0; a < TM; ++a) {
       const int64_t pm = m0 + m_base + a * 32 + li;
-      if (pm >= p.P) continue;
+      const bool live = pm < p.P;
+      if (!live && !(GST && p.gn_sums != nullptr && m0 + m_base + a * 32 < p.P)) continue;
       const int64_t yr = pm;
       if constexpr (SP) {
         float* wrow = p.split_ws + ((int64_t)run * p.P + pm) * g.K;
@@ -441,18 +443,36 @@
         }
         continue;
       }
+      const bool gst = GST && p.gn_sums != nullptr;
+      const int64_t sub = (m0 + m_base + a * 32) >> 5;
+      const int r8 = g.K >> 3, r32 = (g.K + 31) >> 5;
 #pragma unroll
       for (int b = 0; b < TN; ++b) {
+        double gd[8] = {0, 0, 0, 0, 0, 0, 0, 0};
+        float gm = 0.f;
 #pragma unroll
         for (int e4 = 0; e4 < 4; ++e4) {
           const int kc = n0 + n_base + b * 32 + 8 * e4 + 4 * hh;
-          if (kc < g.K) {
+          if (live && kc < g.K) {
             float4 v = make_float4(acc[a][b][4 * e4] * inv, acc[a][b][4 * e4 + 1] * inv, acc[a][b][4 * e4 + 2] * inv, acc[a][b][4 * e4 + 3] * inv);
             if (bias) { const float4 tb = *reinterpret_cast<const float4*>(bias + kc); v.x += tb.x; v.y += tb.y; v.z += tb.z; v.w += tb.w; }
             if (rrow) { const float4 tr = *reinterpret_cast<const float4*>(rrow + kc); v.x += tr.x; v.y += tr.y; v.z += tr.z; v.w += tr.w; }
             *reinterpret_cast<float4*>(yrow + kc) = v;
-            am = amax4(am, v);
+            if (gst) {
+              const double x0 = v.x, x1 = v.y, x2 = v.z, x3 = v.w;
+              gd[2 * e4] = (x0 + x1) + (x2 + x3);
+              gd[2 * e4 + 1] = (x0 * x0 + x1 * x1) + (x2 * x2 + x3 * x3);
+              gm = amax4(gm, v);
+            } else am = amax4(am, v);
           }
+        }
+        if (gst) {
+          const int cb = (n0 + n_base) / 32 + b;
+          const double tot = wave_sum8_f64(gd, lane);
+          if ((lane & 7) == 0 && cb * 4 + (lane >> 4) < r8) p.gn_sums[(sub * r8 + cb * 4) * 2 + (lane >> 3)] = tot;
+          am = fmaxf(am, gm);
+          gm = wave_max_dpp(gm);
+          if (lane == 0 && cb < r32) p.gn_max[sub * r32 + cb] = gm;
         }
       }
     }
@@ -464,17 +484,47 @@
 
 __global__ __launch_bounds__(256) void conv_split_reduce_kernel(const float4* __restrict__ ws, int nruns, int64_t n4, int K4, const float* __restrict__ sx,
                                                                  const float* __restrict__ sw, const float4* __restrict__ bias, const float4* res,
-                                                                 float4* y, float* __restrict__ amax_rec) {
+                                                                 float4* y, float* __restrict__ amax_rec, double* __restrict__ gn_sums,
+                                                                 float* __restrict__ gn_max) {
   const float inv = sx ? 1.0f / (sx[0] * sw[0]) : 1.0f;
   float am = 0.f;
-  for (int64_t i = (int64_t)blockIdx.x * 256 + threadIdx.x; i < n4; i += (int64_t)gridDim.x * 256) {
+  auto value = [&](int64_t i, int k4) {
     float4 v = ws[i];
     for (int r = 1; r < nruns; ++r) { const float4 u = ws[(int64_t)r * n4 + i]; v.x += u.x; v.y += u.y; v.z += u.z; v.w += u.w; }
     v.x *= inv; v.y *= inv; v.z *= inv; v.w *= inv;
-    if (bias) { const float4 tb = bias[(int)(i % K4)]; v.x += tb.x; v.y += tb.y; v.z += tb.z; v.w += tb.w; }
+    if (bias) { const float4 tb = bias[k4]; v.x += tb.x; v.y += tb.y; v.z += tb.z; v.w += tb.w; }
     if (res) { const float4 tr = res[i]; v.x += tr.x; v.y += tr.y; v.z += tr.z; v.w += tr.w; }
     y[i] = v;
-    am = amax4(am, v);
+    return v;
+  };
+  if (gn_sums) {
+    const int lane = threadIdx.x & 63, r32 = K4 >> 3;
+    const int64_t P = n4 / K4, items = ((P + 31) / 32) * r32, nwaves = (int64_t)gridDim.x * 4;
+    for (int64_t it = (int64_t)blockIdx.x * 4 + (threadIdx.x >> 6); it < items; it += nwaves) {
+      const int64_t sub = it / r32;
+      const int cb = (int)(it - sub * r32);
+      const int k4 = cb * 8 + (lane & 7);
+      double s = 0, q = 0;
+      float gm = 0.f;
+#pragma unroll
+      for (int j = 0; j < 4; ++j) {
+        const int64_t row = sub * 32 + j * 8 + (lane >> 3);
+        if (row >= P) continue;
+        const float4 v = value(row * K4 + k4, k4);
+        const double x0 = v.x, x1 = v.y, x2 = v.z, x3 = v.w;
+        s += (x0 + x1) + (x2 + x3);
+        q += (x0 * x0 + x1 * x1) + (x2 * x2 + x3 * x3);
+        gm = amax4(gm, v);
+      }
+#pragma unroll
+      for (int o = 1; o < 64; o = o == 1 ? 8 : o * 2) { s += __shfl_xor(s, o, 64); q += __shfl_xor(q, o, 64); }
+      if ((lane & 0x39) == 0) { double* o = gn_sums + ((sub * r32 + cb) * 4 + (lane >> 1)) * 2; o[0] = s; o[1] = q; }
+      am = fmaxf(am, gm);
+      gm = wave_max(gm);
+      if (lane == 0) gn_max[sub * r32 + cb] = gm;
+    }
+  } else {
+    for (int64_t i = (int64_t)blockIdx.x * 256 + threadIdx.x; i < n4; i += (int64_t)gridDim.x * 256) am = amax4(am, value(i, (int)(i % K4)));
   }
   if (amax_rec) wave_amax_emit(am, amax_rec, (int)blockIdx.x * 4 + (int)(threadIdx.x >> 6));
 }
@@ -499,6 +549,8 @@
     if (p.tsplit < 2 || ((CB / 16) * KW & 1) || nst % p.tsplit || !p.split_ws || (size_t)p.tsplit * p.P * g.K * sizeof(float) > p.split_ws_bytes || (g.K & 3))
       return WDNO_EINVAL;
   } else p.tsplit = 1;
+  if (p.gn_sums && (KW != 3 || p.out_bf16 || (g.K & (SP ? 31 : 7)) || !p.gn_max)) { p.gn_sums = nullptr; p.gn_max = nullptr; }
+  p.gn_taken = p.gn_sums ? 1 : 0;
   int grid = wdno_num_cus() & ~7;
   if (grid < 8) grid = 8;
   if ((int64_t)p.ntiles * p.tsplit < grid) grid = p.ntiles * p.tsplit;
@@ -509,7 +561,8 @@
   if (p.tsplit > 1) {
     const int64_t n4 = p.P * g.K / 4;
     conv_split_reduce_kernel<<<(unsigned)std::min<int64_t>((n4 + 255) / 256, 2048), 256, 0, st>>>(
-        (const float4*)p.split_ws, p.tsplit, n4, g.K / 4, LP ? nullptr : sx, sw, (const float4*)bias, (const float4*)residual, (float4*)y, p.amax_rec);
+        (const float4*)p.split_ws, p.tsplit, n4, g.K / 4, LP ? nullptr : sx, sw, (const float4*)bias, (const float4*)residual, (float4*)y, p.amax_rec,
+        p.gn_sums, p.gn_max);
   }
   return WDNO_OK;
 }
diff --git a/wdno_amd/csrc/debug_modes.h b/wdno_amd/csrc/debug_modes.h
--- a/wdno_amd/csrc/debug_modes.h
+++ b/wdno_amd/csrc/debug_modes.h
@@ -30,6 +30,8 @@
   X(WDNO_DBG_ATTN_BWD_ROWS, 68)                                              \
   X(WDNO_DBG_WGRAD_NO_SPLIT_PAIR, 70)    \
   X(WDNO_DBG_STEM_TILES_256, 72)                             \
+          \
+  X(WDNO_DBG_GN_SEPARATE_STATS, 73)                                                                                                                \
                                \
   X(WDNO_DBG_NO_DMA_STAMP_CYCLES, 123)                                                                                                             \
   X(WDNO_DBG_NO_DMA_STAMP_EPILOGUE, 124)                                                                                                           \
diff --git a/wdno_amd/csrc/norm.hip b/wdno_amd/csrc/norm.hip
--- a/wdno_amd/csrc/norm.hip
+++ b/wdno_amd/csrc/norm.hip
@@ -164,7 +164,8 @@
                                                            const float* __restrict__ ss, float* __restrict__ stats_out,
                                                            float* __restrict__ cb, float* __restrict__ gb, int64_t S, int C, int G,
                                                            int nchunk, float eps, const float* __restrict__ mx = nullptr,
-                                                           float* __restrict__ bound_rec = nullptr) {
+                                                           float* __restrict__ bound_rec = nullptr, const double* __restrict__ rsum = nullptr,
+                                                           const float* __restrict__ rmax = nullptr) {
   __shared__ double chs[GN_MAXC], chq[GN_MAXC];
   __shared__ float gmean[GN_MAXC], grstd[GN_MAXC];
   const int n = blockIdx.x, cg = C / G;
@@ -178,7 +179,44 @@
   if (stats_in) stats_in += (int64_t)gs0 * 2;
   const int Call = C, Gall = G;
   C = csn; G = gs1 - gs0;
-  if (part) {
+  if (rsum) {
+    __shared__ double ta[256], tb[256];
+    const int64_t T = (S + 31) >> 5;
+    const int R8 = Call >> 3, rpg = cg >> 3;
+    const double2* rs = reinterpret_cast<const double2*>(rsum) + (int64_t)n * T * R8;
+    for (int g = 0; g < G; ++g) {
+      const int r0 = (cs0 + g * cg) >> 3;
+      const int64_t items = T * rpg;
+      double a[4] = {0, 0, 0, 0}, b[4] = {0, 0, 0, 0};
+      for (int64_t i0 = threadIdx.x; i0 < items; i0 += 1024) {
+        double2 v[4];
+#pragma unroll
+        for (int u = 0; u < 4; ++u) {
+          const int64_t i = i0 + u * 256, t = i / rpg;
+          v[u] = i < items ? rs[t * R8 + r0 + (int)(i - t * rpg)] : make_double2(0.0, 0.0);
+        }
+#pragma unroll
+        for (int u = 0; u < 4; ++u) { a[u] += v[u].x; b[u] += v[u].y; }
+      }
+      ta[threadIdx.x] = (a[0] + a[1]) + (a[2] + a[3]); tb[threadIdx.x] = (b[0] + b[1]) + (b[2] + b[3]);
+      __syncthreads();
+      for (int o = 128; o > 0; o >>= 1) {
+        if (threadIdx.x < o) { ta[threadIdx.x] += ta[threadIdx.x + o]; tb[threadIdx.x] += tb[threadIdx.x + o]; }
+        __syncthreads();
+      }
+      if (threadIdx.x == 0) {
+        const double m = (double)cg * (double)S;
+        const double mean = ta[0] / m;
+        double var = tb[0] / m - mean * mean;
+        if (var < 0) var = 0;
+        const float rstd = (float)(1.0 / sqrt(var + (double)eps));
+        gmean[g] = (float)mean; grstd[g] = rstd;
+        stats_out[((int64_t)n * Gall + g) * 2 + 0] = (float)mean;
+        stats_out[((int64_t)n * Gall + g) * 2 + 1] = rstd;
+      }
+      __syncthreads();
+    }
+  } else if (part) {
     gn_chunk_totals(part, n, nchunk, Call, chs, chq, cs0, csn);
     if (cg > 64) {
       __shared__ double ra[256], rb[256];
@@ -233,7 +271,11 @@
   }
   if (bound_rec) {
     float mxx = 0.f;
-    for (int k = threadIdx.x; k < nchunk; k += 256) mxx = fmaxf(mxx, mx[((int64_t)n * nchunk + k) * 2]);
+    if (rmax) {
+      const int64_t nm = ((S + 31) >> 5) * ((Call + 31) >> 5);
+      for (int64_t k = threadIdx.x; k < nm; k += 256) mxx = fmaxf(mxx, rmax[(int64_t)n * nm + k]);
+    } else
+      for (int k = threadIdx.x; k < nchunk; k += 256) mxx = fmaxf(mxx, mx[((int64_t)n * nchunk + k) * 2]);
     __shared__ float bm[3][4];
     float v[3] = {wave_max(ma), wave_max(mb), wave_max(mxx)};
     if ((threadIdx.x & 63) == 0)
@@ -544,12 +586,17 @@
   if ((C & 3) || C > GN_MAXC || (C % G) != 0) return WDNO_EUNSUPPORTED;
   return WDNO_OK;
 }
+static int gn_rec_check(int64_t N, int64_t S, int C, int G) { return ((S & 31) && N != 1) || (C & 7) || ((C / G) & 7) ? WDNO_EINVAL : WDNO_OK; }
+static inline const float* gn_rec_max(const void* conv_rec, int64_t N, int64_t S, int C) {
+  return conv_rec ? (const float*)((const char*)conv_rec + (size_t)((N * S + 31) / 32) * (size_t)(C / 8) * 2 * sizeof(double)) : nullptr;
+}
 #define GN_PARTIAL0(XB, ...) do { if (XB) gn_partial_kernel<0, gn_bf16><<<__VA_ARGS__; else gn_partial_kernel<0, float><<<__VA_ARGS__; } while (0)
-extern "C" int wdno_groupnorm_act_fwd_amax_t(const void* x, int x_bf16, const float* gamma, const float* beta, const float* ss, float* y,
+static int gn_fwd_amax(const void* x, int x_bf16, const void* conv_rec, const float* gamma, const float* beta, const float* ss, float* y,
                                       float* stats, float* amax_rec, int64_t N, int64_t S, int C, int G, float eps, int silu,
                                       void* ws, size_t ws_bytes, wdno_stream_t s) {
   int rc = gn_check(N, S, C, G);
   if (rc) return rc;
+  if (conv_rec && (rc = gn_rec_check(N, S, C, G))) return rc;
   if (ws_bytes < wdno_groupnorm_ws_bytes(N, S, C, G)) return WDNO_EWORKSPACE;
   const int nchunk = gn_chunks(S, N, C);
   double* part = (double*)ws;
@@ -558,13 +605,25 @@
   const int txp = pow2ceil(C / 4);
   const int64_t rpc = cdiv64(S, nchunk);
   hipStream_t st = as_stream(s);
-  GN_PARTIAL0(x_bf16, dim3(nchunk, (unsigned)N), 256, 0, st>>>(x, nullptr, nullptr, nullptr, part, S, C, C / G, G, txp, rpc, 0));
-  gn_finalize_kernel<<<dim3((unsigned)N, gn_slices(C, G)), 256, 0, st>>>(part, nullptr, gamma, beta, ss, stats, cb, gb, S, C, G, nchunk, eps);
+  if (!conv_rec) GN_PARTIAL0(x_bf16, dim3(nchunk, (unsigned)N), 256, 0, st>>>(x, nullptr, nullptr, nullptr, part, S, C, C / G, G, txp, rpc, 0));
+  gn_finalize_kernel<<<dim3((unsigned)N, gn_slices(C, G)), 256, 0, st>>>(part, nullptr, gamma, beta, ss, stats, cb, gb, S, C, G, nchunk, eps, nullptr, nullptr,
+                                                                         (const double*)conv_rec, gn_rec_max(conv_rec, N, S, C));
   int gx = stream_grid(S * (C / 4), 256);
   if (gx > 512) gx = 512;
   if (x_bf16) gn_apply_kernel<gn_bf16><<<dim3(gx, (unsigned)N), 256, 0, st>>>(x, cb, y, S, C, silu, amax_rec);
   else gn_apply_kernel<float><<<dim3(gx, (unsigned)N), 256, 0, st>>>(x, cb, y, S, C, silu, amax_rec);
   return wdno_check_launch();
+}
+extern "C" int wdno_groupnorm_act_fwd_amax_t(const void* x, int x_bf16, const float* gamma, const float* beta, const float* ss, float* y,
+                                      float* stats, float* amax_rec, int64_t N, int64_t S, int C, int G, float eps, int silu,
+                                      void* ws, size_t ws_bytes, wdno_stream_t s) {
+  return gn_fwd_amax(x, x_bf16, nullptr, gamma, beta, ss, y, stats, amax_rec, N, S, C, G, eps, silu, ws, ws_bytes, s);
+}
+extern "C" int wdno_groupnorm_act_fwd_amax_rec(const float* x, const void* conv_rec, const float* gamma, const float* beta, const float* ss, float* y,
+                                      float* stats, float* amax_rec, int64_t N, int64_t S, int C, int G, float eps, int silu,
+                                      void* ws, size_t ws_bytes, wdno_stream_t s) {
+  if (!conv_rec) return WDNO_EINVAL;
+  return gn_fwd_amax(x, 0, conv_rec, gamma, beta, ss, y, stats, amax_rec, N, S, C, G, eps, silu, ws, ws_bytes, s);
 }
 extern "C" int wdno_groupnorm_act_fwd_amax(const float* x, const float* gamma, const float* beta, const float* ss, float* y,
                                       float* stats, float* amax_rec, int64_t N, int64_t S, int C, int G, float eps, int silu,
@@ -606,11 +665,12 @@
 extern "C" size_t wdno_groupnorm_fwd_planes_ws_bytes(int64_t N, int64_t S, int C, int G) {
   return wdno_groupnorm_ws_bytes(N, S, C, G) + (size_t)N * gn_chunks(S, N, C) * 2 * sizeof(float) + 128;
 }
-extern "C" int wdno_groupnorm_act_fwd_planes_t(const void* x, int x_bf16, const float* gamma, const float* beta, const float* ss, void* y_hi, void* y_lo,
+static int gn_fwd_planes(const void* x, int x_bf16, const void* conv_rec, const float* gamma, const float* beta, const float* ss, void* y_hi, void* y_lo,
                                              float* y_scale, float* stats, float* bound_rec, int64_t N, int64_t S, int C, int G, float eps,
                                              int silu, void* ws, size_t ws_bytes, wdno_stream_t s) {
   int rc = gn_check(N, S, C, G);
   if (rc) return rc;
+  if (conv_rec && (rc = gn_rec_check(N, S, C, G))) return rc;
   const int C8 = C / 8;
   if ((C & 7) || C8 > 256 || (C8 & (C8 - 1))) return WDNO_EUNSUPPORTED;
   if (ws_bytes < wdno_groupnorm_fwd_planes_ws_bytes(N, S, C, G)) return WDNO_EWORKSPACE;
@@ -622,26 +682,39 @@
   const int txp = pow2ceil(C / 4);
   const int64_t rpc = cdiv64(S, nchunk);
   hipStream_t st = as_stream(s);
-  GN_PARTIAL0(x_bf16, dim3(nchunk, (unsigned)N), 256, 0, st>>>(x, nullptr, nullptr, nullptr, part, S, C, C / G, G, txp, rpc, 0, y_lo ? mx : nullptr));
-  gn_finalize_kernel<<<dim3((unsigned)N, gn_slices(C, G)), 256, 0, st>>>(part, nullptr, gamma, beta, ss, stats, cb, gb, S, C, G, nchunk, eps, mx, y_lo ? bound_rec : nullptr);
+  if (!conv_rec) GN_PARTIAL0(x_bf16, dim3(nchunk, (unsigned)N), 256, 0, st>>>(x, nullptr, nullptr, nullptr, part, S, C, C / G, G, txp, rpc, 0, y_lo ? mx : nullptr));
+  gn_finalize_kernel<<<dim3((unsigned)N, gn_slices(C, G)), 256, 0, st>>>(part, nullptr, gamma, beta, ss, stats, cb, gb, S, C, G, nchunk, eps, mx, y_lo ? bound_rec : nullptr,
+                                                                         (const double*)conv_rec, gn_rec_max(conv_rec, N, S, C));
   int gx = stream_grid(S * (C / 8), 256);
   if (gx > 512) gx = 512;
   if (x_bf16) gn_apply_planes_kernel<gn_bf16><<<dim3(gx, (unsigned)N), 256, 0, st>>>(x, cb, (_Float16*)y_hi, (_Float16*)y_lo, y_scale, bound_rec, S, C, silu);
   else gn_apply_planes_kernel<float><<<dim3(gx, (unsigned)N), 256, 0, st>>>(x, cb, (_Float16*)y_hi, (_Float16*)y_lo, y_scale, bound_rec, S, C, silu);
   return wdno_check_launch();
 }
+extern "C" int wdno_groupnorm_act_fwd_planes_t(const void* x, int x_bf16, const float* gamma, const float* beta, const float* ss, void* y_hi, void* y_lo,
+                                             float* y_scale, float* stats, float* bound_rec, int64_t N, int64_t S, int C, int G, float eps,
+                                             int silu, void* ws, size_t ws_bytes, wdno_stream_t s) {
+  return gn_fwd_planes(x, x_bf16, nullptr, gamma, beta, ss, y_hi, y_lo, y_scale, stats, bound_rec, N, S, C, G, eps, silu, ws, ws_bytes, s);
+}
+extern "C" int wdno_groupnorm_act_fwd_planes_rec(const float* x, const void* conv_rec, const float* gamma, const float* beta, const float* ss, void* y_hi, void* y_lo,
+                                             float* y_scale, float* stats, float* bound_rec, int64_t N, int64_t S, int C, int G, float eps,
+                                             int silu, void* ws, size_t ws_bytes, wdno_stream_t s) {
+  if (!conv_rec) return WDNO_EINVAL;
+  return gn_fwd_planes(x, 0, conv_rec, gamma, beta, ss, y_hi, y_lo, y_scale, stats, bound_rec, N, S, C, G, eps, silu, ws, ws_bytes, s);
+}
 extern "C" int wdno_groupnorm_act_fwd_planes(const float* x, const float* gamma, const float* beta, const float* ss, void* y_hi, void* y_lo,
                                              float* y_scale, float* stats, float* bound_rec, int64_t N, int64_t S, int C, int G, float eps,
                                              int silu, void* ws, size_t ws_bytes, wdno_stream_t s) {
   return wdno_groupnorm_act_fwd_planes_t(x, 0, gamma, beta, ss, y_hi, y_lo, y_scale, stats, bound_rec, N, S, C, G, eps, silu, ws, ws_bytes, s);
 }
 
-extern "C" int wdno_groupnorm_act_add_fwd_planes_t(const void* x, int x_bf16, const float* gamma, const float* beta, const float* ss, const float* residual,
+static int gn_add_fwd_planes(const void* x, int x_bf16, const void* conv_rec, const float* gamma, const float* beta, const float* ss, const float* residual,
                                                  const float* res_rec, float* y, void* y_hi, void* y_lo, float* y_scale, float* stats,
                                                  float* bound_rec, float* y_amax_rec, int64_t N, int64_t S, int C, int G, float eps, int silu,
                                                  void* ws, size_t ws_bytes, wdno_stream_t s) {
   int rc = gn_check(N, S, C, G);
   if (rc) return rc;
+  if (conv_rec && (rc = gn_rec_check(N, S, C, G))) return rc;
   const int C8 = C / 8;
   if ((C & 7) || C8 > 256 || (C8 & (C8 - 1))) return WDNO_EUNSUPPORTED;
   if (!residual || !y || (y_lo && (!y_hi || !res_rec || !bound_rec || !y_scale))) return WDNO_EINVAL;
@@ -654,8 +727,9 @@
   const int txp = pow2ceil(C / 4);
   const int64_t rpc = cdiv64(S, nchunk);
   hipStream_t st = as_stream(s);
-  GN_PARTIAL0(x_bf16, dim3(nchunk, (unsigned)N), 256, 0, st>>>(x, nullptr, nullptr, nullptr, part, S, C, C / G, G, txp, rpc, 0, y_lo ? mx : nullptr));
-  gn_finalize_kernel<<<dim3((unsigned)N, gn_slices(C, G)), 256, 0, st>>>(part, nullptr, gamma, beta, ss, stats, cb, gb, S, C, G, nchunk, eps, mx, y_lo ? bound_rec : nullptr);
+  if (!conv_rec) GN_PARTIAL0(x_bf16, dim3(nchunk, (unsigned)N), 256, 0, st>>>(x, nullptr, nullptr, nullptr, part, S, C, C / G, G, txp, rpc, 0, y_lo ? mx : nullptr));
+  gn_finalize_kernel<<<dim3((unsigned)N, gn_slices(C, G)), 256, 0, st>>>(part, nullptr, gamma, beta, ss, stats, cb, gb, S, C, G, nchunk, eps, mx, y_lo ? bound_rec : nullptr,
+                                                                         (const double*)conv_rec, gn_rec_max(conv_rec, N, S, C));
   int gx = stream_grid(S * (C / 8), 256);
   if (gx > 512) gx = 512;
   if (x_bf16) gn_apply_add_planes_kernel<gn_bf16><<<dim3(gx, (unsigned)N), 256, 0, st>>>(x, cb, residual, y, (_Float16*)y_hi, (_Float16*)y_lo, y_scale, bound_rec,
@@ -663,6 +737,21 @@
   else gn_apply_add_planes_kernel<float><<<dim3(gx, (unsigned)N), 256, 0, st>>>(x, cb, residual, y, (_Float16*)y_hi, (_Float16*)y_lo, y_scale, bound_rec, res_rec,
                                                                            y_amax_rec, S, C, silu);
   return wdno_check_launch();
+}
+extern "C" int wdno_groupnorm_act_add_fwd_planes_t(const void* x, int x_bf16, const float* gamma, const float* beta, const float* ss, const float* residual,
+                                                 const float* res_rec, float* y, void* y_hi, void* y_lo, float* y_scale, float* stats,
+                                                 float* bound_rec, float* y_amax_rec, int64_t N, int64_t S, int C, int G, float eps, int silu,
+                                                 void* ws, size_t ws_bytes, wdno_stream_t s) {
+  return gn_add_fwd_planes(x, x_bf16, nullptr, gamma, beta, ss, residual, res_rec, y, y_hi, y_lo, y_scale, stats, bound_rec, y_amax_rec, N, S, C, G, eps, silu,
+                           ws, ws_bytes, s);
+}
+extern "C" int wdno_groupnorm_act_add_fwd_planes_rec(const float* x, const void* conv_rec, const float* gamma, const float* beta, const float* ss, const float* residual,
+                                                 const float* res_rec, float* y, void* y_hi, void* y_lo, float* y_scale, float* stats,
+                                                 float* bound_rec, float* y_amax_rec, int64_t N, int64_t S, int C, int G, float eps, int silu,
+                                                 void* ws, size_t ws_bytes, wdno_stream_t s) {
+  if (!conv_rec) return WDNO_EINVAL;
+  return gn_add_fwd_planes(x, 0, conv_rec, gamma, beta, ss, residual, res_rec, y, y_hi, y_lo, y_scale, stats, bound_rec, y_amax_rec, N, S, C, G, eps, silu,
+                           ws, ws_bytes, s);
 }
 extern "C" int wdno_groupnorm_act_add_fwd_planes(const float* x, const float* gamma, const float* beta, const float* ss, const float* residual,
                                                  const float* res_rec, float* y, void* y_hi, void* y_lo, float* y_scale, float* stats,
diff --git a/wdno_amd/ops.py b/wdno_amd/ops.py
--- a/wdno_amd/ops.py
+++ b/wdno_amd/ops.py
@@ -421,6 +421,24 @@
     if rec is not None:
         t._wdno_amax = (rec, t._version)
     return t
+
+
+GN_FROM_CONV = os.environ.get('WDNO_GN_FROM_CONV', '1') != '0'
+
+
+def _leave_gn_records(t, buf, c):
+    t._wdno_gn = (buf, t._version, (t.numel() // c, c))
+
+
+def _gn_records(t, n, s, c, groups):
+    h = getattr(t, '_wdno_gn', None)
+    if (h is None or not GN_FROM_CONV or h[1] != t._version or h[2] != (n * s, c) or t.dtype != torch.float32 or (s % 32 and n != 1) or c % groups
+            or (c // groups) % 8):
+        return None
+    return h[0]
+
+
+GN_STATS_PASS_KEY = 'groupnorm_fwd with gn_partial_kernel<0>'
 
 
 def _known_amax(t):
@@ -670,7 +688,7 @@
 
 
 def conv_fwd_h3(planes, shape4, w, pack, kind, bias_p, residual, ks, st, pd, kp, out=None, osp=None, ostride=(1, 1, 1), ooff=(0, 0, 0),
-                amax_rec=None, zero_box=None, out16=False):
+                amax_rec=None, zero_box=None, out16=False, gn_rec=False):
     xh, xl, sx = planes
     n, d, h, ww = shape4
     cp8 = xh.shape[-1]
@@ -708,6 +726,17 @@
             wsb = _split_ws_bytes.get(key)
             if wsb is None:
                 wsb = _split_ws_bytes[key] = int(_lib_().wdno_conv_fwd_split_ws_bytes(C.byref(g)))
+        if gn_rec and tap and ks[2] == 3 and out is None:
+            nrec = int(_lib_().wdno_conv_gn_rec_bytes(C.byref(g)))
+            if nrec:
+                ws = torch.empty(wsb // 4, device=xh.device, dtype=torch.float32) if wsb else None
+                rec = torch.empty(nrec // 8, device=xh.device, dtype=torch.float64)
+                taken = C.c_int(0)
+                _lib.check(_lib_().wdno_conv_fwd_f16x3_gn(_p(xh), _p(xl), _p(sx), _p(wh), _p(wl), _p(sw), _p(bias_p), _p(residual), _p(y), _p(amax_rec),
+                                                          C.byref(g), _p(ws), wsb, _p(rec), nrec, C.byref(taken), _stream()), 'conv_fwd_f16x3_gn')
+                if taken.value:
+                    y._wdno_gn_buf = rec
+                return y
         if wsb:
             ws = torch.empty(wsb // 4, device=xh.device, dtype=torch.float32)
             _lib.check(_lib_().wdno_conv_fwd_f16x3_ws(_p(xh), _p(xl), _p(sx), _p(wh), _p(wl), _p(sw), _p(bias_p), _p(residual), _p(y),
@@ -1098,7 +1127,9 @@
                      and kp // 8 <= 256 and (kp // 8) & (kp // 8 - 1) == 0
                      and (not ctx.needs_input_grad[0] or (tuple(stride) == (1, 1, 1) and _use_h3(nx_ * dx_ * hx_ * wx_, kp * ks[0] * ks[1] * ks[2]))))
             y = _leave_amax(conv_fwd_h3(planes, tuple(x5.shape[:4]), weight, pack_fwd, 'f', bias_p, res5, ks, stride, padding, kp,
-                                        amax_rec=yrec, zero_box=zero_box_of(x_in) if x_in.dim() == 5 else None, out16=out16), yrec)
+                                        amax_rec=yrec, zero_box=zero_box_of(x_in) if x_in.dim() == 5 else None, out16=out16,
+                                        gn_rec=GN_FROM_CONV and getattr(ctx, 'to_norm', False) and x.dim() in (4, 5)), yrec)
+            gn_buf = getattr(y, '_wdno_gn_buf', None)
             ctx.save_for_backward(planes[0], planes[1], planes[2], weight)
         else:
             y = conv_fwd_raw(x5, pack_fwd(weight, cp, kp), bias_p, res5, ks, stride, padding, kp)
@@ -1108,6 +1139,8 @@
         ctx.meta = (ks, stride, padding, k, c, cp, kp, bias is not None, residual is not None, lead, x.dim())
         if lead is not None:
             y = y.reshape(*lead, kp) if x.dim() != 4 else y.squeeze(1)
+        if h3 and gn_buf is not None:
+            _leave_gn_records(y, gn_buf, kp)
         return y
 
     @staticmethod
@@ -1422,6 +1455,7 @@
         stats = torch.empty((lib.wdno_groupnorm_stats_floats(n, c, groups),), device=x.device, dtype=torch.float32)
         ssc = None if ss is None else _chk(ss, 'scale_shift')
         ctx.ss_slot = _claim_grad_slot(ss) if ssc is ss else None
+        grec = _gn_records(x_in, n, s, c, groups)
         c8_ = c // 8
         if out_planes and CONV_MATH in ('f16x3', 'bf16') and c % 8 == 0 and c8_ <= 256 and (c8_ & (c8_ - 1)) == 0:
             nbp = lib.wdno_groupnorm_fwd_planes_ws_bytes(n, s, c, groups)
@@ -1432,8 +1466,13 @@
                 lo = torch.empty((n * s, c), device=x.device, dtype=torch.float16)
                 brec = _amax_slot(x.device)
                 scale = brec[1:2]
-            _lib.check(lib.wdno_groupnorm_act_fwd_planes_t(_p(x), x16, _p(gamma), _p(beta), _p(ssc), _p(hi), _p(lo), _p(scale), _p(stats), _p(brec),
-                                                           n, s, c, groups, float(eps), int(act_silu), _p(wsp), nbp, _stream()), 'groupnorm_fwd_planes')
+            if grec is not None:
+                _lib.check(lib.wdno_groupnorm_act_fwd_planes_rec(_p(x), _p(grec), _p(gamma), _p(beta), _p(ssc), _p(hi), _p(lo), _p(scale), _p(stats), _p(brec),
+                                                                 n, s, c, groups, float(eps), int(act_silu), _p(wsp), nbp, _stream()), 'groupnorm_fwd_planes_rec')
+            else:
+                with _timed(GN_STATS_PASS_KEY, 0.0):
+                    _lib.check(lib.wdno_groupnorm_act_fwd_planes_t(_p(x), x16, _p(gamma), _p(beta), _p(ssc), _p(hi), _p(lo), _p(scale), _p(stats), _p(brec),
+                                                                   n, s, c, groups, float(eps), int(act_silu), _p(wsp), nbp, _stream()), 'groupnorm_fwd_planes')
             ctx.save_for_backward(x, gamma, beta, ssc, stats)
             ctx.meta = (n, s, c, groups, int(act_silu))
             ctx.epoch = _param_epoch(gamma)
@@ -1442,8 +1481,13 @@
             return _planes_only(y, (hi, lo, scale))
         y = torch.empty(x.shape, device=x.device, dtype=torch.float32)
         rec = _new_amax_record(x.device)
-        _lib.check(lib.wdno_groupnorm_act_fwd_amax_t(_p(x), x16, _p(gamma), _p(beta), _p(ssc), _p(y), _p(stats), _p(rec), n, s, c, groups,
-                                                     float(eps), int(act_silu), _p(ws), nb, _stream()), 'groupnorm_fwd')
+        if grec is not None:
+            _lib.check(lib.wdno_groupnorm_act_fwd_amax_rec(_p(x), _p(grec), _p(gamma), _p(beta), _p(ssc), _p(y), _p(stats), _p(rec), n, s, c, groups,
+                                                           float(eps), int(act_silu), _p(ws), nb, _stream()), 'groupnorm_fwd_rec')
+        else:
+            with _timed(GN_STATS_PASS_KEY, 0.0):
+                _lib.check(lib.wdno_groupnorm_act_fwd_amax_t(_p(x), x16, _p(gamma), _p(beta), _p(ssc), _p(y), _p(stats), _p(rec), n, s, c, groups,
+                                                             float(eps), int(act_silu), _p(ws), nb, _stream()), 'groupnorm_fwd')
         ctx.save_for_backward(x, gamma, beta, ssc, stats)
         ctx.meta = (n, s, c, groups, int(act_silu))
         ctx.epoch = _param_epoch(gamma)
@@ -1530,9 +1574,16 @@
         ssc = None if ss is None else _chk(ss, 'scale_shift')
         ctx.ss_slot = _claim_grad_slot(ss) if ssc is ss else None
         yrec = _new_amax_record(x.device)
-        _lib.check(lib.wdno_groupnorm_act_add_fwd_planes_t(_p(x), x16, _p(gamma), _p(beta), _p(ssc), _p(res), None, _p(y), None, None, None, _p(stats),
-                                                         None, _p(yrec), n, s, c, groups, float(eps), int(act_silu), _p(ws), nb, _stream()),
-                   'groupnorm_add_fwd')
+        grec = _gn_records(x_in, n, s, c, groups)
+        if grec is not None:
+            _lib.check(lib.wdno_groupnorm_act_add_fwd_planes_rec(_p(x), _p(grec), _p(gamma), _p(beta), _p(ssc), _p(res), None, _p(y), None, None, None, _p(stats),
+                                                                 None, _p(yrec), n, s, c, groups, float(eps), int(act_silu), _p(ws), nb, _stream()),
+                       'groupnorm_add_fwd_rec')
+        else:
+            with _timed(GN_STATS_PASS_KEY, 0.0):
+                _lib.check(lib.wdno_groupnorm_act_add_fwd_planes_t(_p(x), x16, _p(gamma), _p(beta), _p(ssc), _p(res), None, _p(y), None, None, None, _p(stats),
+                                                                 None, _p(yrec), n, s, c, groups, float(eps), int(act_silu), _p(ws), nb, _stream()),
+                           'groupnorm_add_fwd')
         ctx.save_for_backward(x, gamma, beta, ssc, stats)
         ctx.meta = (n, s, c, groups, int(act_silu))
         ctx.epoch = _param_epoch(gamma)
```

New measurement: 33.83 (median of 2 runs). No clear change (+0.2%).
